# katehai/m-cedm

Measured on AMD Instinct MI355X. Metric: denoised_states_per_sec_18step_edm_heun, higher is better.
Workload: dtype f32; 1 GPU; SWE-periodic 128x128, EDM U-Net ch=128 ch_mult=[1,1,1,1] attn@16^2 (BASELINE config 3); states_per_gpu=32, global_batch=32, H=128, W=128, sampler=EDM Heun, 18 steps, 35 NFE/state, S_churn=0, w=0, fp64 state / fp32 net, parallelism=batch-sharded x1, no data-path collective, launch=one HIP graph per sampler call

## Files before the change

### include/mcedm_hip.h

```cpp
#ifndef MCEDM_HIP_H_
#define MCEDM_HIP_H_

#include <stddef.h>
#include <stdint.h>

#ifdef __cplusplus
extern "C" {
#endif

#define MCEDM_ABI_VERSION 4
#define MCEDM_REDUCE_SCRATCH_BYTES (4096 * 8 + 64)
#define MCEDM_MAX_LEVELS 8

typedef enum {
  MCEDM_OK = 0,
  MCEDM_ERR_INVALID = -1,
  MCEDM_ERR_UNSUPPORTED = -2,
  MCEDM_ERR_WORKSPACE = -3,
  MCEDM_ERR_HIP = -4
} mcedm_status;

#define MCEDM_DX_NONE 0
#define MCEDM_DX_CAT 1
#define MCEDM_DX_ENC 2
typedef struct {
  int32_t in_channels;
  int32_t cond_channels;
  int32_t out_channels;
  int32_t ch;
  int32_t n_levels;
  int32_t ch_mult[MCEDM_MAX_LEVELS];
  int32_t num_res_blocks;
  int32_t resolution;
  int32_t n_attn_resolutions;
  int32_t attn_resolutions[MCEDM_MAX_LEVELS];
  int32_t channels_per_head;
  float eps;
  int32_t dx_channels;
  int32_t dx_mode;
} mcedm_unet_desc;

typedef struct {
  int32_t timesteps;
  double sigma_min, sigma_max, rho;
  double S_churn, S_min, S_max, S_noise;
  double w;
  double sigma_data;
  double net_sigma_min, net_sigma_max;
} mcedm_sampler_desc;

typedef struct mcedm_plan mcedm_plan;

int mcedm_version(void);
const char* mcedm_last_error(void);

int mcedm_unet_plan_create(const mcedm_unet_desc* desc, mcedm_plan** out);
void mcedm_unet_plan_destroy(mcedm_plan* plan);

#define MCEDM_VARIANT_CONV_WINO 0
#define MCEDM_VARIANT_CONV_WINO1 1
#define MCEDM_VARIANT_CONV_RESIDENT 2
#define MCEDM_VARIANT_CONV8 3
#define MCEDM_VARIANT_ATTN_FUSED 4
#define MCEDM_VARIANT_WGRAD_WINO 5
#define MCEDM_VARIANT_CONV1X1_REG 6
#define MCEDM_VARIANT_CONV_WINO_FOLD 7
#define MCEDM_VARIANT_CONV_WINO_UPZ 8
int mcedm_unet_plan_set_variant(mcedm_plan* plan, int which, int value);

int mcedm_unet_param_count(const mcedm_plan* plan);
int mcedm_unet_param_info(const mcedm_plan* plan, int index, const char** name, int64_t* numel,
                          int32_t* ndim, int64_t shape[4]);

int mcedm_unet_packed_bytes(const mcedm_plan* plan, size_t* bytes);
int mcedm_unet_pack_weights(const mcedm_plan* plan, const float* const* params, void* packed, void* stream);

int mcedm_unet_workspace_bytes(const mcedm_plan* plan, int B, int H, int W, int training, size_t* bytes);

int mcedm_unet_forward(const mcedm_plan* plan, const void* packed, const float* x, const float* cond,
                       const float* x_scale, const float* noise_labels, int n_noise, float* out,
                       void* workspace, size_t workspace_bytes, int B, int H, int W, int training,
                       void* stream);

int mcedm_edm_denoise(const mcedm_plan* plan, const void* packed, const float* x, const float* sigma,
                      int n_sigma, const float* cond, float* D_out, float* F_out, void* workspace,
                      size_t workspace_bytes, int B, int H, int W, int training, double sigma_data,
                      void* stream);

int mcedm_sampler_workspace_bytes(const mcedm_plan* plan, int B, int H, int W, size_t* bytes);
int mcedm_heun_sample(const mcedm_plan* plan, const void* packed, const mcedm_sampler_desc* sp,
                      const float* cond, const float* mask, const float* init_noise,
                      const double* step_noise, double* out, int return_last, void* workspace,
                      size_t workspace_bytes, int B, int H, int W, void* stream);

int mcedm_heun_sample_rng(const mcedm_plan* plan, const void* packed, const mcedm_sampler_desc* sp, const float* cond,
                          const float* mask, const float* init_noise, const uint64_t* rng_seed, double* out, int return_last,
                          void* workspace, size_t workspace_bytes, int B, int H, int W, void* stream);
typedef struct {
  int32_t system;
  float half_dt, dx;
  float two_dx;
  float sub_h, div_h, sub_u, div_u;
  double weight;
} mcedm_guidance_desc;
int mcedm_heun_sample_guided(const mcedm_plan* plan, const void* packed, const mcedm_sampler_desc* sp,
                             const mcedm_guidance_desc* gd, const float* cond, const float* mask,
                             const float* init_noise, const double* step_noise, double* out, int return_last,
                             void* workspace, size_t workspace_bytes, int B, int H, int W, void* stream);
int mcedm_heun_sample_guided_rng(const mcedm_plan* plan, const void* packed, const mcedm_sampler_desc* sp,
                                 const mcedm_guidance_desc* gd, const float* cond, const float* mask, const float* init_noise,
                                 const uint64_t* rng_seed, double* out, int return_last, void* workspace, size_t workspace_bytes,
                                 int B, int H, int W, void* stream);
int mcedm_unet_forward_dx(const mcedm_plan* plan, const void* packed, const float* x, const float* dx, const float* cond,
                          const float* x_scale, const float* noise_labels, int n_noise, float* out, void* workspace,
                          size_t workspace_bytes, int B, int H, int W, int training, void* stream);
int mcedm_edm_denoise_dx(const mcedm_plan* plan, const void* packed, const float* x, const float* dx, const float* sigma,
                         int n_sigma, const float* cond, float* D_out, float* F_out, void* workspace,
                         size_t workspace_bytes, int B, int H, int W, int training, double sigma_data, void* stream);
int mcedm_edm_denoise_backward_dx(const mcedm_plan* plan, const void* packed, const float* const* params, const float* x,
                                  const float* dx, const float* sigma, int n_sigma, const float* cond, const float* dD,
                                  float* const* grads, void* workspace, size_t workspace_bytes, int B, int H, int W,
                                  double sigma_data, int n_buckets, const int32_t* bucket_first_param,
                                  void* const* bucket_events, void* stream);
int mcedm_heun_sample_dxcond(const mcedm_plan* plan, const void* packed, const mcedm_sampler_desc* sp,
                             const mcedm_guidance_desc* dxc, const mcedm_guidance_desc* gd, const float* cond,
                             const float* init_noise, const double* step_noise, double* out, int return_last,
                             void* workspace, size_t workspace_bytes, int B, int H, int W, void* stream);
int mcedm_heun_sample_dxcond_rng(const mcedm_plan* plan, const void* packed, const mcedm_sampler_desc* sp,
                                 const mcedm_guidance_desc* dxc, const mcedm_guidance_desc* gd, const float* cond,
                                 const float* init_noise, const uint64_t* rng_seed, double* out, int return_last, void* workspace,
                                 size_t workspace_bytes, int B, int H, int W, void* stream);
int mcedm_edm_t_steps(const mcedm_sampler_desc* sp, double* t_steps);

int mcedm_edm_loss(const float* D, const float* x, const float* mask, const float* sigma, int B, int C,
                   int H, int W, double sigma_data, float* loss_out, float* dD_out, void* scratch, size_t scratch_bytes,
                   void* stream);

int mcedm_edm_noise_inputs(const float* x, const float* mask, const float* noise, const float* rnd_normal,
                           int B, int C, int H, int W, double P_mean, double P_std, float* x_noise,
                           float* sigma_out, void* stream);

int mcedm_edm_denoise_backward(const mcedm_plan* plan, const void* packed, const float* const* params,
                               const float* x, const float* sigma, int n_sigma, const float* cond,
                               const float* dD, float* const* grads, void* workspace,
                               size_t workspace_bytes, int B, int H, int W, double sigma_data, void* stream);

int mcedm_unet_grad_buckets(const mcedm_plan* plan, int max_buckets, int32_t* first_param, int* n_buckets);
int mcedm_edm_denoise_backward_bucketed(const mcedm_plan* plan, const void* packed, const float* const* params,
                                        const float* x, const float* sigma, int n_sigma, const float* cond,
                                        const float* dD, float* const* grads, void* workspace,
                                        size_t workspace_bytes, int B, int H, int W, double sigma_data,
                                        int n_buckets, const int32_t* bucket_first_param,
                                        void* const* bucket_events, void* stream);

int mcedm_sqnorm(const float* g, size_t n, double* sqnorm_out, void* scratch, size_t scratch_bytes, void* stream);

int mcedm_adam_ema_step(float* param, const float* grad, float* exp_avg, float* exp_avg_sq, float* ema,
                        size_t n, double lr, double beta1, double beta2, double eps, double weight_decay,
                        const double* sqnorm, double max_norm, double grad_scale, double ema_beta,
                        int64_t step, void* stream);


int mcedm_eps_noise_inputs(const float* x, const float* noise, const int64_t* t, const float* sqrt_ab, const float* sqrt_1mab,
                           int n_table, int B, int C, int H, int W, float* x_noise, float* labels, void* stream);
int mcedm_eps_self_cond(const float* x_noise, const float* F0, const int64_t* t, const float* sqrt_ab, const float* sqrt_1mab,
                        int n_table, const float* cond, int cond_channels, int in_channels, int B, int H, int W,
                        float* cond_out, void* stream);
int mcedm_eps_loss(const float* F, const float* eps, int B, int C, int H, int W, float* loss_out, float* dF_out, void* scratch,
                   size_t scratch_bytes, void* stream);
int mcedm_unet_backward(const mcedm_plan* plan, const void* packed, const float* const* params, const float* x,
                        const float* cond, const float* x_scale, const float* noise_labels, int n_noise, const float* dF,
                        float* const* grads, void* workspace, size_t workspace_bytes, int B, int H, int W, void* stream);
int mcedm_unet_backward_bucketed(const mcedm_plan* plan, const void* packed, const float* const* params, const float* x,
                                 const float* cond, const float* x_scale, const float* noise_labels, int n_noise,
                                 const float* dF, float* const* grads, void* workspace, size_t workspace_bytes, int B, int H,
                                 int W, int n_buckets, const int32_t* bucket_first_param, void* const* bucket_events,
                                 void* stream);

typedef struct {
  int32_t timesteps;
  int32_t cond_channels;
  const double* t_steps;
  const double* t_hat;
  const float* c_noise;
  double S_noise;
// ... 32 lines not shown
                     mcedm_coef* coef_out, float* stats_out, void* stream);
int mcedm_op_conv(const float* xa, const float* xb, int Ca, int Cb, const mcedm_coef* coef, int coef_batch, int act,
                  int resample, int Hs, int Ws, int H, int W, const float* wpk, const float* bias_pk,
                  const float* res, int res_mode, float* out, int Cout, int B, int k, void* stream);
size_t mcedm_op_conv_wino_packed_floats(int Cout, int Cin);
int mcedm_op_pack_conv_wino(const float* w, int Cout, int Cin, float* wino, void* stream);
int mcedm_op_conv_wino(const float* xa, const float* xb, int Ca, int Cb, const mcedm_coef* coef, int coef_batch, int act,
                       int resample, int H, int W, const float* wino, const float* bias, const float* res, int res_mode,
                       float* out, int Cout, int B, void* stream);
int mcedm_op_conv_wino_sums(const float* xa, const float* xb, int Ca, int Cb, const mcedm_coef* coef, int coef_batch, int act,
                            int resample, int H, int W, const float* wino, const float* bias, const float* res, int res_mode,
                            float* out, float* gsum, int Cout, int B, void* stream);
int mcedm_op_pack_conv_wino_dgrad(const float* w, int Cout, int Cin, float* wino, void* stream);
int mcedm_op_embedding(const float* labels, int n, int ch, const float* w0, const float* b0, const float* w1,
                       const float* b1, const float* waff, const float* baff, int rows, float* freqs_scratch,
                       float* emb_out, float* film_out, void* stream);
int mcedm_op_attention(const float* qkv, float* out, int B, int heads, int T, void* stream);
int mcedm_op_attn_block64(const float* y, const float* gamma, const float* beta, float eps, const float* wq_pk,
                          const float* bq_pk, const float* wp_pk, const float* bp_pk, float* z, float* gsum, int B, void* stream);
size_t mcedm_op_wgrad_scratch_floats(int Cout, int Cin, int k, int B, int H, int W);
int mcedm_op_conv_wgrad(const float* dy, const float* xa, const float* xb, int Ca, int Cb, const mcedm_coef* coef,
                        int coef_batch, int act, int resample, int Hs, int Ws, int H, int W, int Cout, int B, int k,
                        int qkv_heads, float* scratch, float* dw, float* db, void* stream);
int mcedm_op_gn_bwd(const float* dact, int resample, const float* xa, const float* xb, int Ca, int Cb, int Hs, int Ws,
                    int B, const mcedm_coef* coef, const float* stats, const float* gamma, const float* beta,
                    const float* film, int film_batch, int film_stride, int act, float* dxa, float* dxb, int accumulate,
                    const float* add, int add_mode, float* ab, float* dgamma, float* dbeta, float* dfilm,
                    int dfilm_stride, void* stream);
#define MCEDM_GN_SYNC_WORDS 130
int mcedm_op_gn_bwd_sync(const float* dact, int resample, const float* xa, const float* xb, int Ca, int Cb, int Hs, int Ws,
                         int B, const mcedm_coef* coef, const float* stats, const float* gamma, const float* beta,
                         const float* film, int film_batch, int film_stride, int act, float* dxa, float* dxb, int accumulate,
                         const float* add, int add_mode, float* ab, float* dgamma, float* dbeta, float* dfilm,
                         int dfilm_stride, unsigned int* sync, void* stream);
int mcedm_op_attention_bwd(const float* qkv, const float* a, const float* da, float* dqkv, float* lse_scratch, int B,
                           int heads, int T, void* stream);
int mcedm_op_ddim_cond_step(const float* xt, const float* F, const float* Fu, const float* noise, double w, float s0, float s1,
                            float sa_next, float c1, float c2, float* xt_next, float* condp, float* condp_u, int cond_channels,
                            int plan_cond_channels, int B, int C, int H, int W, float* xs, int T_xs, int t_xs, float* x0s,
                            int T_x0, int t_x0, void* stream);
int mcedm_op_ddim_cond_step_rng(const float* xt, const float* F, const float* Fu, const uint64_t* rng_seed, uint64_t draw, double w,
                                float s0, float s1, float sa_next, float c1, float c2, float* xt_next, float* condp, float* condp_u,
                                int cond_channels, int plan_cond_channels, int B, int C, int H, int W, float* xs, int T_xs,
                                int t_xs, float* x0s, int T_x0, int t_x0, void* stream);
int mcedm_op_set_conv_tile(int mt, int ph, int pw);
int mcedm_op_set_conv8(int enable);
int mcedm_op_set_conv_resident(int enable);
int mcedm_op_set_conv_wino(int enable);
int mcedm_op_set_conv_wino1(int enable);
int mcedm_op_set_wgrad_wino(int enable);
int mcedm_op_set_conv1x1_reg(int enable);
int mcedm_op_set_conv_wino_fold(int enable);
int mcedm_op_set_conv_wino_upz(int enable);
int mcedm_op_pack_conv_frag(const float* w, int Cout, int Cin, float* wfrag, void* stream);
int mcedm_op_conv_skip(const float* x, int Cin, const mcedm_coef* coef, int act, int H, int W, const float* wpk, const float* wino,
                       const float* bias, const float* res, const float* sk_xa, const float* sk_xb, int sk_Ca, int sk_Cb,
                       const float* sk_wpk, const float* sk_wfrag, const float* sk_bias, float* out, float* gsum, int Cout, int B,
                       void* stream);
int mcedm_op_set_attn_fused(int enable);
int mcedm_op_set_conv_debug(unsigned long long* buf);

typedef struct {
  int32_t in_channels;
  int32_t out_channels;
  int32_t ch;
  int32_t n_levels;
  int32_t ch_mult[MCEDM_MAX_LEVELS];
  int32_t num_res_blocks;
  int32_t resolution;
  int32_t n_attn_resolutions;
  int32_t attn_resolutions[MCEDM_MAX_LEVELS];
  int32_t self_cond;
  float eps;
} mcedm_ddpm_desc;

typedef struct {
  int32_t timesteps;
  double sigma_min, sigma_max, rho;
  double S_churn, S_min, S_max, S_noise;
  double w;
  int32_t n_repeat;
  int32_t n_time_h, n_time_u;
  int32_t h_ch, u_ch;
  int32_t num_diffusion_timesteps;
  const float* edm_steps;
  const float* alphas_cumprod_ext;
} mcedm_repaint_desc;

typedef struct mcedm_ddpm_plan mcedm_ddpm_plan;
int mcedm_ddpm_plan_create(const mcedm_ddpm_desc* desc, mcedm_ddpm_plan** out);
void mcedm_ddpm_plan_destroy(mcedm_ddpm_plan* plan);
int mcedm_ddpm_plan_set_variant(mcedm_ddpm_plan* plan, int which, int value);
int mcedm_ddpm_param_count(const mcedm_ddpm_plan* plan);
int mcedm_ddpm_param_info(const mcedm_ddpm_plan* plan, int index, const char** name, int64_t* numel, int32_t* ndim,
                          int64_t shape[4]);
int mcedm_ddpm_packed_bytes(const mcedm_ddpm_plan* plan, size_t* bytes);
int mcedm_ddpm_pack_weights(const mcedm_ddpm_plan* plan, const float* const* params, const float* temb_freqs, void* packed,
                            void* stream);
int mcedm_ddpm_workspace_bytes(const mcedm_ddpm_plan* plan, int B, size_t* bytes);
int mcedm_ddpm_forward(const mcedm_ddpm_plan* plan, const void* packed, const float* x, float t, float* out, void* workspace,
                       size_t workspace_bytes, int B, void* stream);
int mcedm_ddpm_denoise(const mcedm_ddpm_plan* plan, const void* packed, const float* x, float sigma, float c_noise,
                       float* D_out, float* F_out, void* workspace, size_t workspace_bytes, int B, void* stream);
int mcedm_repaint_schedule(const mcedm_repaint_desc* sp, double* t_steps);
int mcedm_repaint_workspace_bytes(const mcedm_ddpm_plan* plan, int B, size_t* bytes);
int mcedm_repaint_sample(const mcedm_ddpm_plan* plan, const void* packed, const mcedm_repaint_desc* sp, const float* hu,
// ... 76 lines not shown
```

### m-cedm_amd/csrc/common.hpp

```cpp
#pragma once
#include <hip/hip_runtime.h>
#include <cstdarg>
#include <cstdint>
#include <cstdio>

#include "mcedm_hip.h"

namespace mcedm {

void set_error(const char* fmt, ...);

#define MCEDM_HIP_TRY(expr)                                                                   \
  do {                                                                                        \
    hipError_t e__ = (expr);                                                                  \
    if (e__ != hipSuccess) {                                                                  \
      ::mcedm::set_error("%s failed: %s (%s:%d)", #expr, hipGetErrorString(e__), __FILE__, __LINE__); \
      return MCEDM_ERR_HIP;                                                                   \
    }                                                                                         \
  } while (0)

#define MCEDM_LAUNCH_CHECK(what)                                                               \
  do {                                                                                        \
    hipError_t e__ = hipGetLastError();                                                       \
    if (e__ != hipSuccess) {                                                                  \
      ::mcedm::set_error("launch of %s failed: %s", what, hipGetErrorString(e__));            \
      return MCEDM_ERR_HIP;                                                                   \
    }                                                                                         \
  } while (0)

#define MCEDM_REQUIRE(cond, ...)                                                              \
  do {                                                                                        \
    if (!(cond)) {                                                                            \
      ::mcedm::set_error(__VA_ARGS__);                                                        \
      return MCEDM_ERR_INVALID;                                                               \
    }                                                                                         \
  } while (0)

enum KernelVariant { KV_CONV_WINO = 0, KV_CONV_WINO1 = 1, KV_CONV_RESIDENT = 2, KV_CONV8 = 3, KV_ATTN_FUSED = 4, KV_WGRAD_WINO = 5,
                     KV_CONV1X1_REG = 6, KV_CONV_WINO_FOLD = 7, KV_CONV_WINO_UPZ = 8, KV_COUNT = 9 };
struct KernelVariants { int v[KV_COUNT] = {-1, -1, -1, -1, -1, -1, -1, -1, -1}; };
const KernelVariants* current_variants();
struct VariantScope {
  const KernelVariants* prev;
  explicit VariantScope(const KernelVariants* kv);
  ~VariantScope();
};
static inline int variant_choice(int which, int global, int env_default) {
  const KernelVariants* kv = current_variants();
  if (kv && kv->v[which] >= 0) return kv->v[which];
  return global >= 0 ? global : env_default;
}

typedef float f32x16 __attribute__((ext_vector_type(16)));
typedef float f32x4 __attribute__((ext_vector_type(4)));
typedef float f32x2 __attribute__((ext_vector_type(2)));

static inline int ceil_div(int a, int b) { return (a + b - 1) / b; }
#ifdef __HIPCC__
__device__ __forceinline__ void xcd_group_map(int map, int& bx, int& by) {
  const int nx = gridDim.x, ny = gridDim.y;
  bx = blockIdx.x; by = blockIdx.y;
  if (!map || (ny & 7) != 0) return;
  const int lin = bx + by * nx;
  const int c = lin & 7, i = lin >> 3;
  by = (i / nx) * 8 + c;
  bx = i - (i / nx) * nx;
}
#endif

static inline size_t align_up(size_t v, size_t a) { return (v + a - 1) / a * a; }

struct __attribute__((aligned(16))) Coef {
  float mean, scale, offset, pad;
};

enum Resample { RS_NONE = 0, RS_UP = 1, RS_DOWN = 2, RS_S2 = 3 };

struct SumTiles {
  int tiles = 0;
  int tiles_x = 0;
  int ph = 0, pw = 0;
  int rc = 4;
};
__host__ __device__ static inline int sum_tile_count(const SumTiles& g, int t, int H, int W) {
  const int ty = t / g.tiles_x, tx = t - ty * g.tiles_x;
  const int h = H - ty * g.ph < g.ph ? H - ty * g.ph : g.ph;
  const int w = W - tx * g.pw < g.pw ? W - tx * g.pw : g.pw;
  return g.rc * h * w;
}

struct GnArgs {
  const float* xa; const float* xb; int Ca, Cb;
  int HW, B, groups;
// ... 10 lines not shown
};
int launch_gn_coef_from_sums(const GnArgs& a, hipStream_t stream);
int launch_gn_coef(const GnArgs& a, hipStream_t stream);
bool gn_sums_usable(const GnArgs& a);

struct ConvArgs {
  const float* xa;
  const float* xb;
  int Ca, Cb;
  const Coef* coef;
  int coef_batch;
  int act;
  int resample;
  int Hs, Ws;
  int H, W;
  const float* wpk;
  const float* wino;
  const float* bias;
  const float* res;
  int res_mode;
  float* out;
  int Cout;
  int B;
  float* gsum;
  int gsum_rc;
  SumTiles* gsum_tiles;
  const float* sk_xa; const float* sk_xb; int sk_Ca, sk_Cb;
  const float* sk_wpk; const float* sk_bias;
  GnArgs gn; int gn_on;
  int coef_rows;
  unsigned long long* dbg;
  const float* sk_wfrag;
};

int launch_conv(const ConvArgs& a, int taps, hipStream_t stream);
size_t conv_wino_packed_floats(int Cout, int Cin);
int launch_pack_conv_wino(const float* w, float* dst, int Cout, int Cin, int transpose_flip, hipStream_t stream);
bool conv_wino_applicable(const ConvArgs& a, int taps);
bool conv_wino_shape_ok(int Cout, int Cin, int H, int W);
bool conv_wino_fold_shape_ok(int Cout, int sk_Ca, int sk_Cb, int H, int W);
void set_conv_wino_fold(int enable);
void set_conv_wino_upz(int enable);
size_t conv_frag_packed_floats(int Cout, int Cin);
int launch_pack_conv_frag(const float* w, float* dst, int Cout, int Cin, hipStream_t stream);
void set_conv_wino(int enable);
bool conv_wino_preferred(const ConvArgs& a);
int launch_conv_wino(const ConvArgs& a, hipStream_t stream);
static inline int cout_padded(int Cout) { return (Cout + 31) / 32 * 32; }
int conv_resolve_identity(ConvArgs& a);
unsigned long long* conv_debug_buffer();
int try_launch_conv_resident(const ConvArgs& a, int taps, hipStream_t stream);
int try_launch_conv1x1_reg(const ConvArgs& a, int taps, hipStream_t stream);
void set_conv1x1_reg(int enable);
void set_conv_resident(int enable);
static inline int conv_max_tiles(int H, int W) { return ((H + 3) / 4) * ((W + 7) / 8); }
void set_conv_tile_override(int mt, int ph, int pw);
void set_conv8(int enable);
void set_conv_debug(unsigned long long* buf);
int conv_mt_for(int Cout);
int conv_kc_for(int taps);
size_t conv_packed_floats(int Cout, int Cin, int taps);
int launch_pack_conv(const float* w, float* dst, int Cout, int Cin, int taps, int qkv_heads, int transpose_flip,
                     hipStream_t stream);
int launch_pack_bias(const float* b, float* dst, int Cout, int qkv_heads, hipStream_t stream);



struct EmbArgs {
  const float* labels; int n;
  int ch;
  const float* freqs;
  const float* w0; const float* b0; const float* w1; const float* b1;
  const float* waff; const float* baff; int rows;
  float* emb;
  float* film;
};
int launch_embedding(const EmbArgs& a, hipStream_t stream);

int launch_attention(const float* qkv, float* out, int B, int heads, int T, hipStream_t stream);
bool attn_block_fused_applicable(int C, int heads, int H, int W, int groups);
int launch_attn_block64(const float* y, float* z, const float* gamma, const float* beta, float eps, int groups, const float* wq,
                        const float* bq, const float* wp, const float* bp, float* gsum, SumTiles* gsum_tiles, int B,
                        hipStream_t stream);
void set_attn_fused(int enable);

}
```

### m-cedm_amd/csrc/conv_mfma.hip

```cpp
#include <atomic>
#include <cstdlib>

#include "common.hpp"
#include "conv_tile.hpp"
#include "pack.hpp"
#include "prof.hpp"

namespace mcedm {

__device__ Coef k_identity_coef = {0.f, 1.f, 0.f, 0.f};


template <class C>
__device__ __forceinline__ void conv_skip_phase(const ConvArgs& p, const TileGeom<C, RS_NONE>& G, float* xl, float* wl,
                                                f32x16 (&acc)[C::TM][C::TN], int n, int m0, int coutp, int aoff,
                                                const int (&boff)[C::TN], int tid, int wave) {
  static_assert(C::TAPS == 9, "the folded projection rides on a 3x3 conv");
  constexpr int SUB = TileGeom<C, RS_NONE>::SUB;
  constexpr int KS = 8;
  constexpr int V4 = C::MT / 4;
  constexpr int NV4 = KS * V4;
  static_assert(NV4 <= C::NT && C::KC == KS, "one float4 of the skip slab per thread");
  const int Cin = p.sk_Ca + p.sk_Cb;
  const int iters = (Cin + KS - 1) / KS;
// ... 738 lines not shown
  if (TAPS == 9 && a.W >= 24 && (long long)a.H * a.W <= 1024) {
    if (coutp % 128 == 0 && blocks_for(128, 8, 16) >= want) return launch_cfg<ConvCfg<128, 8, 16, 1, 4, TAPS, KC>>(a, stream);
    if (coutp % 64 == 0) return launch_cfg<ConvCfg<64, 8, 16, 1, 4, TAPS, KC, 256, MID_CPI>>(a, stream);
    return launch_cfg<ConvCfg<32, 8, 32, 1, 4, TAPS, KC>>(a, stream);
  }
  if (a.W >= 24) {
    static int conv8_env = -1;
    if (conv8_env < 0) { const char* e = getenv("MCEDM_CONV8"); conv8_env = e ? atoi(e) : 0; }
    if (variant_choice(KV_CONV8, g_conv8, conv8_env) && !a.sk_wpk && a.gsum_rc != 2 && TAPS == 9 && a.resample == RS_NONE && coutp % 128 == 0 && a.Ca + a.Cb <= 2048 &&
        blocks_for(128, 16, 32) >= 224)
      return launch_conv8(a, stream);
    if (coutp % 128 == 0 && blocks_for(128, 8, 32) >= want) return launch_cfg<ConvCfg<128, 8, 32, 1, 4, TAPS, KC>>(a, stream);
    if (coutp % 64 == 0 && blocks_for(64, 8, 32) >= want) return launch_cfg<ConvCfg<64, 8, 32, 1, 4, TAPS, KC>>(a, stream);
    return launch_cfg<ConvCfg<32, 8, 32, 1, 4, TAPS, KC>>(a, stream);
  }
  if (coutp % 128 == 0 && blocks_for(128, 16, 16) >= want) return launch_cfg<ConvCfg<128, 16, 16, 1, 4, TAPS, KC>>(a, stream);
  if (coutp % 64 == 0 && blocks_for(64, 16, 16) >= want) return launch_cfg<ConvCfg<64, 16, 16, 1, 4, TAPS, KC>>(a, stream);
  return launch_cfg<ConvCfg<32, 16, 16, 1, 4, TAPS, KC>>(a, stream);
#endif
}

int launch_conv(const ConvArgs& a, int taps, hipStream_t stream) {
  MCEDM_REQUIRE(taps == 9 || taps == 1, "conv: taps must be 9 or 1 (got %d)", taps);
  MCEDM_REQUIRE(a.B > 0 && a.H > 0 && a.W > 0 && a.Cout > 0 && a.Ca + a.Cb > 0, "conv: empty shape");
  MCEDM_REQUIRE(a.out && a.wpk, "conv: null output / weights");
  if (a.resample == RS_UP) MCEDM_REQUIRE(a.Hs * 2 == a.H && a.Ws * 2 == a.W, "conv: up-resample needs H = 2*Hs");
  else if (a.resample == RS_DOWN) MCEDM_REQUIRE(a.Hs == a.H * 2 && a.Ws == a.W * 2, "conv: down-resample needs Hs = 2*H");
  else if (a.resample == RS_S2) MCEDM_REQUIRE(taps == 9 && a.Hs == a.H * 2 && a.Ws == a.W * 2 && !a.res,
                                              "conv: the stride-2 conv is 3x3 on an even-sized source, without residual");
  else MCEDM_REQUIRE(a.Hs == a.H && a.Ws == a.W, "conv: source size mismatch");
  if (a.res && a.res_mode == RS_UP) MCEDM_REQUIRE(a.H % 2 == 0 && a.W % 2 == 0, "conv: up residual needs even size");
  if (a.sk_wpk) MCEDM_REQUIRE(taps == 9 && a.resample == RS_NONE && a.sk_Ca + a.sk_Cb > 0 && (a.sk_xa || a.sk_xb) && a.Cout > 4,
                              "conv: a folded 1x1 projection rides on an un-resampled 3x3 conv with more than 4 output channels");
  MCEDM_REQUIRE((unsigned long long)a.Hs * a.Ws * 4ull < (1ull << 32) &&
                (unsigned long long)cout_padded(a.Cout) * (a.Ca + a.Cb + 16) * taps * 4ull < (1ull << 32),
                "conv: plane or weight table exceeds the 4 GiB buffer range");
  if (a.res) {
    const unsigned long long rpix = a.res_mode == RS_DOWN ? 4ull * a.H * a.W : a.res_mode == RS_UP ? (a.H / 2ull) * (a.W / 2ull)
                                                                                                    : 1ull * a.H * a.W;
    MCEDM_REQUIRE(rpix * a.Cout * 4ull < (1ull << 32), "conv: one sample of the residual exceeds the 4 GiB buffer range");
  }
  if (taps == 9 && a.Cout <= 4 && a.resample == RS_NONE && !a.res && !a.gsum && !g_force_mt && (long long)a.H * a.W >= 4096)
    return launch_small_cout(a, stream);
  if (a.resample == RS_S2) return dispatch_s2(a, stream);
  if (!g_force_mt && taps == 9 && a.wino && conv_wino_preferred(a) && conv_wino_applicable(a, taps)) return launch_conv_wino(a, stream);
  if (!g_force_mt && taps == 1) {
    const int rc = try_launch_conv1x1_reg(a, taps, stream);
    if (rc != -1) return rc;
  }
  if (!g_force_mt) {
    const int rc = try_launch_conv_resident(a, taps, stream);
    if (rc != -1) return rc;
  }
  return taps == 9 ? dispatch<9, 8>(a, stream) : dispatch<1, 16>(a, stream);
}

}
```

### m-cedm_amd/csrc/edm.hip

```cpp
#include "common.hpp"
#include "edm.hpp"

namespace mcedm {

static inline int grid_for(size_t n) {
  size_t b = (n + 255) / 256;
  return (int)(b < 2048 ? (b ? b : 1) : 2048);
}

__global__ void precond_prepare_kernel(const float* __restrict__ sigma_dev, float sigma_host, int use_host, int n,
                                       float sigma_data, int cond_ch, int in_ch, int dx_ch, float* __restrict__ coefs4,
                                       float* __restrict__ c_noise, Coef* __restrict__ conv_in_coef) {
  const int i = blockIdx.x * blockDim.x + threadIdx.x;
  if (i >= n) return;
  const float s = use_host ? sigma_host : sigma_dev[i];
  const float sd2 = sigma_data * sigma_data;
  const float s2 = s * s;
  const float c_skip = sd2 / (s2 + sd2);
  const float c_out = s * sigma_data / sqrtf(s2 + sd2);
  const float c_in = 1.0f / sqrtf(sd2 + s2);
  const float cn = logf(s) / 4.0f;
  coefs4[4 * i + 0] = c_skip;
  coefs4[4 * i + 1] = c_out;
  coefs4[4 * i + 2] = c_in;
  coefs4[4 * i + 3] = cn;
  c_noise[i] = cn;
  const int Ct = cond_ch + in_ch + dx_ch;
  for (int c = 0; c < Ct; ++c)
    conv_in_coef[(size_t)i * Ct + c] = Coef{0.f, (c < cond_ch || c >= cond_ch + in_ch) ? 1.0f : c_in, 0.f, 0.f};
}

int launch_precond_prepare(const float* sigma_dev, float sigma_host, int use_host, int n, float sigma_data,
                           int cond_ch, int in_ch, int dx_ch, float* coefs4, float* c_noise, Coef* conv_in_coef,
                           hipStream_t stream) {
  hipLaunchKernelGGL(precond_prepare_kernel, dim3(ceil_div(n, 64)), dim3(64), 0, stream, sigma_dev, sigma_host,
                     use_host, n, sigma_data, cond_ch, in_ch, dx_ch, coefs4, c_noise, conv_in_coef);
  MCEDM_LAUNCH_CHECK("precond_prepare_kernel");
  return MCEDM_OK;
}

__global__ void precond_finish_kernel(const float* __restrict__ x, const float* __restrict__ F,
                                      const float* __restrict__ Fu, float w, const float* __restrict__ coefs4,
                                      int n_sigma, size_t per_sample, size_t total, float* __restrict__ D,
                                      float* __restrict__ F_out) {
  for (size_t i = blockIdx.x * (size_t)blockDim.x + threadIdx.x; i < total; i += (size_t)gridDim.x * blockDim.x) {
    const size_t b = n_sigma == 1 ? 0 : i / per_sample;
    float f = F[i];
    if (Fu) f = (w + 1.0f) * f - w * Fu[i];
    if (F_out) F_out[i] = f;
    D[i] = coefs4[4 * b] * x[i] + coefs4[4 * b + 1] * f;
  }
}

int launch_precond_finish(const float* x, const float* F, const float* Fu, float w, const float* coefs4, int n_sigma,
                          size_t per_sample, size_t total, float* D, float* F_out, hipStream_t stream) {
  hipLaunchKernelGGL(precond_finish_kernel, dim3(grid_for(total)), dim3(256), 0, stream, x, F, Fu, w, coefs4, n_sigma,
                     per_sample, total, D, F_out);
  MCEDM_LAUNCH_CHECK("precond_finish_kernel");
  return MCEDM_OK;
}

__global__ void heun_init_kernel(const float* __restrict__ cond, int cond_ch, int in_ch, size_t hw,
                                 const float* __restrict__ mask, const float* __restrict__ noise, double t0,
                                 size_t total, double* __restrict__ x, float* __restrict__ x32) {
  for (size_t i = blockIdx.x * (size_t)blockDim.x + threadIdx.x; i < total; i += (size_t)gridDim.x * blockDim.x) {
    const size_t b = i / (in_ch * hw), r = i % (in_ch * hw);
    const float m = mask ? mask[i] : 1.0f;
    const float known = mask ? cond[b * cond_ch * hw + r] : 0.0f;
    const float keep = known * (1.0f - m);
    const double v = (double)keep + ((double)noise[i] * t0) * (double)m;
    x[i] = v;
    x32[i] = (float)v;
  }
}

__global__ void heun_churn_kernel(double* __restrict__ x, const double* __restrict__ eps, const float* __restrict__ mask,
                                  double c, size_t total, float* __restrict__ x32) {
  for (size_t i = blockIdx.x * (size_t)blockDim.x + threadIdx.x; i < total; i += (size_t)gridDim.x * blockDim.x) {
    const double v = x[i] + (c * eps[i]) * (mask ? (double)mask[i] : 1.0);
    x[i] = v;
    x32[i] = (float)v;
  }
}

__global__ void heun_euler_kernel(const double* __restrict__ x_hat, const float* __restrict__ D,
                                  const float* __restrict__ mask, double t_hat, double dt, size_t total,
                                  double* __restrict__ d_cur, double* __restrict__ x_next, float* __restrict__ x32,
                                  const float* __restrict__ dxg, float wgt, float gdiv) {
  for (size_t i = blockIdx.x * (size_t)blockDim.x + threadIdx.x; i < total; i += (size_t)gridDim.x * blockDim.x) {
    const double xh = x_hat[i];
    double d = (xh - (double)D[i]) / t_hat;
    if (dxg) d = d - (double)((wgt * dxg[i]) / gdiv);
    const double v = xh + (dt * d) * (mask ? (double)mask[i] : 1.0);
    d_cur[i] = d;
    x_next[i] = v;
    x32[i] = (float)v;
  }
}

__global__ void heun_correct_kernel(const double* __restrict__ x_hat, const double* __restrict__ d_cur,
                                    const float* __restrict__ D, const float* __restrict__ mask, double t_next, double dt,
                                    size_t total, double* __restrict__ x_next, float* __restrict__ x32,
                                    const float* __restrict__ dxg, float wgt, float gdiv) {
  for (size_t i = blockIdx.x * (size_t)blockDim.x + threadIdx.x; i < total; i += (size_t)gridDim.x * blockDim.x) {
    double dp = (x_next[i] - (double)D[i]) / t_next;
    if (dxg) dp = dp - (double)((wgt * dxg[i]) / gdiv);
    const double v = x_hat[i] + (dt * (0.5 * d_cur[i] + 0.5 * dp)) * (mask ? (double)mask[i] : 1.0);
    x_next[i] = v;
    x32[i] = (float)v;
  }
}

__global__ void heun_store_kernel(const double* __restrict__ x, int C, size_t hw, int t, int T, size_t total,
                                  double* __restrict__ out) {
  for (size_t i = blockIdx.x * (size_t)blockDim.x + threadIdx.x; i < total; i += (size_t)gridDim.x * blockDim.x) {
    const size_t c = i % C;
    const size_t p = (i / C) % hw;
    const size_t b = i / (C * hw);
    out[((b * T + t) * hw + p) * C + c] = x[(b * C + c) * hw + p];
  }
}

int launch_heun_init(const float* cond, int cond_ch, int in_ch, size_t hw, const float* mask, const float* noise,
                     double t0, size_t total, double* x, float* x32, hipStream_t s) {
  hipLaunchKernelGGL(heun_init_kernel, dim3(grid_for(total)), dim3(256), 0, s, cond, cond_ch, in_ch, hw, mask, noise, t0,
                     total, x, x32);
  MCEDM_LAUNCH_CHECK("heun_init_kernel");
  return MCEDM_OK;
}
int launch_heun_churn(double* x, const double* eps, const float* mask, double c, size_t total, float* x32, hipStream_t s) {
  hipLaunchKernelGGL(heun_churn_kernel, dim3(grid_for(total)), dim3(256), 0, s, x, eps, mask, c, total, x32);
  MCEDM_LAUNCH_CHECK("heun_churn_kernel");
  return MCEDM_OK;
}
int launch_heun_euler(const double* x_hat, const float* D, const float* mask, double t_hat, double dt, size_t total,
                      double* d_cur, double* x_next, float* x32, hipStream_t s, const float* dxg, float wgt, float gdiv) {
  hipLaunchKernelGGL(heun_euler_kernel, dim3(grid_for(total)), dim3(256), 0, s, x_hat, D, mask, t_hat, dt, total, d_cur,
                     x_next, x32, dxg, wgt, gdiv);
  MCEDM_LAUNCH_CHECK("heun_euler_kernel");
  return MCEDM_OK;
}
int launch_heun_correct(const double* x_hat, const double* d_cur, const float* D, const float* mask, double t_next,
                        double dt, size_t total, double* x_next, float* x32, hipStream_t s, const float* dxg, float wgt,
                        float gdiv) {
  hipLaunchKernelGGL(heun_correct_kernel, dim3(grid_for(total)), dim3(256), 0, s, x_hat, d_cur, D, mask, t_next, dt,
                     total, x_next, x32, dxg, wgt, gdiv);
  MCEDM_LAUNCH_CHECK("heun_correct_kernel");
  return MCEDM_OK;
}
int launch_heun_store(const double* x, int C, size_t hw, int t, int T, size_t total, double* out, hipStream_t s) {
  hipLaunchKernelGGL(heun_store_kernel, dim3(grid_for(total)), dim3(256), 0, s, x, C, hw, t, T, total, out);
  MCEDM_LAUNCH_CHECK("heun_store_kernel");
  return MCEDM_OK;
}

__device__ __forceinline__ void philox4x32_10(unsigned (&c)[4], unsigned k0, unsigned k1) {
#pragma unroll
  for (int r = 0; r < 10; ++r) {
    const unsigned long long p0 = 0xD2511F53ull * c[0], p1 = 0xCD9E8D57ull * c[2];
    const unsigned n0 = (unsigned)(p1 >> 32) ^ c[1] ^ k0, n1 = (unsigned)p1;
    const unsigned n2 = (unsigned)(p0 >> 32) ^ c[3] ^ k1, n3 = (unsigned)p0;
    c[0] = n0; c[1] = n1; c[2] = n2; c[3] = n3;
    k0 += 0x9E3779B9u; k1 += 0xBB67AE85u;
  }
}
__device__ __forceinline__ void normal_pair(const unsigned (&c)[4], double& z0, double& z1) {
  const double u1 = ((double)((((unsigned long long)c[0] << 32) | c[1]) >> 11) + 1.0) * (1.0 / 9007199254740992.0);
  const double u2 = (double)((((unsigned long long)c[2] << 32) | c[3]) >> 11) * (1.0 / 9007199254740992.0);
  const double r = sqrt(-2.0 * log(u1));
  double sn, cs;
  sincos(6.283185307179586476925 * u2, &sn, &cs);
  z0 = r * cs; z1 = r * sn;
}
__global__ void heun_churn_rng_kernel(double* __restrict__ x, const unsigned long long* __restrict__ seed_dev,
                                      unsigned long long draw, double c, size_t total, float* __restrict__ x32,
                                      const float* __restrict__ mask) {
  const unsigned long long seed = *seed_dev;
  const size_t pairs = (total + 1) / 2;
  for (size_t i = blockIdx.x * (size_t)blockDim.x + threadIdx.x; i < pairs; i += (size_t)gridDim.x * blockDim.x) {
    unsigned ctr[4] = {(unsigned)i, (unsigned)((unsigned long long)i >> 32), (unsigned)draw, (unsigned)(draw >> 32)};
    philox4x32_10(ctr, (unsigned)seed, (unsigned)(seed >> 32));
    double z0, z1;
    normal_pair(ctr, z0, z1);
    const double m0 = mask ? (double)mask[2 * i] : 1.0;
    const double v0 = x[2 * i] + (c * z0) * m0;
    x[2 * i] = v0; x32[2 * i] = (float)v0;
    if (2 * i + 1 < total) {
      const double m1 = mask ? (double)mask[2 * i + 1] : 1.0;
      const double v1 = x[2 * i + 1] + (c * z1) * m1;
      x[2 * i + 1] = v1; x32[2 * i + 1] = (float)v1;
    }
  }
}
int launch_heun_churn_rng(double* x, const unsigned long long* seed_dev, unsigned long long draw, double c, size_t total, float* x32,
                          hipStream_t s, const float* mask) {
  hipLaunchKernelGGL(heun_churn_rng_kernel, dim3(grid_for((total + 1) / 2)), dim3(256), 0, s, x, seed_dev, draw, c, total, x32, mask);
  MCEDM_LAUNCH_CHECK("heun_churn_rng_kernel");
// ... 599 lines not shown
```

### m-cedm_amd/csrc/edm.hpp

```cpp
#pragma once
#include <cmath>
#include <vector>

#include "common.hpp"

namespace mcedm {

int launch_precond_prepare(const float* sigma_dev, float sigma_host, int use_host, int n, float sigma_data,
                           int cond_ch, int in_ch, int dx_ch, float* coefs4, float* c_noise, Coef* conv_in_coef,
                           hipStream_t stream);
int launch_precond_finish(const float* x, const float* F, const float* Fu, float w, const float* coefs4, int n_sigma,
                          size_t per_sample, size_t total, float* D, float* F_out, hipStream_t stream);
int launch_heun_init(const float* cond, int cond_ch, int in_ch, size_t hw, const float* mask, const float* noise,
                     double t0, size_t total, double* x, float* x32, hipStream_t s);
int launch_heun_churn(double* x, const double* eps, const float* mask, double c, size_t total, float* x32,
                      hipStream_t s);
int launch_heun_churn_rng(double* x, const unsigned long long* seed_dev, unsigned long long draw, double c, size_t total, float* x32,
                          hipStream_t s, const float* mask = nullptr);
int launch_normal_fill(double* out, const unsigned long long* seed_dev, unsigned long long draw, size_t total, hipStream_t s);
int launch_uniform_fill(float* out, const unsigned long long* seed_dev, unsigned long long draw, size_t total, hipStream_t s);
int launch_heun_euler(const double* x_hat, const float* D, const float* mask, double t_hat, double dt, size_t total,
                      double* d_cur, double* x_next, float* x32, hipStream_t s, const float* dxg = nullptr, float wgt = 0.f,
                      float gdiv = 1.f);
int launch_heun_correct(const double* x_hat, const double* d_cur, const float* D, const float* mask, double t_next,
                        double dt, size_t total, double* x_next, float* x32, hipStream_t s, const float* dxg = nullptr,
                        float wgt = 0.f, float gdiv = 1.f);
int launch_heun_store(const double* x, int C, size_t hw, int t, int T, size_t total, double* out, hipStream_t s);

struct GuideIO {
  const float* in[2]; const float* gt[2];
  long in_sb[2], st, sx;
  float* out[2]; long out_sb[2], out_st, out_sx;
  float sub[2], div[2];
  int mean;
};
int launch_swe_guidance(const GuideIO& io, int B, int T, int X, float half_dt, float dx, float scale2_h, float scale2_u,
                        hipStream_t s);
int launch_darcy_guidance(const GuideIO& io, float* scratch, int B, int S, float two_dx, int calc_prob, hipStream_t s);

int launch_vp_finish(const float* x, const float* F, float sigma, size_t total, float* D, hipStream_t s);
int launch_vp_coef(float c_in, int n_self, int n_in, Coef* out, hipStream_t s);
int launch_vp_prepare(float c_in, int n_rows, float c_noise, Coef* coef, float* label, hipStream_t s);
int launch_vp_cfg_finish(const float* x, const float* F, const float* Fu, double w, float sigma, size_t total, float* D,
                         hipStream_t s);
int launch_edm_cfg_finish(const float* x, const float* F, const float* Fu, double w, float c_skip, float c_out, size_t total,
                          float* D, float* F_out, hipStream_t s);
int launch_repaint_init(const float* hu, const float* noise, const float* mask, float sa, float sb, double t0, size_t total,
                        double* x, float* x32, hipStream_t s);
int launch_repaint_known(double* x, const float* hu, const float* noise, const float* mask, float sa, float sb, int final_clean,
                         size_t total, float* x32, hipStream_t s);

int launch_ddim_x0(float* xt, const float* et, const float* hu, const float* mask, float s0, float s1, int renoise, size_t total,
                   float* x0, hipStream_t s);
int launch_ddim_next(const float* x0, const float* et, const float* hu, const float* hn, const float* mask, const float* noise,
                     float sa, float c1, float c2, size_t total, float* xt, hipStream_t s);
int launch_ddim_next_rng(const float* x0, const float* et, const float* hu, const float* hn, const float* mask,
                         const unsigned long long* seed_dev, unsigned long long draw, float sa, float c1, float c2, size_t total,
                         float* xt, hipStream_t s);
int launch_ddim_init(const float* hu, const float* hn, const float* mask, float sa, float sb, size_t total, float* xt, hipStream_t s);
int launch_store_f32(const float* x, int C, size_t hw, int t, int T, size_t total, float* out, hipStream_t s);

static inline std::vector<int> ddim_timestep_seq(int n, int N, int skip_type) {
  std::vector<int> seq;
  if (skip_type == 0) {
    const int skip = n / N;
    for (int v = 0; v < n; v += skip) seq.push_back(v);
  } else {
    const double hi = std::sqrt(n * 0.8);
    const double step = N > 1 ? hi / (double)(N - 1) : 0.0;
    for (int i = 0; i < N; ++i) {
      const double v = (N > 1 && i == N - 1) ? hi : (double)i * step;
      seq.push_back((int)(v * v));
    }
  }
  return seq;
}

struct DdimCondStep {
  const float *xt, *F, *Fu, *noise;
// ... 14 lines not shown
```

### m-cedm_amd/csrc/heun.hpp

```cpp
#pragma once
#include <cmath>
#include <utility>
#include <vector>

#include "edm.hpp"
#include "plan.hpp"

namespace mcedm {

struct HeunBufs { size_t x, xn, d, x32, D, total; };
template <class Bufs>
static inline size_t heun_take(Bufs& b, size_t bytes) { size_t o = b.total; b.total += align_up(bytes, 256); return o; }
static inline HeunBufs heun_bufs(size_t n) {
  HeunBufs b{};
  b.x = heun_take(b, n * 8); b.xn = heun_take(b, n * 8); b.d = heun_take(b, n * 8);
  b.x32 = heun_take(b, n * 4); b.D = heun_take(b, n * 4);
  return b;
}

struct HeunState {
  double *x, *xn, *d;
  float *x32, *D;
  int C;
  size_t hw, total;
  int N, Tout, return_last;
  hipStream_t s;
  double* out;
};
static inline HeunState heun_state(void* ws, const HeunBufs& b, int B, int C, size_t hw, int N, int return_last, double* out,
                                   hipStream_t s) {
  return HeunState{at<double>(ws, b.x), at<double>(ws, b.xn), at<double>(ws, b.d), at<float>(ws, b.x32), at<float>(ws, b.D),
                   C, hw, (size_t)B * C * hw, N, return_last ? 1 : N + 1, return_last, s, out};
}

static inline int heun_check_workspace(const char* who, size_t have, size_t need) {
  if (need > have) {
    set_error("%s: workspace too small (%zu < %zu bytes)", who, have, need);
    return MCEDM_ERR_WORKSPACE;
  }
  return MCEDM_OK;
}

static inline int heun_store_step(const HeunState& h, int slot) {
  return h.return_last ? MCEDM_OK : launch_heun_store(h.x, h.C, h.hw, slot, h.Tout, h.total, h.out, h.s);
}
static inline int heun_store_last(const HeunState& h) {
  return h.return_last ? launch_heun_store(h.x, h.C, h.hw, 0, 1, h.total, h.out, h.s) : MCEDM_OK;
}

static inline int heun_churn(const HeunState& h, double c, const double* eps, const unsigned long long* seed,
                             unsigned long long draw, const float* mask) {
  if (eps) return launch_heun_churn(h.x, eps, mask, c, h.total, h.x32, h.s);
  return launch_heun_churn_rng(h.x, seed, draw, c, h.total, h.x32, h.s, mask);
}

template <class Denoise>
static inline int heun_update(HeunState& h, int i, double t_hat, double t_next, const float* mask, Denoise&& denoise,
                              const float* dxg = nullptr, float wgt = 0.f, float gdiv = 1.f) {
  int rc;
  if ((rc = denoise(t_hat, false))) return rc;
  if ((rc = launch_heun_euler(h.x, h.D, mask, t_hat, t_next - t_hat, h.total, h.d, h.xn, h.x32, h.s, dxg, wgt, gdiv)))
    return rc;
  if (i < h.N - 1) {
    if ((rc = denoise(t_next, true))) return rc;
    if ((rc = launch_heun_correct(h.x, h.d, h.D, mask, t_next, t_next - t_hat, h.total, h.xn, h.x32, h.s, dxg, wgt, gdiv)))
      return rc;
  }
  std::swap(h.x, h.xn);
  return MCEDM_OK;
}

static inline int guidance_dx(int cond_channels, const mcedm_guidance_desc& g, const float* cond, const float* D, float* dx,
                              float* scratch, int B, int H, int W, hipStream_t s) {
  GuideIO io{};
  const long hw = (long)H * W;
  io.in[0] = cond; io.in[1] = D; io.gt[0] = cond; io.gt[1] = D;
  io.in_sb[0] = (long)cond_channels * hw; io.in_sb[1] = hw; io.st = W; io.sx = 1;
  io.out[0] = dx; io.out[1] = nullptr; io.out_sb[0] = hw; io.out_sb[1] = 0; io.out_st = W; io.out_sx = 1;
  io.sub[0] = g.sub_h; io.sub[1] = g.sub_u; io.div[0] = g.div_h; io.div[1] = g.div_u;
  io.mean = 1;
  if (g.system == 1)
    return launch_swe_guidance(io, B, H, W, g.half_dt, g.dx, g.div_h * g.div_h, g.div_u * g.div_u, s);
  MCEDM_REQUIRE(H == W && H > 4, "guidance: the Darcy residual needs a square grid larger than 4 x 4 (got %d x %d)", H, W);
  return launch_darcy_guidance(io, scratch, B, H, g.two_dx, 1, s);
}

static inline int vp_check_schedule(const mcedm_vp_sampler_desc* sp, const double* step_noise, const uint64_t* rng_seed) {
  MCEDM_REQUIRE(sp->timesteps >= 1 && sp->timesteps <= 4096, "vp_heun_sample: timesteps=%d out of range", sp->timesteps);
  for (int i = 0; i < sp->timesteps; ++i) {
    MCEDM_REQUIRE(sp->t_hat[i] >= sp->t_steps[i] && sp->t_steps[i] > 0.0, "vp_heun_sample: step %d: t_hat %g < t_cur %g or t_cur <= 0", i,
                  sp->t_hat[i], sp->t_steps[i]);
    MCEDM_REQUIRE(sp->t_hat[i] == sp->t_steps[i] || step_noise != nullptr || rng_seed != nullptr,
                  "vp_heun_sample: step %d churns (t_hat > t_cur) and needs step_noise (or mcedm_vp_heun_sample_rng)", i);
  }
  return MCEDM_OK;
}

template <class Denoise>
static inline int vp_heun_loop(HeunState& h, const mcedm_vp_sampler_desc* sp, const float* init_noise, const double* step_noise,
                               const uint64_t* rng_seed, Denoise&& denoise, const float* dxg = nullptr, float wgt = 0.f) {
  int rc;
  const int N = sp->timesteps;
  const double* t = sp->t_steps;
  if ((rc = launch_heun_init(nullptr, 0, h.C, h.hw, nullptr, init_noise, t[0], h.total, h.x, h.x32, h.s))) return rc;
  if ((rc = heun_store_step(h, 0))) return rc;
  for (int i = 0; i < N; ++i) {
    const double t_cur = t[i], t_next = t[i + 1], t_hat = sp->t_hat[i];
    if (t_hat != t_cur) {
      const double c = std::sqrt(t_hat * t_hat - t_cur * t_cur) * sp->S_noise;
      if ((rc = heun_churn(h, c, step_noise ? step_noise + (size_t)i * h.total : nullptr,
                           reinterpret_cast<const unsigned long long*>(rng_seed), (unsigned long long)i, nullptr))) return rc;
    }
    auto at_level = [&](double sigma, bool second) { return denoise(sigma, sp->c_noise[2 * i + (second ? 1 : 0)]); };
    if ((rc = heun_update(h, i, t_hat, t_next, nullptr, at_level, dxg, wgt, dxg ? (float)t_hat : 1.f))) return rc;
    if ((rc = heun_store_step(h, i + 1))) return rc;
  }
  return heun_store_last(h);
}
// ... 71 lines not shown
```

### m-cedm_amd/csrc/norm_emb_attn.hip

```cpp
#include <cstdlib>
#include <atomic>
#include "common.hpp"
#include "prof.hpp"

namespace mcedm {

__global__ __launch_bounds__(256) void gn_coef_kernel(GnArgs a) {
  const int C = a.Ca + a.Cb;
  const int cpg = C / a.groups;
  const int n = blockIdx.x / a.groups;
  const int g = blockIdx.x % a.groups;
  const int c0 = g * cpg;
  auto plane = [&](int c) {
    return (c < a.Ca) ? a.xa + ((size_t)n * a.Ca + c) * a.HW : a.xb + ((size_t)n * a.Cb + (c - a.Ca)) * a.HW;
  };
  const int N = cpg * a.HW;
  const float shift = plane(c0)[0];
  float s1[4] = {0.f, 0.f, 0.f, 0.f}, s2[4] = {0.f, 0.f, 0.f, 0.f};
  const int tid = threadIdx.x;
  for (int cl = 0; cl < cpg; ++cl) {
    const float* src = plane(c0 + cl);
    if ((a.HW & 3) == 0) {
      const float4* s4 = reinterpret_cast<const float4*>(src);
      const int N4 = a.HW >> 2;
// ... 158 lines not shown
#pragma unroll
  for (int off = 32; off > 0; off >>= 1)
#pragma unroll
    for (int r = 0; r < R; ++r) s[r] += __shfl_xor(s[r], off);
#pragma unroll
  for (int r = 0; r < R; ++r) out[r] = s[r];
}

constexpr int EMB_NT = 1024, EMB_R = 4;
__global__ __launch_bounds__(EMB_NT) void embedding_kernel(EmbArgs a) {
  extern __shared__ float sm[];
  float* e0 = sm;
  float* e1 = sm + a.ch;
  constexpr int NW = EMB_NT / 64;
  const int n = blockIdx.x, split = blockIdx.y, nsplit = gridDim.y;
  const int tid = threadIdx.x, lane = tid & 63, wave = tid >> 6, ch = a.ch, half = a.ch / 2;
  const float x = a.labels[n];
  for (int k = tid; k < ch; k += EMB_NT) {
    const float arg = x * a.freqs[k < half ? k : k - half];
    e0[k] = (k < half) ? cosf(arg) : sinf(arg);
  }
  __syncthreads();
  float s[EMB_R];
  for (int j = wave * EMB_R; j < ch; j += NW * EMB_R) {
    wave_dot_rows<EMB_R>(e0, a.w0 + (size_t)j * ch, ch, ch - j, ch, lane, s);
    if (lane == 0)
      for (int r = 0; r < EMB_R && j + r < ch; ++r) e1[j + r] = silu_e(s[r] + a.b0[j + r]);
  }
  __syncthreads();
  for (int j = wave * EMB_R; j < ch; j += NW * EMB_R) {
    wave_dot_rows<EMB_R>(e1, a.w1 + (size_t)j * ch, ch, ch - j, ch, lane, s);
    if (lane == 0)
      for (int r = 0; r < EMB_R && j + r < ch; ++r) {
        const float v = silu_e(s[r] + a.b1[j + r]);
        e0[j + r] = v;
        if (a.emb && split == 0) a.emb[(size_t)n * ch + j + r] = v;
      }
  }
  __syncthreads();
  const int per = (a.rows + nsplit - 1) / nsplit;
  const int r1 = min(a.rows, (split + 1) * per);
  for (int r0 = split * per + wave * EMB_R; r0 < r1; r0 += NW * EMB_R) {
    wave_dot_rows<EMB_R>(e0, a.waff + (size_t)r0 * ch, ch, r1 - r0, ch, lane, s);
    if (lane == 0)
      for (int r = 0; r < EMB_R && r0 + r < r1; ++r) a.film[(size_t)n * a.rows + r0 + r] = s[r] + a.baff[r0 + r];
  }
}

int launch_embedding(const EmbArgs& a, hipStream_t stream) {
  MCEDM_REQUIRE(a.n > 0 && a.ch > 0 && a.ch % 2 == 0, "embedding: bad shape n=%d ch=%d", a.n, a.ch);
  int nsplit = a.rows / 64;
  if (nsplit > 512 / a.n) nsplit = 512 / a.n;
  if (nsplit < 1) nsplit = 1;
  hipLaunchKernelGGL(embedding_kernel, dim3(a.n, nsplit), dim3(EMB_NT), 2 * a.ch * sizeof(float), stream, a);
  MCEDM_LAUNCH_CHECK("embedding_kernel");
  return MCEDM_OK;
}

__global__ __launch_bounds__(64) void attention_kernel(const float* __restrict__ qkv, float* __restrict__ out,
                                                       int T) {
  const int lane = threadIdx.x;
  const int l31 = lane & 31, h = lane >> 5;
  const int q0 = blockIdx.x * 32;
  const size_t bh = blockIdx.y;
  const float* Q = qkv + (bh * 3 + 0) * 64 * (size_t)T;
  const float* K = qkv + (bh * 3 + 1) * 64 * (size_t)T;
  const float* V = qkv + (bh * 3 + 2) * 64 * (size_t)T;
  const int q = q0 + l31;
  const int qc = q < T ? q : T - 1;

  float qreg[32];
#pragma unroll
  for (int s = 0; s < 32; ++s) qreg[s] = Q[(size_t)(2 * s + h) * T + qc] * 0.125f;

  float m = -INFINITY, l = 0.f;
  f32x16 o[2];
#pragma unroll
  for (int i = 0; i < 2; ++i)
#pragma unroll
    for (int r = 0; r < 16; ++r) o[i][r] = 0.f;

  for (int k0 = 0; k0 < T; k0 += 32) {
    const bool full = (k0 + 32 <= T);
    const int kk = k0 + l31;
    const int kc = kk < T ? kk : T - 1;
    f32x16 s;
#pragma unroll
    for (int r = 0; r < 16; ++r) s[r] = 0.f;
#pragma unroll
    for (int st = 0; st < 32; ++st) {
      const float a = K[(size_t)(2 * st + h) * T + kc];
      s = __builtin_amdgcn_mfma_f32_32x32x2f32(a, qreg[st], s, 0, 0, 0);
    }
    float mx = -INFINITY;
#pragma unroll
    for (int r = 0; r < 16; ++r) {
      const int key = k0 + (r & 3) + 8 * (r >> 2) + 4 * h;
      if (!full && key >= T) s[r] = -INFINITY;
      mx = fmaxf(mx, s[r]);
    }
    mx = fmaxf(mx, __shfl_xor(mx, 32));
    const float m_new = fmaxf(m, mx);
    const float alpha = expf(m - m_new);
    float p[16];
    float rs = 0.f;
#pragma unroll
// ... 343 lines not shown
```

### m-cedm_amd/csrc/ops_api.hip

```cpp
#include "common.hpp"
#include "conv_wino.hpp"
#include "bwd.hpp"
#include "edm.hpp"

using namespace mcedm;

static_assert(sizeof(mcedm_coef) == sizeof(Coef), "mcedm_coef must mirror Coef");

extern "C" size_t mcedm_op_conv_packed_floats(int Cout, int Cin, int k) {
  if (Cout <= 0 || Cin <= 0 || (k != 1 && k != 3)) return 0;
  return conv_packed_floats(Cout, Cin, k * k);
}

extern "C" int mcedm_op_pack_conv(const float* w, const float* b, int Cout, int Cin, int k, int qkv_heads, int dgrad,
                                  float* wpk, float* bias_pk, void* stream) {
  MCEDM_REQUIRE(w && wpk, "op_pack_conv: null pointer");
  MCEDM_REQUIRE(Cout > 0 && Cin > 0 && (k == 1 || k == 3), "op_pack_conv: bad shape");
  MCEDM_REQUIRE(qkv_heads == 0 || (Cout % (3 * qkv_heads) == 0 && !dgrad), "op_pack_conv: bad qkv_heads");
  int rc = dgrad ? launch_pack_conv(w, wpk, Cin, Cout, k * k, 0, 1, (hipStream_t)stream)
                 : launch_pack_conv(w, wpk, Cout, Cin, k * k, qkv_heads, 0, (hipStream_t)stream);
  if (rc) return rc;
  if (b && bias_pk) rc = launch_pack_bias(b, bias_pk, Cout, qkv_heads, (hipStream_t)stream);
  return rc;
}
// ... 153 lines not shown
              stats, gamma, film, film_batch, film_stride, act, dxa, dxb, accumulate, add, add_mode, C, ab};
  a.sync = sync;
  int rc = launch_gn_bwd(a, (hipStream_t)stream);
  if (rc) return rc;
  return launch_gn_param_grads(ab, gamma, beta, film, film_batch, film_stride, B, C, dgamma, dbeta, dfilm, dfilm_stride,
                               (hipStream_t)stream);
}

extern "C" int mcedm_op_gn_bwd(const float* dact, int resample, const float* xa, const float* xb, int Ca, int Cb, int Hs,
                               int Ws, int B, const mcedm_coef* coef, const float* stats, const float* gamma,
                               const float* beta, const float* film, int film_batch, int film_stride, int act,
                               float* dxa, float* dxb, int accumulate, const float* add, int add_mode, float* ab,
                               float* dgamma, float* dbeta, float* dfilm, int dfilm_stride, void* stream) {
  return op_gn_bwd_impl(dact, resample, xa, xb, Ca, Cb, Hs, Ws, B, coef, stats, gamma, beta, film, film_batch, film_stride, act, dxa, dxb,
                        accumulate, add, add_mode, ab, dgamma, dbeta, dfilm, dfilm_stride, nullptr, stream);
}

extern "C" int mcedm_op_gn_bwd_sync(const float* dact, int resample, const float* xa, const float* xb, int Ca, int Cb, int Hs,
                                    int Ws, int B, const mcedm_coef* coef, const float* stats, const float* gamma,
                                    const float* beta, const float* film, int film_batch, int film_stride, int act,
                                    float* dxa, float* dxb, int accumulate, const float* add, int add_mode, float* ab,
                                    float* dgamma, float* dbeta, float* dfilm, int dfilm_stride, unsigned int* sync, void* stream) {
  return op_gn_bwd_impl(dact, resample, xa, xb, Ca, Cb, Hs, Ws, B, coef, stats, gamma, beta, film, film_batch, film_stride, act, dxa, dxb,
                        accumulate, add, add_mode, ab, dgamma, dbeta, dfilm, dfilm_stride, sync, stream);
}

extern "C" int mcedm_op_attention_bwd(const float* qkv, const float* a, const float* da, float* dqkv, float* lse_scratch,
                                      int B, int heads, int T, void* stream) {
  return launch_attention_bwd(qkv, a, da, dqkv, lse_scratch, B, heads, T, (hipStream_t)stream);
}

extern "C" int mcedm_op_set_conv8(int enable) {
  set_conv8(enable);
  return MCEDM_OK;
}

extern "C" int mcedm_op_set_conv_wino(int enable) {
  set_conv_wino(enable);
  return MCEDM_OK;
}

extern "C" int mcedm_op_set_conv_wino1(int enable) {
  set_conv_wino1(enable);
  return MCEDM_OK;
}

extern "C" int mcedm_op_set_conv_wino_fold(int enable) {
  set_conv_wino_fold(enable);
  return MCEDM_OK;
}

extern "C" int mcedm_op_set_conv_wino_upz(int enable) {
  set_conv_wino_upz(enable);
  return MCEDM_OK;
}

extern "C" int mcedm_op_set_conv1x1_reg(int enable) {
  set_conv1x1_reg(enable);
  return MCEDM_OK;
}

extern "C" int mcedm_op_set_wgrad_wino(int enable) {
  set_wgrad_wino(enable);
  return MCEDM_OK;
}

extern "C" int mcedm_op_set_conv_resident(int enable) {
  set_conv_resident(enable);
  return MCEDM_OK;
}

extern "C" int mcedm_op_set_attn_fused(int enable) {
  set_attn_fused(enable);
  return MCEDM_OK;
}

extern "C" int mcedm_op_set_conv_debug(unsigned long long* buf) {
  set_conv_debug(buf);
  return MCEDM_OK;
}

static int op_ddim_cond_step(const float* xt, const float* F, const float* Fu, const float* noise, const uint64_t* rng_seed,
                             uint64_t draw, double w, float s0, float s1, float sa_next, float c1, float c2, float* xt_next,
                             float* condp, float* condp_u, int cond_channels, int plan_cond_channels, int B, int C, int H, int W,
                             float* xs, int T_xs, int t_xs, float* x0s, int T_x0, int t_x0, void* stream) {
  MCEDM_REQUIRE(xt && F && xt_next, "op_ddim_cond_step: null pointer");
  MCEDM_REQUIRE(B > 0 && C > 0 && H > 0 && W > 0, "op_ddim_cond_step: empty shape");
  MCEDM_REQUIRE(!condp_u || condp, "op_ddim_cond_step: the twin goes with cond'");
  MCEDM_REQUIRE(!condp || (cond_channels >= 0 && cond_channels + C <= plan_cond_channels),
                "op_ddim_cond_step: channels [%d, %d) outside cond' (%d channels)", cond_channels, cond_channels + C, plan_cond_channels);
  MCEDM_REQUIRE((!xs || (t_xs >= 0 && t_xs < T_xs)) && (!x0s || (t_x0 >= 0 && t_x0 < T_x0)), "op_ddim_cond_step: slot outside the trajectory");
  DdimCondStep k{};
  k.xt = xt; k.F = F; k.Fu = Fu; k.noise = noise;
  k.seed = reinterpret_cast<const unsigned long long*>(rng_seed); k.draw = draw;
  k.w1 = (float)(w + 1.0); k.w = (float)w; k.s0 = s0; k.s1 = s1; k.sa = sa_next; k.c1 = c1; k.c2 = c2;
  k.xt_next = xt_next; k.sc = condp; k.sc_u = condp_u;
  k.C = C; k.Cp = plan_cond_channels; k.sc_off = cond_channels; k.hw = (size_t)H * W; k.n = (size_t)B * C * k.hw;
  k.xs = xs; k.x0s = x0s; k.T_xs = T_xs; k.t_xs = t_xs; k.T_x0 = T_x0; k.t_x0 = t_x0;
  return launch_ddim_cond_step(k, (hipStream_t)stream);
}
extern "C" int mcedm_op_ddim_cond_step(const float* xt, const float* F, const float* Fu, const float* noise, double w, float s0,
                                       float s1, float sa_next, float c1, float c2, float* xt_next, float* condp, float* condp_u,
                                       int cond_channels, int plan_cond_channels, int B, int C, int H, int W, float* xs,
                                       int T_xs, int t_xs, float* x0s, int T_x0, int t_x0, void* stream) {
  return op_ddim_cond_step(xt, F, Fu, noise, nullptr, 0, w, s0, s1, sa_next, c1, c2, xt_next, condp, condp_u, cond_channels,
                           plan_cond_channels, B, C, H, W, xs, T_xs, t_xs, x0s, T_x0, t_x0, stream);
// ... 11 lines not shown
```

### m-cedm_amd/csrc/plan.hip

```cpp
#include <algorithm>
#include <cmath>
#include <cstring>

#include "edm.hpp"
#include "pack.hpp"
#include "plan.hpp"
#include "prof.hpp"
#include "bwd.hpp"

namespace mcedm {

static thread_local char g_err[1024] = "";

void set_error(const char* fmt, ...) {
  va_list ap;
  va_start(ap, fmt);
  vsnprintf(g_err, sizeof(g_err), fmt, ap);
  va_end(ap);
}

static NormP make_norm(mcedm_plan& P, const std::string& key, int C) {
  NormP n;
  n.C = C;
  n.groups = std::min(32, C / 4);
// ... 448 lines not shown

  for (const BlockP& b : P.enc) {
    const int o = do_block(b, cur, -1);
    lb.retain(o);
    lb.retain(o); skips.push_back(o);
    lb.release(cur);
    cur = o;
  }
  for (const BlockP& b : P.dec) {
    int xb = -1;
    if (L.t[cur].C != b.cin) {
      MCEDM_REQUIRE(!skips.empty(), "layout: skip stack underflow at %s", b.key.c_str());
      xb = skips.back(); skips.pop_back();
      MCEDM_REQUIRE(L.t[cur].C + L.t[xb].C == b.cin && L.t[cur].H == L.t[xb].H && L.t[cur].W == L.t[xb].W,
                    "layout: concat mismatch at %s", b.key.c_str());
    }
    const int o = do_block(b, cur, xb);
    lb.retain(o);
    lb.release(cur);
    lb.release(xb);
    cur = o;
  }
  L.last = cur;
  L.coef_out = lb.coef(P.out_norm.C);
  if (training) L.stats_out = lb.stats(P.out_norm.groups);
  L.total_bytes = lb.pool.peak;
  return MCEDM_OK;
}

Header header_for(const mcedm_plan& P, int B, int H, int W) {
  Header h;
  size_t cur = 0;
  auto take = [&](size_t bytes) { size_t o = cur; cur += align_up(bytes, 256); return o; };
  const int Ct = P.desc.in_channels + P.desc.cond_channels + P.desc.dx_channels;
  h.coefs4 = take((size_t)B * 4 * sizeof(float));
  h.c_noise = take((size_t)B * sizeof(float));
  h.coef_in = take((size_t)B * Ct * sizeof(Coef));
  h.F = take((size_t)B * P.desc.out_channels * H * W * sizeof(float));
  h.Fu = take((size_t)B * P.desc.out_channels * H * W * sizeof(float));
  h.total = cur;
  return h;
}


static int gn_for_conv(const GnArgs& g, ConvArgs& c, bool need_table, hipStream_t s) {
  if (!need_table && g.stats == nullptr && gn_sums_usable(g)) {
    c.gn = g; c.gn_on = 1; c.coef = nullptr;
    return MCEDM_OK;
  }
  return launch_gn_coef_from_sums(g, s);
}

static int run_block(const mcedm_plan& P, const BlockP& b, const BlockLayout& bl, const Layout& L, void* act,
                     const float* pk, int B, int n_noise, hipStream_t s, std::vector<SumTiles>& st) {
  auto T = [&](int id) -> float* { return id < 0 ? nullptr : at<float>(act, L.t[id].off); };
  auto CF = [&](int id) -> Coef* { return id < 0 ? nullptr : at<Coef>(act, L.t[id].off); };
  auto SUMS = [&](int id) -> float* { return (id < 0 || L.t[id].sums == NONE) ? nullptr : at<float>(act, L.t[id].sums); };
  auto TL = [&](int id) -> SumTiles { return id < 0 ? SumTiles{} : st[id]; };
  const float* xa = T(bl.xa);
  const float* xb = T(bl.xb);
  const int Ca = L.t[bl.xa].C, Cb = bl.xb >= 0 ? L.t[bl.xb].C : 0;
  const float eps = P.desc.eps;
  int rc;
  GnArgs g0{xa, xb, Ca, Cb, bl.Hin * bl.Win, B, b.norm0.groups, pk + b.norm0.gamma, pk + b.norm0.beta,
            nullptr, 0, 0, eps, CF(bl.coef0), T(bl.stats0), SUMS(bl.xa), SUMS(bl.xb), TL(bl.xa), TL(bl.xb), bl.Win};
  ConvArgs c0{};
  c0.xa = xa; c0.xb = xb; c0.Ca = Ca; c0.Cb = Cb;
  c0.coef = CF(bl.coef0); c0.coef_batch = 1; c0.act = 1;
  const int rs = b.up ? RS_UP : (b.down ? RS_DOWN : RS_NONE);
  c0.resample = rs;
  c0.Hs = bl.Hin; c0.Ws = bl.Win; c0.H = bl.H; c0.W = bl.W;
  c0.wpk = pk + b.conv0.wpk; c0.bias = pk + b.conv0.bias;
  c0.wino = b.conv0.wino != NONE ? pk + b.conv0.wino : nullptr;
  c0.out = T(bl.h); c0.Cout = b.cout; c0.B = B; c0.gsum = SUMS(bl.h); c0.gsum_tiles = &st[bl.h];
  if ((rc = gn_for_conv(g0, c0, bl.xd >= 0, s))) return rc;
  if (bl.xd >= 0) {
    WgradArgs m{};
    m.xa = xa; m.xb = xb; m.Ca = Ca; m.Cb = Cb; m.coef = c0.coef; m.coef_batch = 1; m.act = 1; m.resample = RS_DOWN;
    m.Hs = bl.Hin; m.Ws = bl.Win; m.H = bl.H; m.W = bl.W; m.B = B;
    if ((rc = launch_act_materialize(m, T(bl.xd), s))) return rc;
    c0.xa = T(bl.xd); c0.xb = nullptr; c0.Ca = Ca + Cb; c0.Cb = 0;
    c0.coef = nullptr; c0.act = 0; c0.resample = RS_NONE; c0.Hs = bl.H; c0.Ws = bl.W;
  }
  if ((rc = launch_conv(c0, 9, s))) return rc;
  const float* film = at<float>(act, L.t[L.film].off) + b.film_row0;
  GnArgs g1{T(bl.h), nullptr, b.cout, 0, bl.H * bl.W, B, b.norm1.groups, pk + b.norm1.gamma, pk + b.norm1.beta,
            film, n_noise > 1 ? 1 : 0, P.film_rows, eps, CF(bl.coef1), T(bl.stats1), SUMS(bl.h), nullptr, TL(bl.h), SumTiles{}, bl.W};
  const float* res = xa;
  int res_mode = RS_NONE;
  const bool fold_skip = b.skip_kernel == 1 && (bl.sk < 0 || bl.wfold);
  if (b.skip_kernel == 1 && !fold_skip) {
    ConvArgs cs{};
    cs.xa = xa; cs.xb = xb; cs.Ca = Ca; cs.Cb = Cb;
    cs.resample = rs; cs.Hs = bl.Hin; cs.Ws = bl.Win; cs.H = bl.H; cs.W = bl.W;
    cs.wpk = pk + b.skip.wpk; cs.bias = pk + b.skip.bias;
    cs.out = T(bl.sk); cs.Cout = b.cout; cs.B = B;
    if ((rc = launch_conv(cs, 1, s))) return rc;
    res = T(bl.sk);
  } else if (b.skip_kernel == 0) {
    res_mode = rs;
  }
  ConvArgs c1{};
  c1.xa = T(bl.h); c1.Ca = b.cout;
  c1.coef = CF(bl.coef1); c1.coef_batch = 1; c1.act = 1;
  c1.Hs = bl.H; c1.Ws = bl.W; c1.H = bl.H; c1.W = bl.W;
  c1.wpk = pk + b.conv1.wpk; c1.bias = pk + b.conv1.bias;
  c1.wino = b.conv1.wino != NONE ? pk + b.conv1.wino : nullptr;
  c1.res = res; c1.res_mode = res_mode;
  if (fold_skip) {
    c1.res = nullptr; c1.res_mode = RS_NONE;
    c1.sk_xa = xa; c1.sk_xb = xb; c1.sk_Ca = Ca; c1.sk_Cb = Cb;
    c1.sk_wpk = pk + b.skip.wpk; c1.sk_bias = pk + b.skip.bias;
    c1.sk_wfrag = b.skip.wfrag != NONE ? pk + b.skip.wfrag : nullptr;
  }
  c1.out = T(bl.y); c1.Cout = b.cout; c1.B = B; c1.gsum = SUMS(bl.y); c1.gsum_tiles = &st[bl.y];
  if ((rc = gn_for_conv(g1, c1, false, s))) return rc;
  if ((rc = launch_conv(c1, 9, s))) return rc;
  if (!b.attn) return MCEDM_OK;
  if (bl.stats2 < 0 && attn_block_fused_applicable(b.cout, b.heads, bl.H, bl.W, b.norm2.groups))
    return launch_attn_block64(T(bl.y), T(bl.z), pk + b.norm2.gamma, pk + b.norm2.beta, eps, b.norm2.groups, pk + b.qkv.wpk,
                               pk + b.qkv.bias, pk + b.proj.wpk, pk + b.proj.bias, SUMS(bl.z), &st[bl.z], B, s);
  GnArgs g2{T(bl.y), nullptr, b.cout, 0, bl.H * bl.W, B, b.norm2.groups, pk + b.norm2.gamma, pk + b.norm2.beta,
            nullptr, 0, 0, eps, CF(bl.coef2), T(bl.stats2), SUMS(bl.y), nullptr, TL(bl.y), SumTiles{}, bl.W};
  ConvArgs cq{};
  cq.xa = T(bl.y); cq.Ca = b.cout;
  cq.coef = CF(bl.coef2); cq.coef_batch = 1; cq.act = 0;
  cq.Hs = bl.H; cq.Ws = bl.W; cq.H = bl.H; cq.W = bl.W;
  cq.wpk = pk + b.qkv.wpk; cq.bias = pk + b.qkv.bias;
  cq.out = T(bl.qkv); cq.Cout = 3 * b.cout; cq.B = B;
  if ((rc = gn_for_conv(g2, cq, false, s))) return rc;
  if ((rc = launch_conv(cq, 1, s))) return rc;
  if ((rc = launch_attention(T(bl.qkv), T(bl.a), B, b.heads, bl.H * bl.W, s))) return rc;
  ConvArgs cp{};
  cp.xa = T(bl.a); cp.Ca = b.cout;
  cp.Hs = bl.H; cp.Ws = bl.W; cp.H = bl.H; cp.W = bl.W;
  cp.wpk = pk + b.proj.wpk; cp.bias = pk + b.proj.bias;
  cp.res = T(bl.y); cp.res_mode = RS_NONE;
  cp.out = T(bl.z); cp.Cout = b.cout; cp.B = B; cp.gsum = SUMS(bl.z); cp.gsum_tiles = &st[bl.z];
  return launch_conv(cp, 1, s);
}

__global__ void concat_x_dx_kernel(const float* __restrict__ x, const float* __restrict__ dx, int cx, int cd, size_t hw,
                                   size_t total, float* __restrict__ out) {
  for (size_t i = blockIdx.x * (size_t)blockDim.x + threadIdx.x; i < total; i += (size_t)gridDim.x * blockDim.x) {
    const size_t per = (size_t)(cx + cd) * hw;
    const size_t n = i / per, r = i - n * per;
    out[i] = r < (size_t)cx * hw ? x[n * cx * hw + r] : (dx ? dx[n * cd * hw + (r - (size_t)cx * hw)] : 0.f);
  }
}
__global__ void gelu_kernel(const float* __restrict__ v, const float* g, float* out, size_t n, int mode) {
  for (size_t i = blockIdx.x * (size_t)blockDim.x + threadIdx.x; i < n; i += (size_t)gridDim.x * blockDim.x) {
    const float a = v[i];
    const float cdf = 0.5f * (1.0f + erff(a * 0.70710678118654752440f));
    out[i] = mode ? g[i] * (cdf + a * 0.39894228040143267794f * expf(-0.5f * a * a)) : a * cdf;
  }
}
int launch_gelu(const float* v, const float* g, float* out, size_t n, int mode, hipStream_t s) {
  const size_t b = (n + 255) / 256;
  hipLaunchKernelGGL(gelu_kernel, dim3((unsigned)(b < 4096 ? (b ? b : 1) : 4096)), dim3(256), 0, s, v, g, out, n, mode);
  MCEDM_LAUNCH_CHECK("gelu_kernel");
  return MCEDM_OK;
}

int forward_impl(const mcedm_plan& P, const Layout& L, const float* pk, const float* x, const float* dx, const float* cond,
                 const Coef* coef_in, int coef_batch, const float* noise_labels, int n_noise, float* out,
                 void* act, int B, int H, int W, hipStream_t s) {
  const int ch = P.desc.ch;
  const int dxm = P.desc.dx_mode;
  int rc;
  EmbArgs e{noise_labels, n_noise, ch, pk + P.freqs, pk + P.w0, pk + P.b0, pk + P.w1, pk + P.b1,
            pk + P.waff, pk + P.baff, P.film_rows, nullptr, at<float>(act, L.t[L.film].off)};
  if ((rc = launch_embedding(e, s))) return rc;
  std::vector<SumTiles> st(L.t.size());
  ConvArgs ci{};
  ci.xa = cond; ci.Ca = P.desc.cond_channels;
  ci.xb = x; ci.Cb = P.desc.in_channels;
  if (dxm == MCEDM_DX_CAT) {
    float* xdx = at<float>(act, L.t[L.xdx].off);
    const size_t hw = (size_t)H * W, total = (size_t)B * (P.desc.in_channels + P.desc.dx_channels) * hw;
    const size_t nb = (total + 255) / 256;
    hipLaunchKernelGGL(concat_x_dx_kernel, dim3((unsigned)(nb < 4096 ? nb : 4096)), dim3(256), 0, s, x, dx, P.desc.in_channels,
                       P.desc.dx_channels, hw, total, xdx);
    MCEDM_LAUNCH_CHECK("concat_x_dx_kernel");
    ci.xb = xdx; ci.Cb = P.desc.in_channels + P.desc.dx_channels;
  }
  ci.coef = coef_in; ci.coef_batch = coef_batch; ci.act = 0;
  ci.Hs = H; ci.Ws = W; ci.H = H; ci.W = W;
  ci.wpk = pk + P.conv_in.wpk; ci.bias = pk + P.conv_in.bias;
  ci.out = at<float>(act, L.t[L.t0].off); ci.Cout = P.conv_in.cout; ci.B = B;
  ci.gsum = at<float>(act, L.t[L.t0].sums); ci.gsum_tiles = &st[L.t0];
  if (dxm == MCEDM_DX_ENC) { ci.out = at<float>(act, L.t[L.xf].off); ci.gsum = nullptr; ci.gsum_tiles = nullptr; }
  if ((rc = launch_conv(ci, 9, s))) return rc;
  if (dxm == MCEDM_DX_ENC) {
    const int c0 = P.conv_in.cout;
    float* d2 = at<float>(act, L.t[L.d2].off);
    auto plain = [&](const ConvP& cv, const float* xa, int Ca, const float* xb, int Cb, float* o) {
      ConvArgs c{};
      c.xa = xa; c.Ca = Ca; c.xb = xb; c.Cb = Cb;
      c.Hs = H; c.Ws = W; c.H = H; c.W = W;
      c.wpk = pk + cv.wpk; c.bias = pk + cv.bias;
      c.wino = cv.wino != NONE ? pk + cv.wino : nullptr;
      c.out = o; c.Cout = cv.cout; c.B = B;
      return c;
    };
    if (dx) {
      float* d1 = at<float>(act, L.t[L.d1].off);
      float* g1 = at<float>(act, L.t[L.g1].off);
      ConvArgs ca = plain(P.dx_enc0, dx, P.desc.dx_channels, nullptr, 0, d1);
      if ((rc = launch_conv(ca, 9, s))) return rc;
      if ((rc = launch_gelu(d1, nullptr, g1, (size_t)B * c0 * H * W, 0, s))) return rc;
      ConvArgs cb = plain(P.dx_enc2, g1, c0, nullptr, 0, d2);
      if ((rc = launch_conv(cb, 9, s))) return rc;
    } else {
      MCEDM_HIP_TRY(hipMemsetAsync(d2, 0, L.t[L.d2].bytes, s));
    }
    ConvArgs cc = plain(P.combine, at<float>(act, L.t[L.xf].off), c0, d2, c0, at<float>(act, L.t[L.t0].off));
    cc.gsum = at<float>(act, L.t[L.t0].sums); cc.gsum_tiles = &st[L.t0];
    if ((rc = launch_conv(cc, 9, s))) return rc;
  }
  size_t bi = 0;
  for (const BlockP& b : P.enc) if ((rc = run_block(P, b, L.blocks[bi++], L, act, pk, B, n_noise, s, st))) return rc;
  for (const BlockP& b : P.dec) if ((rc = run_block(P, b, L.blocks[bi++], L, act, pk, B, n_noise, s, st))) return rc;
  const TRef& last = L.t[L.last];
  GnArgs go{at<float>(act, last.off), nullptr, last.C, 0, H * W, B, P.out_norm.groups, pk + P.out_norm.gamma,
            pk + P.out_norm.beta, nullptr, 0, 0, 1e-5f, at<Coef>(act, L.t[L.coef_out].off),
            L.stats_out >= 0 ? at<float>(act, L.t[L.stats_out].off) : nullptr,
            last.sums != NONE ? at<float>(act, last.sums) : nullptr, nullptr, st[L.last], SumTiles{}, W};
  ConvArgs co{};
  co.xa = at<float>(act, last.off); co.Ca = last.C;
  co.coef = at<Coef>(act, L.t[L.coef_out].off); co.coef_batch = 1; co.act = 1;
  co.Hs = H; co.Ws = W; co.H = H; co.W = W;
  co.wpk = pk + P.conv_out.wpk; co.bias = pk + P.conv_out.bias;
  co.out = out; co.Cout = P.desc.out_channels; co.B = B;
  if ((rc = gn_for_conv(go, co, false, s))) return rc;
  return launch_conv(co, 9, s);
}

__global__ void scale_to_coef_kernel(const float* __restrict__ x_scale, int n, int cond_ch, int in_ch, int dx_ch, Coef* out) {
  const int i = blockIdx.x * blockDim.x + threadIdx.x;
  if (i >= n) return;
  const int Ct = cond_ch + in_ch + dx_ch;
  for (int c = 0; c < Ct; ++c) out[(size_t)i * Ct + c] = Coef{0.f, (c < cond_ch || c >= cond_ch + in_ch) ? 1.0f : x_scale[i], 0.f, 0.f};
}

int denoise_impl(const mcedm_plan& P, const Layout& L, const Header& hd, const float* pk, const float* x, const float* dx,
                 const float* sigma_dev, float sigma_host, int use_host, int n_sigma, const float* cond,
                 float w, float* D_out, float* F_out, void* ws, int B, int H, int W, float sigma_data,
                 hipStream_t s) {
  int rc;
  float* coefs4 = at<float>(ws, hd.coefs4);
  float* c_noise = at<float>(ws, hd.c_noise);
  Coef* coef_in = at<Coef>(ws, hd.coef_in);
  float* Fbuf = at<float>(ws, hd.F);
  void* act = at<char>(ws, hd.total);
  if ((rc = launch_precond_prepare(sigma_dev, sigma_host, use_host, n_sigma, sigma_data, P.desc.cond_channels,
                                   P.desc.in_channels, P.desc.dx_mode == MCEDM_DX_CAT ? P.desc.dx_channels : 0, coefs4, c_noise,
                                   coef_in, s))) return rc;
  if ((rc = forward_impl(P, L, pk, x, dx, cond, coef_in, n_sigma > 1 ? 1 : 0, c_noise, n_sigma, Fbuf, act, B, H, W, s))) return rc;
  const float* Fu = nullptr;
  if (fabsf(w) >= 0.001f && (cond != nullptr || dx != nullptr)) {
    float* Fubuf = at<float>(ws, hd.Fu);
    if ((rc = forward_impl(P, L, pk, x, nullptr, nullptr, coef_in, n_sigma > 1 ? 1 : 0, c_noise, n_sigma, Fubuf, act, B, H, W, s))) return rc;
    Fu = Fubuf;
  }
  const size_t per = (size_t)P.desc.out_channels * H * W;
  return launch_precond_finish(x, Fbuf, Fu, w, coefs4, n_sigma, per, per * B, D_out, F_out, s);
}

}

extern "C" int mcedm_unet_workspace_bytes(const mcedm_plan* plan, int B, int H, int W, int training, size_t* bytes) {
  VariantScope variant_scope__(plan ? &plan->variants : nullptr);
  MCEDM_REQUIRE(plan && bytes, "workspace_bytes: null argument");
  Layout L;
  int rc = build_layout(*plan, B, H, W, training, B, &L);
  if (rc) return rc;
  *bytes = header_for(*plan, B, H, W).total + L.total_bytes + (training ? backward_scratch_bytes(*plan, L, B, H, W) : 0);
  return MCEDM_OK;
}

extern "C" int mcedm_unet_forward_dx(const mcedm_plan* plan, const void* packed, const float* x, const float* dx, const float* cond,
                                     const float* x_scale, const float* noise_labels, int n_noise, float* out,
                                     void* workspace, size_t workspace_bytes, int B, int H, int W, int training,
                                     void* stream) {
  VariantScope variant_scope__(plan ? &plan->variants : nullptr);
  MCEDM_REQUIRE(plan && packed && x && noise_labels && out && workspace, "unet_forward: null argument");
  MCEDM_REQUIRE(dx == nullptr || plan->desc.dx_mode != MCEDM_DX_NONE, "unet_forward: dx given to a plan without dx_cond");
  Layout L;
  int rc = build_layout(*plan, B, H, W, training, n_noise, &L);
  if (rc) return rc;
  const Header hd = header_for(*plan, B, H, W);
  if (hd.total + L.total_bytes > workspace_bytes) {
    set_error("unet_forward: workspace too small (%zu < %zu bytes)", workspace_bytes, hd.total + L.total_bytes);
    return MCEDM_ERR_WORKSPACE;
  }
  hipStream_t s = (hipStream_t)stream;
  const Coef* coef_in = nullptr;
  if (x_scale) {
    Coef* c = at<Coef>(workspace, hd.coef_in);
    hipLaunchKernelGGL(scale_to_coef_kernel, dim3(ceil_div(n_noise, 64)), dim3(64), 0, s, x_scale, n_noise,
                       plan->desc.cond_channels, plan->desc.in_channels,
                       plan->desc.dx_mode == MCEDM_DX_CAT ? plan->desc.dx_channels : 0, c);
    MCEDM_LAUNCH_CHECK("scale_to_coef_kernel");
    coef_in = c;
  }
  return forward_impl(*plan, L, (const float*)packed, x, dx, cond, coef_in, n_noise > 1 ? 1 : 0, noise_labels, n_noise, out,
                      at<char>(workspace, hd.total), B, H, W, s);
}

extern "C" int mcedm_unet_forward(const mcedm_plan* plan, const void* packed, const float* x, const float* cond,
                                  const float* x_scale, const float* noise_labels, int n_noise, float* out,
                                  void* workspace, size_t workspace_bytes, int B, int H, int W, int training,
                                  void* stream) {
  VariantScope variant_scope__(plan ? &plan->variants : nullptr);
  return mcedm_unet_forward_dx(plan, packed, x, nullptr, cond, x_scale, noise_labels, n_noise, out, workspace, workspace_bytes, B, H,
                               W, training, stream);
}
// ... 29 lines not shown
```

### m-cedm_amd/csrc/plan.hpp

```cpp
#pragma once
#include <algorithm>
#include <initializer_list>
#include <string>
#include <utility>
#include <vector>

#include "common.hpp"

namespace mcedm {

constexpr size_t NONE = (size_t)-1;

struct Pool {
  std::vector<std::pair<size_t, size_t>> free_;
  size_t top = 0, peak = 0;
  bool keep_all = false;
  size_t alloc(size_t bytes) {
    bytes = align_up(bytes ? bytes : 1, 256);
    for (size_t i = 0; i < free_.size(); ++i)
      if (free_[i].second >= bytes) {
        const size_t off = free_[i].first;
        if (free_[i].second == bytes) free_.erase(free_.begin() + i);
        else { free_[i].first += bytes; free_[i].second -= bytes; }
        return off;
// ... 111 lines not shown
  int ref = 0;
};

struct BlockLayout {
  int xa = -1, xb = -1;
  int coef0 = -1, h = -1, coef1 = -1, sk = -1, y = -1, coef2 = -1, qkv = -1, a = -1, z = -1;
  int stats0 = -1, stats1 = -1, stats2 = -1;
  int xd = -1;
  int out = -1;
  int wfold = 0;
  int Hin = 0, Win = 0, H = 0, W = 0;
};

struct Layout {
  std::vector<TRef> t;
  std::vector<BlockLayout> blocks;
  int film = -1, t0 = -1, coef_out = -1, stats_out = -1, last = -1;
  int xdx = -1, xf = -1, d1 = -1, g1 = -1, d2 = -1;
  size_t sums_base = 0, sums_bytes = 0;
  size_t total_bytes = 0;
};

}

struct mcedm_plan {
  mcedm_unet_desc desc;
  std::vector<mcedm::ParamInfo> params;
  mcedm::ConvP conv_in, conv_out;
  mcedm::ConvP dx_enc0, dx_enc2, combine;
  mcedm::NormP out_norm;
  std::vector<mcedm::BlockP> enc, dec;
  int map0_w = -1, map0_b = -1, map1_w = -1, map1_b = -1;
  size_t freqs = mcedm::NONE, w0 = mcedm::NONE, b0 = mcedm::NONE, w1 = mcedm::NONE, b1 = mcedm::NONE;
  size_t waff = mcedm::NONE, baff = mcedm::NONE;
  int film_rows = 0;
  size_t packed_floats = 0;
  int levels_div = 1;
  mcedm::KernelVariants variants;
};

namespace mcedm {
int build_layout(const mcedm_plan& P, int B, int H, int W, int training, int n_noise, Layout* out);

struct Header {
  size_t coefs4, c_noise, coef_in, F, Fu, total;
};
Header header_for(const mcedm_plan& P, int B, int H, int W);

template <class T>
static inline T* at(void* ws, size_t off) { return reinterpret_cast<T*>(reinterpret_cast<char*>(ws) + off); }

int forward_impl(const mcedm_plan& P, const Layout& L, const float* pk, const float* x, const float* dx, const float* cond,
                 const Coef* coef_in, int coef_batch, const float* noise_labels, int n_noise, float* out,
                 void* act, int B, int H, int W, hipStream_t s);
int denoise_impl(const mcedm_plan& P, const Layout& L, const Header& hd, const float* pk, const float* x, const float* dx,
                 const float* sigma_dev, float sigma_host, int use_host, int n_sigma, const float* cond,
                 float w, float* D_out, float* F_out, void* ws, int B, int H, int W, float sigma_data,
                 hipStream_t s);

size_t backward_scratch_bytes(const mcedm_plan& P, const Layout& L, int B, int H, int W);
}
```

### m-cedm_amd/csrc/sampler.hip

```cpp
#include <algorithm>
#include <cmath>
#include <vector>

#include "heun.hpp"

using namespace mcedm;

extern "C" int mcedm_edm_t_steps(const mcedm_sampler_desc* sp, double* t) {
  MCEDM_REQUIRE(sp && t, "t_steps: null argument");
  MCEDM_REQUIRE(sp->timesteps >= 2, "t_steps: timesteps=%d (the reference divides by timesteps-1)", sp->timesteps);
  const double smin = std::max(sp->sigma_min, sp->net_sigma_min);
  const double smax = std::min(sp->sigma_max, sp->net_sigma_max);
  const int N = sp->timesteps;
  const double a = std::pow(smax, 1.0 / sp->rho), b = std::pow(smin, 1.0 / sp->rho) - std::pow(smax, 1.0 / sp->rho);
  for (int i = 0; i < N; ++i) t[i] = std::pow(a + (double)i / (double)(N - 1) * b, sp->rho);
  t[N] = 0.0;
  return MCEDM_OK;
}

namespace mcedm {
struct SamplerBufs : HeunBufs { size_t dx, g, dxin; };
static SamplerBufs sampler_bufs(const mcedm_plan& P, int B, int H, int W) {
  const size_t n = (size_t)B * P.desc.in_channels * H * W;
  SamplerBufs s{heun_bufs(n), 0, 0, 0};
  s.dx = heun_take(s, n * 4); s.g = heun_take(s, n * 4);
  s.dxin = heun_take(s, n * 4);
  return s;
}
}

extern "C" int mcedm_sampler_workspace_bytes(const mcedm_plan* plan, int B, int H, int W, size_t* bytes) {
  VariantScope variant_scope__(plan ? &plan->variants : nullptr);
  MCEDM_REQUIRE(plan && bytes, "sampler_workspace_bytes: null argument");
  const int rc = mcedm_unet_workspace_bytes(plan, B, H, W, 0, bytes);
  if (rc == MCEDM_OK) *bytes += sampler_bufs(*plan, B, H, W).total;
  return rc;
}

static int heun_sample_impl(const mcedm_plan* plan, const void* packed, const mcedm_sampler_desc* sp,
                            const float* cond, const float* mask, const float* init_noise,
                            const double* step_noise, double* out, int return_last, void* workspace,
                            size_t workspace_bytes, int B, int H, int W, const mcedm_guidance_desc* gd, void* stream,
                            const mcedm_guidance_desc* dxc, const uint64_t* rng_seed) {
  MCEDM_REQUIRE(plan && packed && sp && init_noise && out && workspace, "heun_sample: null argument");
  const mcedm_plan& P = *plan;
  int rc;
  MCEDM_REQUIRE(P.desc.in_channels == P.desc.out_channels, "heun_sample: in_channels != out_channels");
  MCEDM_REQUIRE(mask == nullptr || (cond != nullptr && P.desc.cond_channels >= P.desc.in_channels),
                "heun_sample: with a mask, cond must carry hu_known in its first %d channels", P.desc.in_channels);
  MCEDM_REQUIRE(sp->timesteps >= 2 && sp->timesteps <= 4096, "heun_sample: timesteps=%d out of range", sp->timesteps);
  const int N = sp->timesteps;
  std::vector<double> t(N + 1);
  if ((rc = mcedm_edm_t_steps(sp, t.data()))) return rc;
  std::vector<double> gammas(N);
  for (int i = 0; i < N; ++i) {
    const bool in_range = sp->S_min <= t[i] && t[i] <= sp->S_max;
    gammas[i] = in_range ? std::min(sp->S_churn / N, std::sqrt(2.0) - 1.0) : 0.0;
    MCEDM_REQUIRE(gammas[i] == 0.0 || step_noise != nullptr || rng_seed != nullptr, "heun_sample: S_churn > 0 needs step_noise (or mcedm_heun_sample_rng)");
  }
  Layout L;
  if ((rc = build_layout(P, B, H, W, 0, 1, &L))) return rc;
  const Header hd = header_for(P, B, H, W);
  const SamplerBufs sb = sampler_bufs(P, B, H, W);
  if ((rc = heun_check_workspace("heun_sample", workspace_bytes, sb.total + hd.total + L.total_bytes))) return rc;
  hipStream_t s = (hipStream_t)stream;
  const float* pk = (const float*)packed;
  HeunState h = heun_state(workspace, sb, B, P.desc.in_channels, (size_t)H * W, N, return_last, out, s);
  void* uws = at<char>(workspace, sb.total);
  const float w = (float)sp->w;
  const float sd = (float)sp->sigma_data;
  float* gscratch = at<float>(workspace, sb.g);
  float* dxin = dxc ? at<float>(workspace, sb.dxin) : nullptr;
  float* dxg = gd ? at<float>(workspace, sb.dx) : nullptr;
  const float wgt = gd ? (float)gd->weight : 0.f;
  auto denoise = [&](double sigma, bool) -> int {
    int e = dxc ? guidance_dx(P.desc.cond_channels, *dxc, cond, h.x32, dxin, gscratch, B, H, W, s) : MCEDM_OK;
    if (e) return e;
    e = denoise_impl(P, L, hd, pk, h.x32, dxin, nullptr, (float)sigma, 1, 1, cond, w, h.D, nullptr, uws, B, H, W, sd, s);
    if (e) return e;
    return gd ? guidance_dx(P.desc.cond_channels, *gd, cond, h.D, dxg, gscratch, B, H, W, s) : MCEDM_OK;
  };

  if ((rc = launch_heun_init(cond, P.desc.cond_channels, h.C, h.hw, mask, init_noise, t[0], h.total, h.x, h.x32, s))) return rc;
  if ((rc = heun_store_step(h, 0))) return rc;
  for (int i = 0; i < N; ++i) {
    const double t_cur = t[i], t_next = t[i + 1];
    const double t_hat = t_cur + gammas[i] * t_cur;
    if (gammas[i] != 0.0) {
      const double c = std::sqrt(t_hat * t_hat - t_cur * t_cur) * sp->S_noise;
      if ((rc = heun_churn(h, c, step_noise ? step_noise + (size_t)i * h.total : nullptr,
                           reinterpret_cast<const unsigned long long*>(rng_seed), (unsigned long long)i, mask))) return rc;
    }
    if ((rc = heun_update(h, i, t_hat, t_next, mask, denoise, dxg, wgt, (float)t_hat))) return rc;
    if ((rc = heun_store_step(h, i + 1))) return rc;
  }
  return heun_store_last(h);
}

extern "C" int mcedm_heun_sample(const mcedm_plan* plan, const void* packed, const mcedm_sampler_desc* sp,
                                 const float* cond, const float* mask, const float* init_noise,
                                 const double* step_noise, double* out, int return_last, void* workspace,
                                 size_t workspace_bytes, int B, int H, int W, void* stream) {
  VariantScope variant_scope__(plan ? &plan->variants : nullptr);
  return heun_sample_impl(plan, packed, sp, cond, mask, init_noise, step_noise, out, return_last, workspace, workspace_bytes,
                          B, H, W, nullptr, stream, nullptr, nullptr);
}

extern "C" int mcedm_heun_sample_rng(const mcedm_plan* plan, const void* packed, const mcedm_sampler_desc* sp,
                                     const float* cond, const float* mask, const float* init_noise, const uint64_t* rng_seed,
                                     double* out, int return_last, void* workspace, size_t workspace_bytes, int B, int H, int W,
                                     void* stream) {
  VariantScope variant_scope__(plan ? &plan->variants : nullptr);
  MCEDM_REQUIRE(rng_seed != nullptr, "heun_sample_rng: rng_seed (a 64-bit seed in device memory) is null");
  return heun_sample_impl(plan, packed, sp, cond, mask, init_noise, nullptr, out, return_last, workspace, workspace_bytes,
                          B, H, W, nullptr, stream, nullptr, rng_seed);
}

static int heun_guided(const mcedm_plan* plan, const void* packed, const mcedm_sampler_desc* sp, const mcedm_guidance_desc* gd,
                       const float* cond, const float* mask, const float* init_noise, const double* step_noise,
                       const uint64_t* rng_seed, double* out, int return_last, void* workspace, size_t workspace_bytes, int B, int H,
                       int W, void* stream) {
  MCEDM_REQUIRE(gd != nullptr && (gd->system == 1 || gd->system == 2), "heun_sample_guided: guidance system must be 1 (SWE) or 2 (Darcy)");
  MCEDM_REQUIRE(plan && plan->desc.in_channels == 1 && plan->desc.cond_channels >= 1 && cond != nullptr && mask == nullptr,
                "heun_sample_guided: PDE guidance is defined for the single-task sampler (state u, conditioning h in cond[:, 0]; "
                "mask NULL), models/ddim.py:1532-1601; the joint model's hook fails in the reference (models/mcedm.py:500-518)");
  return heun_sample_impl(plan, packed, sp, cond, mask, init_noise, step_noise, out, return_last, workspace, workspace_bytes,
                          B, H, W, gd, stream, nullptr, rng_seed);
}

extern "C" int mcedm_heun_sample_guided(const mcedm_plan* plan, const void* packed, const mcedm_sampler_desc* sp,
                                        const mcedm_guidance_desc* gd, const float* cond, const float* mask,
                                        const float* init_noise, const double* step_noise, double* out, int return_last,
// ... 223 lines not shown
```

### m-cedm_amd/lib.py

```python
from __future__ import annotations

import ctypes as C
import os
from typing import Dict, List, Optional, Sequence

import torch

_HERE = os.path.dirname(os.path.abspath(__file__))
LIB_PATH = os.environ.get("MCEDM_LIB") or os.path.join(_HERE, "libmcedm_hip.so")
MAX_LEVELS = 8

EXPORTS = [
    "mcedm_version", "mcedm_last_error", "mcedm_unet_plan_create", "mcedm_unet_plan_destroy",
    "mcedm_unet_param_count", "mcedm_unet_param_info", "mcedm_unet_packed_bytes", "mcedm_unet_pack_weights",
    "mcedm_unet_workspace_bytes", "mcedm_unet_forward", "mcedm_edm_denoise", "mcedm_sampler_workspace_bytes",
    "mcedm_heun_sample", "mcedm_edm_t_steps", "mcedm_edm_loss", "mcedm_edm_noise_inputs",
    "mcedm_edm_denoise_backward", "mcedm_edm_denoise_backward_bucketed", "mcedm_unet_grad_buckets", "mcedm_sqnorm",
    "mcedm_adam_ema_step",
    "mcedm_swe_fv_step", "mcedm_swe_fv_residual", "mcedm_darcy_residual", "mcedm_swe_fv_guidance", "mcedm_darcy_guidance",
    "mcedm_heun_sample_guided",
    "mcedm_ddpm_plan_create", "mcedm_ddpm_plan_destroy", "mcedm_ddpm_param_count", "mcedm_ddpm_param_info",
    "mcedm_ddpm_packed_bytes", "mcedm_ddpm_pack_weights", "mcedm_ddpm_workspace_bytes", "mcedm_ddpm_forward",
    "mcedm_ddpm_denoise", "mcedm_repaint_schedule", "mcedm_repaint_workspace_bytes", "mcedm_repaint_sample",
    "mcedm_repaint_sample_rng", "mcedm_normal_fill", "mcedm_ddpm_forward_sc", "mcedm_ddim_workspace_bytes",
    "mcedm_ddim_repaint_sample", "mcedm_ddim_timesteps",
    "mcedm_unet_forward_dx", "mcedm_edm_denoise_dx", "mcedm_edm_denoise_backward_dx", "mcedm_heun_sample_dxcond",
    "mcedm_unet_plan_set_variant", "mcedm_ddpm_plan_set_variant", "mcedm_heun_sample_rng",
    "mcedm_eps_noise_inputs", "mcedm_eps_self_cond", "mcedm_eps_loss", "mcedm_unet_backward", "mcedm_unet_backward_bucketed",
    "mcedm_vp_sampler_workspace_bytes", "mcedm_vp_heun_sample", "mcedm_vp_heun_sample_rng",
    "mcedm_cond_ddim_workspace_bytes", "mcedm_cond_ddim_sample",
    "mcedm_uniform_fill", "mcedm_cond_ddim_sample_rng", "mcedm_ddim_repaint_sample_rng", "mcedm_heun_sample_guided_rng",
    "mcedm_heun_sample_dxcond_rng",
    "mcedm_ddpm_plan_create_cond", "mcedm_ddpm_cond_map", "mcedm_ddpm_forward_cond", "mcedm_ddpm_vp_sampler_workspace_bytes",
    "mcedm_ddpm_vp_heun_sample", "mcedm_ddpm_vp_heun_sample_rng", "mcedm_ddpm_cond_ddim_workspace_bytes",
    "mcedm_ddpm_cond_ddim_sample", "mcedm_ddpm_cond_ddim_sample_rng",
    "mcedm_ddpm_forward_cat", "mcedm_ddpm_edm_denoise", "mcedm_ddpm_edm_sampler_workspace_bytes", "mcedm_ddpm_edm_heun_sample",
    "mcedm_ddpm_edm_heun_sample_rng",
]
SAMPLER_STEMS = {
    "mcedm_heun_sample": 1, "mcedm_heun_sample_guided": 1, "mcedm_heun_sample_dxcond": 1,
    "mcedm_vp_heun_sample": 1, "mcedm_ddpm_vp_heun_sample": 1, "mcedm_cond_ddim_sample": 1, "mcedm_ddpm_cond_ddim_sample": 1,
    "mcedm_ddim_repaint_sample": 1, "mcedm_repaint_sample": 2, "mcedm_ddpm_edm_heun_sample": 1,
}
GN_SYNC_WORDS = 130
VARIANTS = {"conv_wino": 0, "conv_wino1": 1, "conv_resident": 2, "conv8": 3, "attn_fused": 4, "wgrad_wino": 5, "conv1x1_reg": 6,
            "conv_wino_fold": 7, "conv_wino_upz": 8}


class UNetDesc(C.Structure):
    _fields_ = [("in_channels", C.c_int32), ("cond_channels", C.c_int32), ("out_channels", C.c_int32),
                ("ch", C.c_int32), ("n_levels", C.c_int32), ("ch_mult", C.c_int32 * MAX_LEVELS),
                ("num_res_blocks", C.c_int32), ("resolution", C.c_int32), ("n_attn_resolutions", C.c_int32),
                ("attn_resolutions", C.c_int32 * MAX_LEVELS), ("channels_per_head", C.c_int32), ("eps", C.c_float),
                ("dx_channels", C.c_int32), ("dx_mode", C.c_int32)]


DX_NONE, DX_CAT, DX_ENC = 0, 1, 2
ABI_VERSION = 4
REDUCE_SCRATCH_BYTES = 4096 * 8 + 64


class SamplerDesc(C.Structure):
    _fields_ = [("timesteps", C.c_int32), ("sigma_min", C.c_double), ("sigma_max", C.c_double), ("rho", C.c_double),
                ("S_churn", C.c_double), ("S_min", C.c_double), ("S_max", C.c_double), ("S_noise", C.c_double),
                ("w", C.c_double), ("sigma_data", C.c_double), ("net_sigma_min", C.c_double),
                ("net_sigma_max", C.c_double)]


class GuidanceDesc(C.Structure):
    _fields_ = [("system", C.c_int32), ("half_dt", C.c_float), ("dx", C.c_float), ("two_dx", C.c_float), ("sub_h", C.c_float),
                ("div_h", C.c_float), ("sub_u", C.c_float), ("div_u", C.c_float), ("weight", C.c_double)]


class DdpmDesc(C.Structure):
    _fields_ = [("in_channels", C.c_int32), ("out_channels", C.c_int32), ("ch", C.c_int32), ("n_levels", C.c_int32),
                ("ch_mult", C.c_int32 * MAX_LEVELS), ("num_res_blocks", C.c_int32), ("resolution", C.c_int32),
                ("n_attn_resolutions", C.c_int32), ("attn_resolutions", C.c_int32 * MAX_LEVELS), ("self_cond", C.c_int32),
                ("eps", C.c_float)]


class DdpmCondDesc(C.Structure):
    _fields_ = [("cond_channels", C.c_int32), ("cat_cond", C.c_int32)]


class RepaintDesc(C.Structure):
    _fields_ = [("timesteps", C.c_int32), ("sigma_min", C.c_double), ("sigma_max", C.c_double), ("rho", C.c_double),
                ("S_churn", C.c_double), ("S_min", C.c_double), ("S_max", C.c_double), ("S_noise", C.c_double),
                ("w", C.c_double), ("n_repeat", C.c_int32), ("n_time_h", C.c_int32), ("n_time_u", C.c_int32),
                ("h_ch", C.c_int32), ("u_ch", C.c_int32), ("num_diffusion_timesteps", C.c_int32),
                ("edm_steps", C.POINTER(C.c_float)), ("alphas_cumprod_ext", C.POINTER(C.c_float))]


class DdimDesc(C.Structure):
    _fields_ = [("timesteps", C.c_int32), ("skip_type", C.c_int32), ("eta", C.c_double), ("n_repeat", C.c_int32),
                ("n_time_h", C.c_int32), ("n_time_u", C.c_int32), ("h_ch", C.c_int32), ("u_ch", C.c_int32),
                ("num_diffusion_timesteps", C.c_int32), ("self_cond", C.c_int32), ("alphas_cumprod_ext", C.POINTER(C.c_float))]


class VpSamplerDesc(C.Structure):
    _fields_ = [("timesteps", C.c_int32), ("cond_channels", C.c_int32), ("t_steps", C.POINTER(C.c_double)),
                ("t_hat", C.POINTER(C.c_double)), ("c_noise", C.POINTER(C.c_float)), ("S_noise", C.c_double), ("w", C.c_double)]


class CondDdimDesc(C.Structure):
    _fields_ = [("timesteps", C.c_int32), ("skip_type", C.c_int32), ("eta", C.c_double), ("w", C.c_double),
                ("cond_channels", C.c_int32), ("self_cond", C.c_int32), ("num_diffusion_timesteps", C.c_int32),
                ("alphas_cumprod_ext", C.POINTER(C.c_float))]


_lib = None


def load() -> C.CDLL:
    global _lib
    if _lib is not None:
        return _lib
    if not os.path.exists(LIB_PATH):
        raise RuntimeError(f"{LIB_PATH} not found: build it with `python m-cedm_amd/build.py` "
                           "(hipcc --offload-arch=gfx950); there is no CPU/PyTorch fallback")
    lib = C.CDLL(LIB_PATH)
    vp, i32, f32p, f64p, sz = C.c_void_p, C.c_int, C.c_void_p, C.c_void_p, C.c_size_t
    lib.mcedm_version.restype = C.c_int
    if lib.mcedm_version() != ABI_VERSION:
        raise RuntimeError(f"{LIB_PATH} implements ABI {lib.mcedm_version()}, this binding ABI {ABI_VERSION}: rebuild it with "
                           "`python m-cedm_amd/build.py`")
    lib.mcedm_last_error.restype = C.c_char_p
    lib.mcedm_unet_plan_create.argtypes = [C.POINTER(UNetDesc), C.POINTER(vp)]
    lib.mcedm_unet_plan_destroy.argtypes = [vp]
    lib.mcedm_unet_plan_destroy.restype = None
    lib.mcedm_unet_param_count.argtypes = [vp]
    lib.mcedm_unet_param_info.argtypes = [vp, i32, C.POINTER(C.c_char_p), C.POINTER(C.c_int64), C.POINTER(C.c_int32),
                                          C.POINTER(C.c_int64 * 4)]
    lib.mcedm_unet_packed_bytes.argtypes = [vp, C.POINTER(sz)]
    lib.mcedm_unet_pack_weights.argtypes = [vp, C.POINTER(vp), vp, vp]
    lib.mcedm_unet_workspace_bytes.argtypes = [vp, i32, i32, i32, i32, C.POINTER(sz)]
    lib.mcedm_unet_forward.argtypes = [vp, vp, f32p, f32p, f32p, f32p, i32, f32p, vp, sz, i32, i32, i32, i32, vp]
    lib.mcedm_edm_denoise.argtypes = [vp, vp, f32p, f32p, i32, f32p, f32p, f32p, vp, sz, i32, i32, i32, i32,
                                      C.c_double, vp]
    lib.mcedm_sampler_workspace_bytes.argtypes = [vp, i32, i32, i32, C.POINTER(sz)]
    lib.mcedm_heun_sample.argtypes = [vp, vp, C.POINTER(SamplerDesc), f32p, f32p, f32p, f64p, f64p, i32, vp, sz,
                                      i32, i32, i32, vp]
    lib.mcedm_heun_sample_rng.argtypes = [vp, vp, C.POINTER(SamplerDesc), f32p, f32p, f32p, vp, f64p, i32, vp, sz,
                                          i32, i32, i32, vp]
    lib.mcedm_unet_plan_set_variant.argtypes = [vp, i32, i32]
    lib.mcedm_ddpm_plan_set_variant.argtypes = [vp, i32, i32]
    lib.mcedm_edm_t_steps.argtypes = [C.POINTER(SamplerDesc), C.POINTER(C.c_double)]
    lib.mcedm_edm_loss.argtypes = [f32p, f32p, f32p, f32p, i32, i32, i32, i32, C.c_double, f32p, f32p, vp, sz, vp]
    lib.mcedm_edm_noise_inputs.argtypes = [f32p, f32p, f32p, f32p, i32, i32, i32, i32, C.c_double, C.c_double, f32p,
                                           f32p, vp]
    lib.mcedm_edm_denoise_backward.argtypes = [vp, vp, C.POINTER(vp), f32p, f32p, i32, f32p, f32p, C.POINTER(vp), vp,
                                               sz, i32, i32, i32, C.c_double, vp]
    lib.mcedm_edm_denoise_backward_bucketed.argtypes = [vp, vp, C.POINTER(vp), f32p, f32p, i32, f32p, f32p, C.POINTER(vp),
                                                        vp, sz, i32, i32, i32, C.c_double, i32, C.POINTER(C.c_int32),
                                                        C.POINTER(vp), vp]
    lib.mcedm_unet_grad_buckets.argtypes = [vp, i32, C.POINTER(C.c_int32), C.POINTER(C.c_int)]
    lib.mcedm_unet_forward_dx.argtypes = [vp, vp, f32p, f32p, f32p, f32p, f32p, i32, f32p, vp, sz, i32, i32, i32, i32, vp]
    lib.mcedm_edm_denoise_dx.argtypes = [vp, vp, f32p, f32p, f32p, i32, f32p, f32p, f32p, vp, sz, i32, i32, i32, i32,
                                         C.c_double, vp]
    lib.mcedm_edm_denoise_backward_dx.argtypes = [vp, vp, C.POINTER(vp), f32p, f32p, f32p, i32, f32p, f32p, C.POINTER(vp),
                                                  vp, sz, i32, i32, i32, C.c_double, i32, C.POINTER(C.c_int32),
                                                  C.POINTER(vp), vp]
    lib.mcedm_heun_sample_dxcond.argtypes = [vp, vp, C.POINTER(SamplerDesc), C.POINTER(GuidanceDesc), C.POINTER(GuidanceDesc),
                                             f32p, f32p, f64p, f64p, i32, vp, sz, i32, i32, i32, vp]
    lib.mcedm_sqnorm.argtypes = [f32p, sz, f64p, vp, sz, vp]
    lib.mcedm_adam_ema_step.argtypes = [f32p, f32p, f32p, f32p, f32p, sz, C.c_double, C.c_double, C.c_double,
                                        C.c_double, C.c_double, f64p, C.c_double, C.c_double, C.c_double, C.c_int64, vp]
    lib.mcedm_swe_fv_step.argtypes = [f32p, f32p, i32, i32, i32, C.c_float, C.c_float, vp]
    lib.mcedm_swe_fv_residual.argtypes = [f32p, f32p, f32p, i32, i32, i32, C.c_float, C.c_float, C.c_float, C.c_float,
                                          i32, vp]
    lib.mcedm_darcy_residual.argtypes = [f32p, f32p, i32, i32, C.c_float, C.c_float, i32, vp]
    lib.mcedm_swe_fv_guidance.argtypes = [f32p, f32p, f32p, i32, i32, i32, C.c_float, C.c_float, C.c_float, C.c_float, vp]
    lib.mcedm_darcy_guidance.argtypes = [f32p, f32p, f32p, i32, i32, C.c_float, i32, vp]
    lib.mcedm_heun_sample_guided.argtypes = [vp, vp, C.POINTER(SamplerDesc), C.POINTER(GuidanceDesc), f32p, f32p, f32p, f64p,
                                             f64p, i32, vp, sz, i32, i32, i32, vp]
    lib.mcedm_heun_sample_guided_rng.argtypes = [vp, vp, C.POINTER(SamplerDesc), C.POINTER(GuidanceDesc), f32p, f32p, f32p, vp,
                                                 f64p, i32, vp, sz, i32, i32, i32, vp]
    lib.mcedm_heun_sample_dxcond_rng.argtypes = [vp, vp, C.POINTER(SamplerDesc), C.POINTER(GuidanceDesc), C.POINTER(GuidanceDesc),
                                                 f32p, f32p, vp, f64p, i32, vp, sz, i32, i32, i32, vp]
    lib.mcedm_ddpm_plan_create.argtypes = [C.POINTER(DdpmDesc), C.POINTER(vp)]
    lib.mcedm_ddpm_plan_destroy.argtypes = [vp]
    lib.mcedm_ddpm_plan_destroy.restype = None
    lib.mcedm_ddpm_param_count.argtypes = [vp]
    lib.mcedm_ddpm_param_info.argtypes = [vp, i32, C.POINTER(C.c_char_p), C.POINTER(C.c_int64), C.POINTER(C.c_int32),
                                          C.POINTER(C.c_int64 * 4)]
    lib.mcedm_ddpm_packed_bytes.argtypes = [vp, C.POINTER(sz)]
    lib.mcedm_ddpm_pack_weights.argtypes = [vp, C.POINTER(vp), f32p, vp, vp]
    lib.mcedm_ddpm_workspace_bytes.argtypes = [vp, i32, C.POINTER(sz)]
    lib.mcedm_ddpm_forward.argtypes = [vp, vp, f32p, C.c_float, f32p, vp, sz, i32, vp]
    lib.mcedm_ddpm_denoise.argtypes = [vp, vp, f32p, C.c_float, C.c_float, f32p, f32p, vp, sz, i32, vp]
    lib.mcedm_repaint_schedule.argtypes = [C.POINTER(RepaintDesc), C.POINTER(C.c_double)]
    lib.mcedm_repaint_workspace_bytes.argtypes = [vp, i32, C.POINTER(sz)]
    lib.mcedm_repaint_sample.argtypes = [vp, vp, C.POINTER(RepaintDesc), f32p, f32p, f64p, f64p, f64p, i32, vp, sz, i32, vp]
    lib.mcedm_repaint_sample_rng.argtypes = [vp, vp, C.POINTER(RepaintDesc), f32p, f32p, vp, f64p, i32, vp, sz, i32, vp]
    lib.mcedm_normal_fill.argtypes = [f64p, sz, vp, C.c_uint64, vp]
    lib.mcedm_uniform_fill.argtypes = [f32p, sz, vp, C.c_uint64, vp]
    lib.mcedm_ddpm_forward_sc.argtypes = [vp, vp, f32p, f32p, C.c_float, f32p, vp, sz, i32, vp]
    lib.mcedm_ddim_workspace_bytes.argtypes = [vp, i32, C.POINTER(sz)]
    lib.mcedm_ddim_repaint_sample.argtypes = [vp, vp, C.POINTER(DdimDesc), f32p, f32p, f32p, f32p, f32p, i32, vp, sz, i32, vp]
    lib.mcedm_ddim_repaint_sample_rng.argtypes = [vp, vp, C.POINTER(DdimDesc), f32p, f32p, vp, f32p, f32p, i32, vp, sz, i32, vp]
# ... 27 lines not shown
    lib.mcedm_ddpm_forward_cat.argtypes = [vp, vp, f32p, f32p, C.c_float, f32p, vp, sz, i32, vp]
    lib.mcedm_ddpm_edm_denoise.argtypes = [vp, vp, f32p, f32p, C.c_float, C.c_float, C.c_double, C.c_double, f32p, f32p, vp, sz, i32, vp]
    lib.mcedm_ddpm_edm_sampler_workspace_bytes.argtypes = [vp, i32, C.POINTER(sz)]
    lib.mcedm_ddpm_edm_heun_sample.argtypes = [vp, vp, C.POINTER(VpSamplerDesc), C.c_double, C.POINTER(GuidanceDesc), f32p, f32p, f64p,
                                               f64p, i32, vp, sz, i32, vp]
    lib.mcedm_ddpm_edm_heun_sample_rng.argtypes = [vp, vp, C.POINTER(VpSamplerDesc), C.c_double, C.POINTER(GuidanceDesc), f32p, f32p, vp,
                                                   f64p, i32, vp, sz, i32, vp]
    for name in EXPORTS:
        fn = getattr(lib, name)
        if name not in ("mcedm_last_error", "mcedm_unet_plan_destroy", "mcedm_ddpm_plan_destroy"):
            fn.restype = C.c_int
    _lib = lib
    return lib


def check(rc: int, what: str = "") -> None:
    if rc != 0:
        msg = load().mcedm_last_error().decode(errors="replace")
        raise RuntimeError(f"libmcedm_hip {what} failed ({rc}): {msg}")


def _ptr(t: Optional[torch.Tensor], dtype=torch.float32) -> Optional[int]:
    if t is None:
        return None
    if not t.is_cuda:
        raise RuntimeError("libmcedm_hip needs device tensors (got a CPU tensor); there is no CPU fallback")
    if t.dtype != dtype:
        raise RuntimeError(f"expected dtype {dtype}, got {t.dtype}")
    if not t.is_contiguous():
        raise RuntimeError("expected a contiguous tensor")
    return t.data_ptr()


def _stream() -> int:
    return torch.cuda.current_stream().cuda_stream


def sampler_desc(sp, sigma_data=1.0, net_sigma_min=0.002, net_sigma_max=80.0) -> SamplerDesc:
    return SamplerDesc(int(sp.timesteps), float(sp.sigma_min), float(sp.sigma_max), float(sp.rho), float(sp.S_churn),
                       float(sp.S_min), float(sp.S_max), float(sp.S_noise), float(sp.w), float(sigma_data),
                       float(net_sigma_min), float(net_sigma_max))


def desc_key(desc: C.Structure, skip: Sequence[str] = ()) -> tuple:
    return tuple(getattr(desc, f) for f, _ in desc._fields_ if f not in skip)


def edm_t_steps(sd: SamplerDesc) -> List[float]:
    arr = (C.c_double * (sd.timesteps + 1))()
    check(load().mcedm_edm_t_steps(C.byref(sd), arr), "edm_t_steps")
    return list(arr)


class Workspace:

    def __init__(self):
        self.buf: Optional[torch.Tensor] = None

    def get(self, nbytes: int, device) -> torch.Tensor:
        if self.buf is None or self.buf.numel() < nbytes or self.buf.device != torch.device(device):
            self.buf = None
            self.buf = torch.empty(int(nbytes), dtype=torch.uint8, device=device)
        return self.buf


def _bucket_args(bucket_first, bucket_events, who: str):
    if bucket_first is None:
        return 0, None, None
    nb = len(bucket_first)
    firsts = (C.c_int32 * nb)(*[int(f) for f in bucket_first])
    handles = [int(e.cuda_event) for e in bucket_events]
    if len(handles) != nb or not all(handles):
        raise RuntimeError(f"{who}: one created (recorded at least once) torch.cuda.Event per bucket is needed")
    return nb, firsts, (C.c_void_p * nb)(*handles)


def _seed_ptr(rng_seed: torch.Tensor, device, who: str) -> int:
    if rng_seed.dtype != torch.int64 or rng_seed.numel() != 1 or rng_seed.device != device:
        raise RuntimeError(f"{who}: rng_seed must be a one-element int64 tensor on the sampler's device")
    return rng_seed.data_ptr()


class _PlanBase:
    _SYM = _WHAT = ""

    def _adopt(self, lib, h) -> None:
        self._h, self._lib = h, lib
        self.param_names: List[str] = []
        self.param_shapes: List[tuple] = []
        for i in range(getattr(lib, self._SYM + "_param_count")(h)):
            name, numel, ndim, shape = C.c_char_p(), C.c_int64(), C.c_int32(), (C.c_int64 * 4)()
            check(getattr(lib, self._SYM + "_param_info")(h, i, C.byref(name), C.byref(numel), C.byref(ndim), C.byref(shape)))
            self.param_names.append(name.value.decode())
            self.param_shapes.append(tuple(shape[j] for j in range(ndim.value)))
        self.packed_bytes = self._bytes(self._SYM + "_packed_bytes", "")

    def __del__(self):
        h, self._h = getattr(self, "_h", None), None
        if h:
            getattr(self._lib, self._SYM + "_plan_destroy")(h)

    def set_variant(self, which: str, value: int = -1) -> None:
        fn = getattr(self._lib, self._SYM + "_plan_set_variant")
        check(fn(self._h, VARIANTS[which], int(value)), self._WHAT + "plan_set_variant")

    def _collect(self, params: Dict[str, torch.Tensor]) -> List[torch.Tensor]:
# ... 52 lines not shown
                         ws: Optional["Workspace"] = None, out=None, rng_seed: Optional[torch.Tensor] = None):
        H, W = self._state_hw(init_noise, cond, "cond_ddim_sample")
        B, Cc = init_noise.shape[0], self.in_channels
        S = len(ddim_timesteps(dd.num_diffusion_timesteps, dd.timesteps, dd.skip_type))
        return self._sample_call("cond_ddim_sample", f"mcedm_{self._WHAT}cond_ddim_sample", packed,
                                 (C.byref(dd), _ptr(cond), _ptr(init_noise)),
                                 [("eta_noise", eta_noise, torch.float32, (S,) + tuple(init_noise.shape))], rng_seed, out,
                                 [(B, 1 if return_last else S + 1, H, W, Cc), (B, 1 if return_last else S, H, W, Cc)],
                                 torch.float32, return_last, ws, self.cond_ddim_workspace_bytes(B, H, W), self._dims(B, H, W),
                                 init_noise.device)


class Plan(_PlanBase):
    _SYM, _WHAT = "mcedm_unet", ""

    def __init__(self, in_channels: int, cond_channels: int, out_channels: int, ch: int, ch_mult: Sequence[int],
                 num_res_blocks: int, attn_resolutions: Sequence[int], resolution: int, channels_per_head: int = 64,
                 eps: float = 1e-5, dx_channels: int = 0, dx_mode: int = DX_NONE):
        lib = load()
        if len(ch_mult) > MAX_LEVELS or len(attn_resolutions) > MAX_LEVELS:
            raise RuntimeError("too many levels / attention resolutions")
        d = UNetDesc()
        d.in_channels, d.cond_channels, d.out_channels, d.ch = in_channels, cond_channels, out_channels, ch
        d.n_levels = len(ch_mult)
        for i, m in enumerate(ch_mult):
            d.ch_mult[i] = int(m)
        d.num_res_blocks, d.resolution = num_res_blocks, resolution
        d.n_attn_resolutions = len(attn_resolutions)
        for i, r in enumerate(attn_resolutions):
            d.attn_resolutions[i] = int(r)
        d.channels_per_head, d.eps = channels_per_head, eps
        d.dx_channels, d.dx_mode = int(dx_channels), int(dx_mode)
        self.dx_channels, self.dx_mode = int(dx_channels), int(dx_mode)
        self.desc = d
        h = C.c_void_p()
        check(lib.mcedm_unet_plan_create(C.byref(d), C.byref(h)), "plan_create")
        self._adopt(lib, h)
        self.in_channels, self.cond_channels, self.out_channels = in_channels, cond_channels, out_channels

    def pack(self, params: Dict[str, torch.Tensor], packed: Optional[torch.Tensor] = None) -> torch.Tensor:
        tens = self._collect(params)
        dev = tens[0].device
        if packed is None:
            packed = torch.empty(self.packed_bytes, dtype=torch.uint8, device=dev)
        arr = (C.c_void_p * len(tens))(*[_ptr(t) for t in tens])
        check(self._lib.mcedm_unet_pack_weights(self._h, arr, packed.data_ptr(), _stream()), "pack_weights")
        return packed

    def workspace_bytes(self, B: int, H: int, W: int, training: bool = False) -> int:
        return self._bytes("mcedm_unet_workspace_bytes", "workspace_bytes", B, H, W, int(training))

    def sampler_workspace_bytes(self, B: int, H: int, W: int) -> int:
        return self._bytes("mcedm_sampler_workspace_bytes", "sampler_workspace_bytes", B, H, W)

    def _check_dx(self, x, dx):
        if dx is None:
            return
        if self.dx_mode == DX_NONE:
            raise RuntimeError("dx given to a plan without dx_cond")
        if tuple(dx.shape) != (x.shape[0], self.dx_channels, x.shape[2], x.shape[3]) or dx.dtype != torch.float32:
            raise RuntimeError(f"dx must be fp32 [B, {self.dx_channels}, H, W], got {tuple(dx.shape)} {dx.dtype}")

    def forward(self, packed, x, noise_labels, cond=None, x_scale=None, ws: Optional[Workspace] = None,
                training: bool = False, dx=None) -> torch.Tensor:
        self._check_dx(x, dx)
        B, _, H, W = x.shape
        n_noise = noise_labels.numel()
        ws = ws or Workspace()
        need = self.workspace_bytes(B, H, W, training)
        buf = ws.get(need, x.device)
        out = torch.empty((B, self.out_channels, H, W), dtype=torch.float32, device=x.device)
        check(self._lib.mcedm_unet_forward_dx(self._h, packed.data_ptr(), _ptr(x), _ptr(dx), _ptr(cond), _ptr(x_scale),
                                              _ptr(noise_labels), n_noise, _ptr(out), buf.data_ptr(), buf.numel(), B, H, W,
                                              int(training), _stream()), "unet_forward")
        return out

    def denoise(self, packed, x, sigma, cond=None, ws: Optional[Workspace] = None, training: bool = False,
                sigma_data: float = 1.0, want_F: bool = False, dx=None):
        self._check_dx(x, dx)
        B, _, H, W = x.shape
        n_sigma = sigma.numel()
        ws = ws or Workspace()
        buf = ws.get(self.workspace_bytes(B, H, W, training), x.device)
        D = torch.empty((B, self.out_channels, H, W), dtype=torch.float32, device=x.device)
        F = torch.empty_like(D) if want_F else None
        check(self._lib.mcedm_edm_denoise_dx(self._h, packed.data_ptr(), _ptr(x), _ptr(dx), _ptr(sigma), n_sigma, _ptr(cond),
                                             _ptr(D), _ptr(F), buf.data_ptr(), buf.numel(), B, H, W, int(training),
                                             float(sigma_data), _stream()), "edm_denoise")
        return (D, F) if want_F else D

    def grad_buckets(self, max_buckets: int) -> List[int]:
        arr = (C.c_int32 * max(1, max_buckets))()
        n = C.c_int()
        check(self._lib.mcedm_unet_grad_buckets(self._h, int(max_buckets), arr, C.byref(n)), "grad_buckets")
        return [arr[i] for i in range(n.value)]

    def denoise_backward(self, packed, params: Dict[str, torch.Tensor], x, sigma, cond, dD, grads: Sequence[torch.Tensor],
                         ws: Workspace, sigma_data: float = 1.0, bucket_first: Optional[Sequence[int]] = None,
                         bucket_events: Optional[Sequence[torch.cuda.Event]] = None, dx=None) -> None:
        self._check_dx(x, dx)
        B, _, H, W = x.shape
        buf = ws.get(self.workspace_bytes(B, H, W, True), x.device)
        parr = (C.c_void_p * len(self.param_names))(*[_ptr(params[n].detach()) for n in self.param_names])
        garr = (C.c_void_p * len(self.param_names))(*[_ptr(g) for g in grads])
        if dx is None and bucket_first is None:
            check(self._lib.mcedm_edm_denoise_backward(self._h, packed.data_ptr(), parr, _ptr(x), _ptr(sigma), sigma.numel(),
# ... 650 lines not shown
def _bind_ops():
    global _OPS_BOUND
    lib = load()
    if _OPS_BOUND:
        return lib
    vp, i32, sz = C.c_void_p, C.c_int, C.c_size_t
    lib.mcedm_op_conv_packed_floats.argtypes = [i32, i32, i32]
    lib.mcedm_op_conv_packed_floats.restype = sz
    lib.mcedm_op_pack_conv.argtypes = [vp, vp, i32, i32, i32, i32, i32, vp, vp, vp]
    lib.mcedm_op_gn_coef.argtypes = [vp, vp, i32, i32, i32, i32, vp, vp, vp, i32, i32, C.c_float, vp, vp, vp]
    lib.mcedm_op_conv.argtypes = [vp, vp, i32, i32, vp, i32, i32, i32, i32, i32, i32, i32, vp, vp, vp, i32, vp, i32,
                                  i32, i32, vp]
    lib.mcedm_op_attention.argtypes = [vp, vp, i32, i32, i32, vp]
    lib.mcedm_op_attn_block64.argtypes = [vp, vp, vp, C.c_float, vp, vp, vp, vp, vp, vp, i32, vp]
    lib.mcedm_op_embedding.argtypes = [vp, i32, i32, vp, vp, vp, vp, vp, vp, i32, vp, vp, vp, vp]
    lib.mcedm_op_wgrad_scratch_floats.argtypes = [i32, i32, i32, i32, i32, i32]
    lib.mcedm_op_wgrad_scratch_floats.restype = sz
    lib.mcedm_op_conv_wgrad.argtypes = [vp, vp, vp, i32, i32, vp, i32, i32, i32, i32, i32, i32, i32, i32, i32, i32, i32,
                                        vp, vp, vp, vp]
    lib.mcedm_op_gn_bwd.argtypes = [vp, i32, vp, vp, i32, i32, i32, i32, i32, vp, vp, vp, vp, vp, i32, i32, i32, vp, vp,
                                    i32, vp, i32, vp, vp, vp, vp, i32, vp]
    lib.mcedm_op_gn_bwd_sync.argtypes = [vp, i32, vp, vp, i32, i32, i32, i32, i32, vp, vp, vp, vp, vp, i32, i32, i32, vp, vp,
                                         i32, vp, i32, vp, vp, vp, vp, i32, vp, vp]
    lib.mcedm_op_attention_bwd.argtypes = [vp, vp, vp, vp, vp, i32, i32, i32, vp]
    lib.mcedm_op_conv_wino_packed_floats.argtypes = [i32, i32]
    lib.mcedm_op_conv_wino_packed_floats.restype = sz
    lib.mcedm_op_pack_conv_wino.argtypes = [vp, i32, i32, vp, vp]
    lib.mcedm_op_pack_conv_wino_dgrad.argtypes = [vp, i32, i32, vp, vp]
    lib.mcedm_op_conv_wino.argtypes = [vp, vp, i32, i32, vp, i32, i32, i32, i32, i32, vp, vp, vp, i32, vp, i32, i32, vp]
    lib.mcedm_op_conv_wino_sums.argtypes = [vp, vp, i32, i32, vp, i32, i32, i32, i32, i32, vp, vp, vp, i32, vp, vp, i32, i32, vp]
    lib.mcedm_op_pack_conv_frag.argtypes = [vp, i32, i32, vp, vp]
    lib.mcedm_op_conv_skip.argtypes = [vp, i32, vp, i32, i32, i32, vp, vp, vp, vp, vp, vp, i32, i32, vp, vp, vp, vp, vp, i32, i32, vp]
    f32 = C.c_float
    lib.mcedm_op_ddim_cond_step.argtypes = [vp, vp, vp, vp, C.c_double, f32, f32, f32, f32, f32, vp, vp, vp, i32, i32, i32, i32, i32,
                                            i32, vp, i32, i32, vp, i32, i32, vp]
    lib.mcedm_op_ddim_cond_step_rng.argtypes = [vp, vp, vp, vp, C.c_uint64, C.c_double, f32, f32, f32, f32, f32, vp, vp, vp, i32, i32,
                                                i32, i32, i32, i32, vp, i32, i32, vp, i32, i32, vp]
    for n in ("mcedm_op_pack_conv", "mcedm_op_gn_coef", "mcedm_op_conv", "mcedm_op_attention", "mcedm_op_embedding", "mcedm_op_conv_wgrad",
              "mcedm_op_gn_bwd", "mcedm_op_gn_bwd_sync", "mcedm_op_attention_bwd", "mcedm_op_pack_conv_wino", "mcedm_op_conv_wino",
              "mcedm_op_conv_wino_sums", "mcedm_op_pack_conv_wino_dgrad", "mcedm_op_ddim_cond_step", "mcedm_op_ddim_cond_step_rng", "mcedm_op_pack_conv_frag", "mcedm_op_conv_skip",
              "mcedm_op_attn_block64"):
        getattr(lib, n).restype = C.c_int
    _OPS_BOUND = True
    return lib


OP_EXPORTS = ["mcedm_op_conv_packed_floats", "mcedm_op_pack_conv", "mcedm_op_gn_coef", "mcedm_op_conv",
              "mcedm_op_attention", "mcedm_op_set_conv_tile", "mcedm_prof_enable", "mcedm_prof_report",
              "mcedm_op_wgrad_scratch_floats", "mcedm_op_conv_wgrad", "mcedm_op_gn_bwd", "mcedm_op_attention_bwd",
              "mcedm_op_set_conv_debug", "mcedm_op_set_conv8", "mcedm_op_set_conv_resident", "mcedm_op_set_attn_fused", "mcedm_op_embedding",
              "mcedm_op_conv_wino_packed_floats", "mcedm_op_pack_conv_wino", "mcedm_op_conv_wino", "mcedm_op_set_conv_wino", "mcedm_op_set_conv_wino1",
              "mcedm_op_set_wgrad_wino", "mcedm_op_set_conv1x1_reg", "mcedm_op_gn_bwd_sync", "mcedm_op_pack_conv_wino_dgrad",
              "mcedm_op_ddim_cond_step", "mcedm_op_ddim_cond_step_rng", "mcedm_op_set_conv_wino_fold", "mcedm_op_set_conv_wino_upz", "mcedm_op_conv_wino_sums", "mcedm_op_pack_conv_frag", "mcedm_op_conv_skip",
              "mcedm_op_attn_block64"]


def prof_enable(on: bool) -> None:
    lib = load()
    lib.mcedm_prof_enable.argtypes = [C.c_int]
    check(lib.mcedm_prof_enable(int(on)), "prof_enable")


def prof_report() -> list:
    import json
    lib = load()
    lib.mcedm_prof_report.argtypes = [C.c_char_p, C.c_size_t]
    buf = C.create_string_buffer(1 << 16)
    check(lib.mcedm_prof_report(buf, len(buf)), "prof_report")
    return json.loads(buf.value.decode())


def set_conv_tile(mt: int = 0, ph: int = 0, pw: int = 0) -> None:
    lib = _bind_ops()
    lib.mcedm_op_set_conv_tile.argtypes = [C.c_int, C.c_int, C.c_int]
    check(lib.mcedm_op_set_conv_tile(mt, ph, pw), "set_conv_tile")
def set_conv8(enable: int = -1) -> None:
    lib = _bind_ops()
    lib.mcedm_op_set_conv8.argtypes = [C.c_int]
    check(lib.mcedm_op_set_conv8(int(enable)), "set_conv8")


def set_conv_wino(enable: int = -1) -> None:
    lib = _bind_ops()
    lib.mcedm_op_set_conv_wino.argtypes = [C.c_int]
    check(lib.mcedm_op_set_conv_wino(int(enable)), "set_conv_wino")


def set_conv_wino1(enable: int = -1) -> None:
    lib = _bind_ops()
    lib.mcedm_op_set_conv_wino1.argtypes = [C.c_int]
    check(lib.mcedm_op_set_conv_wino1(int(enable)), "set_conv_wino1")


def set_conv1x1_reg(enable: int = -1) -> None:
    lib = _bind_ops()
    lib.mcedm_op_set_conv1x1_reg.argtypes = [C.c_int]
    check(lib.mcedm_op_set_conv1x1_reg(int(enable)), "set_conv1x1_reg")


def set_conv_wino_fold(enable: int = -1) -> None:
    lib = _bind_ops()
    lib.mcedm_op_set_conv_wino_fold.argtypes = [C.c_int]
    check(lib.mcedm_op_set_conv_wino_fold(int(enable)), "set_conv_wino_fold")


def set_conv_wino_upz(enable: int = -1) -> None:
    lib = _bind_ops()
    lib.mcedm_op_set_conv_wino_upz.argtypes = [C.c_int]
    check(lib.mcedm_op_set_conv_wino_upz(int(enable)), "set_conv_wino_upz")


def set_wgrad_wino(enable: int = -1) -> None:
    lib = _bind_ops()
    lib.mcedm_op_set_wgrad_wino.argtypes = [C.c_int]
    check(lib.mcedm_op_set_wgrad_wino(int(enable)), "set_wgrad_wino")


def set_conv_resident(enable: int = -1) -> None:
    lib = _bind_ops()
    lib.mcedm_op_set_conv_resident.argtypes = [C.c_int]
    check(lib.mcedm_op_set_conv_resident(int(enable)), "set_conv_resident")


def set_attn_fused(enable: int = -1) -> None:
    lib = _bind_ops()
    lib.mcedm_op_set_attn_fused.argtypes = [C.c_int]
    check(lib.mcedm_op_set_attn_fused(int(enable)), "set_attn_fused")


def set_conv_debug(buf: Optional[torch.Tensor] = None) -> None:
    lib = _bind_ops()
    lib.mcedm_op_set_conv_debug.argtypes = [C.c_void_p]
    if buf is not None and (not buf.is_cuda or buf.element_size() != 8 or not buf.is_contiguous() or buf.numel() % 16):
        raise ValueError("set_conv_debug: buf must be a contiguous device tensor of 64-bit words, 16 per workgroup")
    check(lib.mcedm_op_set_conv_debug(buf.data_ptr() if buf is not None else None), "set_conv_debug")


RS_NONE, RS_UP, RS_DOWN, RS_S2 = 0, 1, 2, 3


def op_pack_conv(w: torch.Tensor, b: Optional[torch.Tensor], qkv_heads: int = 0, dgrad: bool = False):
    lib = _bind_ops()
    Cout, Cin, k, _ = w.shape
    rows, cols = (Cin, Cout) if dgrad else (Cout, Cin)
    n = lib.mcedm_op_conv_packed_floats(rows, cols, k)
    wpk = torch.empty(n, dtype=torch.float32, device=w.device)
    bpk = torch.zeros((Cout + 31) // 32 * 32, dtype=torch.float32, device=w.device) if b is not None else None
    check(lib.mcedm_op_pack_conv(_ptr(w), _ptr(b), Cout, Cin, k, qkv_heads, int(dgrad), _ptr(wpk), _ptr(bpk), _stream()),
          "op_pack_conv")
    return wpk, bpk


def op_gn_coef(xa, xb, gamma, beta, film=None, film_batch=0, film_stride=0, eps=1e-5, want_stats=False):
    lib = _bind_ops()
    B, Ca = xa.shape[:2]
    Cb = xb.shape[1] if xb is not None else 0
    HW = xa[0, 0].numel()
    Ct = Ca + Cb
    coef = torch.empty((B, Ct, 4), dtype=torch.float32, device=xa.device)
    stats = torch.empty((B, min(32, Ct // 4), 2), dtype=torch.float32, device=xa.device) if want_stats else None
    check(lib.mcedm_op_gn_coef(_ptr(xa), _ptr(xb), Ca, Cb, B, HW, _ptr(gamma), _ptr(beta), _ptr(film), film_batch,
                               film_stride, eps, _ptr(coef), _ptr(stats), _stream()), "op_gn_coef")
# ... 161 lines not shown
```

Measured before the change: 81.92 states/s.

## Add thin-input conv kernel and precomputed per-step sampler tables with fused Heun precond

Adds a specialized 3x3 conv kernel for layers with at most 4 input channels (the U-Net input conv). It stages input tiles in LDS with double buffering and uses MFMA with a small K, instead of the generic path that pads Cin to 8. The sampler now precomputes the preconditioning coefficients, noise embeddings and FiLM rows for every evaluation sigma in one upfront pass, then indexes these tables per step. It also fuses the precond finish into the Heun Euler and correct update kernels. This removes per-step small kernel launches and redundant embedding work, at the cost of extra workspace and a stricter check that each evaluation matches its table row.

```diff
diff --git a/include/mcedm_hip.h b/include/mcedm_hip.h
--- a/include/mcedm_hip.h
+++ b/include/mcedm_hip.h
@@ -66,6 +66,7 @@
 #define MCEDM_VARIANT_CONV1X1_REG 6
 #define MCEDM_VARIANT_CONV_WINO_FOLD 7
 #define MCEDM_VARIANT_CONV_WINO_UPZ 8
+#define MCEDM_VARIANT_CONV_THIN_IN 9
 int mcedm_unet_plan_set_variant(mcedm_plan* plan, int which, int value);
 
 int mcedm_unet_param_count(const mcedm_plan* plan);
@@ -131,6 +132,8 @@
                                  const float* init_noise, const uint64_t* rng_seed, double* out, int return_last, void* workspace,
                                  size_t workspace_bytes, int B, int H, int W, void* stream);
 int mcedm_edm_t_steps(const mcedm_sampler_desc* sp, double* t_steps);
+int mcedm_edm_eval_sigmas(const mcedm_sampler_desc* sp, float* sigmas);
+int mcedm_sampler_table_bytes(const mcedm_plan* plan, size_t* bytes);
 
 int mcedm_edm_loss(const float* D, const float* x, const float* mask, const float* sigma, int B, int C,
                    int H, int W, double sigma_data, float* loss_out, float* dD_out, void* scratch, size_t scratch_bytes,
@@ -269,6 +272,8 @@
 int mcedm_op_set_conv1x1_reg(int enable);
 int mcedm_op_set_conv_wino_fold(int enable);
 int mcedm_op_set_conv_wino_upz(int enable);
+int mcedm_op_set_conv_thin_in(int enable);
+int mcedm_op_set_sampler_tables(int enable);
 int mcedm_op_pack_conv_frag(const float* w, int Cout, int Cin, float* wfrag, void* stream);
 int mcedm_op_conv_skip(const float* x, int Cin, const mcedm_coef* coef, int act, int H, int W, const float* wpk, const float* wino,
                        const float* bias, const float* res, const float* sk_xa, const float* sk_xb, int sk_Ca, int sk_Cb,
diff --git a/m-cedm_amd/csrc/common.hpp b/m-cedm_amd/csrc/common.hpp
--- a/m-cedm_amd/csrc/common.hpp
+++ b/m-cedm_amd/csrc/common.hpp
@@ -37,8 +37,8 @@
   } while (0)
 
 enum KernelVariant { KV_CONV_WINO = 0, KV_CONV_WINO1 = 1, KV_CONV_RESIDENT = 2, KV_CONV8 = 3, KV_ATTN_FUSED = 4, KV_WGRAD_WINO = 5,
-                     KV_CONV1X1_REG = 6, KV_CONV_WINO_FOLD = 7, KV_CONV_WINO_UPZ = 8, KV_COUNT = 9 };
-struct KernelVariants { int v[KV_COUNT] = {-1, -1, -1, -1, -1, -1, -1, -1, -1}; };
+                     KV_CONV1X1_REG = 6, KV_CONV_WINO_FOLD = 7, KV_CONV_WINO_UPZ = 8, KV_CONV_THIN_IN = 9, KV_COUNT = 10 };
+struct KernelVariants { int v[KV_COUNT] = {-1, -1, -1, -1, -1, -1, -1, -1, -1, -1}; };
 const KernelVariants* current_variants();
 struct VariantScope {
   const KernelVariants* prev;
@@ -155,6 +155,8 @@
 int try_launch_conv_resident(const ConvArgs& a, int taps, hipStream_t stream);
 int try_launch_conv1x1_reg(const ConvArgs& a, int taps, hipStream_t stream);
 void set_conv1x1_reg(int enable);
+int try_launch_conv_thin_in(const ConvArgs& a, int taps, hipStream_t stream);
+void set_conv_thin_in(int enable);
 void set_conv_resident(int enable);
 static inline int conv_max_tiles(int H, int W) { return ((H + 3) / 4) * ((W + 7) / 8); }
 void set_conv_tile_override(int mt, int ph, int pw);
diff --git a/m-cedm_amd/csrc/conv_mfma.hip b/m-cedm_amd/csrc/conv_mfma.hip
--- a/m-cedm_amd/csrc/conv_mfma.hip
+++ b/m-cedm_amd/csrc/conv_mfma.hip
@@ -814,6 +814,10 @@
     const int rc = try_launch_conv_resident(a, taps, stream);
     if (rc != -1) return rc;
   }
+  if (!g_force_mt) {
+    const int rc = try_launch_conv_thin_in(a, taps, stream);
+    if (rc != -1) return rc;
+  }
   return taps == 9 ? dispatch<9, 8>(a, stream) : dispatch<1, 16>(a, stream);
 }
 
diff --git a/m-cedm_amd/csrc/conv_thin_in.hip b/m-cedm_amd/csrc/conv_thin_in.hip
--- /dev/null
+++ b/m-cedm_amd/csrc/conv_thin_in.hip
@@ -0,0 +1,194 @@
+#include <cstdlib>
+
+#include "common.hpp"
+#include "conv_tile.hpp"
+#include "prof.hpp"
+
+namespace mcedm {
+
+template <int MT_, int NP_>
+struct ThinCfg : ConvCfg<MT_, 8, 32, 1, 4, 9, 8> {
+  static constexpr int NP = NP_, NCH = 2 * NP_;
+  static constexpr int PER = 4;
+};
+
+template <class C>
+__global__ __launch_bounds__(256, 2) void conv_thin_in_kernel(ConvArgs p, int tiles_x, int tiles, int mtiles, int groups,
+                                                              int coutp) {
+  constexpr int NCH = C::NCH, NP = C::NP, SUB = (C::PLANE + 255) / 256;
+  __shared__ __attribute__((aligned(16))) float xl[2][NCH * C::PLANE];
+  __shared__ __attribute__((aligned(16))) float wl[9 * NCH * C::MT];
+  __shared__ __attribute__((aligned(16))) float red[4 * (C::MT / 2) * 3];
+  __shared__ __attribute__((aligned(16))) float bl[C::MT];
+  extern __shared__ __attribute__((aligned(16))) float dyn_lds[];
+  Coef* cfl = reinterpret_cast<Coef*>(dyn_lds);
+  const int tid = threadIdx.x;
+  const int lane = tid & 63;
+  const int wn = tid >> 6;
+
+  int bid = blockIdx.x;
+  const int mt = bid % mtiles; bid /= mtiles;
+  const int g = bid % groups;
+  const int n = bid / groups;
+  const int m0 = mt * C::MT;
+  const int t0 = g * C::PER;
+  const int cnt = tiles - t0 < C::PER ? tiles - t0 : C::PER;
+
+  int er[SUB], ec[SUB];
+#pragma unroll
+  for (int sub = 0; sub < SUB; ++sub) {
+    const int e = tid + sub * 256;
+    er[sub] = e / C::PITCH; ec[sub] = e - er[sub] * C::PITCH;
+  }
+  const int Cin = p.Ca + p.Cb;
+  const size_t plane = (size_t)p.H * p.W;
+  const float* safe = p.xa ? p.xa : p.xb;
+  const float* pl[NCH];
+  unsigned ckeep[NCH];
+#pragma unroll
+  for (int ci = 0; ci < NCH; ++ci) {
+    const bool in_a = ci < p.Ca;
+    const float* src = in_a ? p.xa : p.xb;
+    const int cc = in_a ? ci : ci - p.Ca, CC = in_a ? p.Ca : p.Cb;
+    const bool ok = ci < Cin && src != nullptr;
+    pl[ci] = ok ? src + ((size_t)n * CC + cc) * plane : safe;
+    ckeep[ci] = ok ? 0xffffffffu : 0u;
+  }
+  float raw[NCH][SUB];
+  unsigned keep[SUB];
+  auto issue = [&](int t) {
+    const int ty = t / tiles_x, tx = t - ty * tiles_x;
+#pragma unroll
+    for (int sub = 0; sub < SUB; ++sub) {
+      const int y = ty * C::PH + er[sub] - 1, x = tx * C::PW + ec[sub] - 1;
+      const bool inb = tid + sub * 256 < C::PLANE && (unsigned)y < (unsigned)p.H && (unsigned)x < (unsigned)p.W;
+      keep[sub] = inb ? 0xffffffffu : 0u;
+      const unsigned off = inb ? (unsigned)(y * p.W + x) : 0u;
+#pragma unroll
+      for (int ci = 0; ci < NCH; ++ci) raw[ci][sub] = pl[ci][off];
+    }
+  };
+  auto commit = [&](float* dst) {
+#pragma unroll
+    for (int ci = 0; ci < NCH; ++ci) {
+      const Coef cf = cfl[ci < Cin ? ci : Cin - 1];
+#pragma unroll
+      for (int sub = 0; sub < SUB; ++sub) {
+        float v = apply_coef(raw[ci][sub], cf, p.act);
+        v = __builtin_bit_cast(float, __builtin_bit_cast(unsigned, v) & (keep[sub] & ckeep[ci]));
+        if (tid + sub * 256 < C::PLANE) dst[ci * C::PLANE + tid + sub * 256] = v;
+      }
+    }
+  };
+
+  issue(t0);
+  {
+    constexpr int V4 = C::MT / 4;
+    for (int idx = tid; idx < 9 * NCH * V4; idx += 256) {
+      const int row = idx / V4, c4 = idx - row * V4;
+      const int tap = row / NCH, cil = row - tap * NCH;
+      reinterpret_cast<f32x4*>(wl)[idx] = *reinterpret_cast<const f32x4*>(p.wpk + (size_t)(tap * 8 + cil) * coutp + m0 + c4 * 4);
+    }
+  }
+  stage_coef_rows<256>(p, n, cfl, tid);
+  if (tid < C::MT) bl[tid] = (p.bias ? p.bias[m0 + tid] : 0.f) + 0.f;
+  __syncthreads();
+  commit(xl[0]);
+
+  const int aoff = (lane >> 5) * C::MT + (lane & 31);
+  int boff[C::TN];
+#pragma unroll
+  for (int j = 0; j < C::TN; ++j) boff[j] = (lane >> 5) * C::PLANE + (wn * C::TN + j) * C::PITCH + (lane & 31);
+
+#pragma unroll 1
+  for (int k = 0; k < cnt; ++k) {
+    const int t = t0 + k;
+    issue(t0 + (k + 1 < cnt ? k + 1 : k));
+    __syncthreads();
+    const float* xc = xl[k & 1];
+    f32x16 acc[C::TM][C::TN];
+#pragma unroll
+    for (int i = 0; i < C::TM; ++i) {
+#pragma unroll
+      for (int q = 0; q < 4; ++q) {
+        const f32x4 b4 = *reinterpret_cast<const f32x4*>(bl + i * 32 + 4 * (lane >> 5) + 8 * q);
+#pragma unroll
+        for (int j = 0; j < C::TN; ++j)
+#pragma unroll
+          for (int r = 0; r < 4; ++r) acc[i][j][4 * q + r] = b4[r];
+      }
+    }
+#pragma unroll
+    for (int tap = 0; tap < 9; ++tap) {
+      const int toff = (tap / 3) * C::PITCH + tap % 3;
+#pragma unroll
+      for (int kk = 0; kk < NP; ++kk) {
+        float fa[C::TM], fb[C::TN];
+#pragma unroll
+        for (int i = 0; i < C::TM; ++i) fa[i] = wl[aoff + (tap * NCH + 2 * kk) * C::MT + i * 32];
+#pragma unroll
+        for (int j = 0; j < C::TN; ++j) fb[j] = xc[boff[j] + toff + 2 * kk * C::PLANE];
+#pragma unroll
+        for (int i = 0; i < C::TM; ++i)
+#pragma unroll
+          for (int j = 0; j < C::TN; ++j) acc[i][j] = __builtin_amdgcn_mfma_f32_32x32x2f32(fa[i], fb[j], acc[i][j], 0, 0, 0);
+      }
+    }
+#pragma unroll
+    for (int i = 0; i < C::TM; ++i)
+#pragma unroll
+      for (int j = 0; j < C::TN; ++j) acc[i][j] = __builtin_amdgcn_mfma_f32_32x32x2f32(0.f, 0.f, acc[i][j], 0, 0, 0);
+    commit(xl[(k + 1) & 1]);
+    const int ty = t / tiles_x, tx = t - ty * tiles_x;
+    int ne = n, me = m0;
+    asm volatile("" : "+s"(ne), "+s"(me));
+    if (!p.gsum) conv_epilogue<C, true, 0>(p, acc, ne, me, ty * C::PH, tx * C::PW, 0, wn, lane, red);
+    else if (p.gsum_rc == 2) conv_epilogue<C, true, 2>(p, acc, ne, me, ty * C::PH, tx * C::PW, 0, wn, lane, red);
+    else conv_epilogue<C, true, 4>(p, acc, ne, me, ty * C::PH, tx * C::PW, 0, wn, lane, red);
+    if (p.gsum) {
+      __syncthreads();
+      conv_stats_store<C, C::WN>(p, red, n, m0, t, tiles, tid);
+    }
+  }
+}
+
+static int g_thin_in = -1;
+void set_conv_thin_in(int enable) { g_thin_in = enable; }
+
+template <class C>
+static int launch_thin(const ConvArgs& a, hipStream_t stream) {
+  const int tiles_x = a.W / C::PW, tiles = tiles_x * (a.H / C::PH);
+  const int mtiles = a.Cout / C::MT;
+  const int groups = ceil_div(tiles, C::PER);
+  const long long blocks = (long long)a.B * groups * mtiles;
+  if (blocks <= 0 || blocks > 0x7fffffffLL) { set_error("conv grid out of range (%lld blocks)", blocks); return MCEDM_ERR_INVALID; }
+  char name[64] = "";
+  if (prof_enabled()) snprintf(name, sizeof(name), "conv_thin_in_kernel<ThinCfg<%d, %d> >", C::MT, C::NP);
+  const double px = (double)a.B * a.H * a.W;
+  const int Cin = a.Ca + a.Cb;
+  ProfScope ps(name, 2.0 * px * a.Cout * (double)Cin * 9, 4.0 * ((double)a.B * Cin * a.Hs * a.Ws + px * a.Cout + (double)a.Cout * Cin * 9),
+               stream);
+  hipLaunchKernelGGL((conv_thin_in_kernel<C>), dim3((unsigned)blocks), dim3(256), (unsigned)Cin * (unsigned)sizeof(Coef), stream, a,
+                     tiles_x, tiles, mtiles, groups, cout_padded(a.Cout));
+  MCEDM_LAUNCH_CHECK("conv_thin_in_kernel");
+  if (a.gsum_tiles) *a.gsum_tiles = SumTiles{tiles, tiles_x, C::PH, C::PW, a.gsum_rc == 2 ? 2 : 4};
+  return MCEDM_OK;
+}
+
+int try_launch_conv_thin_in(const ConvArgs& a_in, int taps, hipStream_t stream) {
+  static int env = -1;
+  if (env < 0) { const char* e = getenv("MCEDM_CONV_THIN_IN"); env = e ? atoi(e) : 1; }
+  const int on = variant_choice(KV_CONV_THIN_IN, g_thin_in, env);
+  const int Cin = a_in.Ca + a_in.Cb;
+  if (!on || taps != 9 || (!a_in.xa && !a_in.xb) || a_in.resample != RS_NONE || a_in.res || a_in.sk_wpk || Cin > 4 || a_in.Cout % 64 != 0 || a_in.W % 32 != 0 ||
+      a_in.H % 8 != 0 || ((long long)a_in.H * a_in.W < 4096 && on != 2))
+    return -1;
+  ConvArgs a = a_in;
+  a.dbg = nullptr;
+  const int rc = conv_resolve_identity(a);
+  if (rc) return rc;
+  if (a.Cout % 128 == 0) return Cin <= 2 ? launch_thin<ThinCfg<128, 1>>(a, stream) : launch_thin<ThinCfg<128, 2>>(a, stream);
+  return Cin <= 2 ? launch_thin<ThinCfg<64, 1>>(a, stream) : launch_thin<ThinCfg<64, 2>>(a, stream);
+}
+
+}
diff --git a/m-cedm_amd/csrc/edm.hip b/m-cedm_amd/csrc/edm.hip
--- a/m-cedm_amd/csrc/edm.hip
+++ b/m-cedm_amd/csrc/edm.hip
@@ -1,5 +1,6 @@
 #include "common.hpp"
 #include "edm.hpp"
+#include "prof.hpp"
 
 namespace mcedm {
 
@@ -8,12 +9,8 @@
   return (int)(b < 2048 ? (b ? b : 1) : 2048);
 }
 
-__global__ void precond_prepare_kernel(const float* __restrict__ sigma_dev, float sigma_host, int use_host, int n,
-                                       float sigma_data, int cond_ch, int in_ch, int dx_ch, float* __restrict__ coefs4,
-                                       float* __restrict__ c_noise, Coef* __restrict__ conv_in_coef) {
-  const int i = blockIdx.x * blockDim.x + threadIdx.x;
-  if (i >= n) return;
-  const float s = use_host ? sigma_host : sigma_dev[i];
+__device__ __forceinline__ void precond_rows(float s, int i, float sigma_data, int cond_ch, int in_ch, int dx_ch,
+                                             float* __restrict__ coefs4, float* __restrict__ c_noise, Coef* __restrict__ conv_in_coef) {
   const float sd2 = sigma_data * sigma_data;
   const float s2 = s * s;
   const float c_skip = sd2 / (s2 + sd2);
@@ -30,9 +27,40 @@
     conv_in_coef[(size_t)i * Ct + c] = Coef{0.f, (c < cond_ch || c >= cond_ch + in_ch) ? 1.0f : c_in, 0.f, 0.f};
 }
 
+__global__ void precond_prepare_kernel(const float* __restrict__ sigma_dev, float sigma_host, int use_host, int n,
+                                       float sigma_data, int cond_ch, int in_ch, int dx_ch, float* __restrict__ coefs4,
+                                       float* __restrict__ c_noise, Coef* __restrict__ conv_in_coef) {
+  const int i = blockIdx.x * blockDim.x + threadIdx.x;
+  if (i >= n) return;
+  precond_rows(use_host ? sigma_host : sigma_dev[i], i, sigma_data, cond_ch, in_ch, dx_ch, coefs4, c_noise, conv_in_coef);
+}
+
+struct SigmaRowArgs { float s[SIGMA_ROWS]; };
+__global__ void precond_prepare_rows_kernel(SigmaRowArgs sig, int n, int row0, float sigma_data, int cond_ch, int in_ch, int dx_ch,
+                                            float* __restrict__ coefs4, float* __restrict__ c_noise, Coef* __restrict__ conv_in_coef) {
+  const int i = threadIdx.x;
+  if (i >= n) return;
+  precond_rows(sig.s[i], row0 + i, sigma_data, cond_ch, in_ch, dx_ch, coefs4, c_noise, conv_in_coef);
+}
+
+int launch_precond_prepare_rows(const float* sigmas_host, int n, float sigma_data, int cond_ch, int in_ch, int dx_ch, float* coefs4,
+                                float* c_noise, Coef* conv_in_coef, hipStream_t stream) {
+  for (int row0 = 0; row0 < n; row0 += SIGMA_ROWS) {
+    SigmaRowArgs sig{};
+    const int m = n - row0 < SIGMA_ROWS ? n - row0 : SIGMA_ROWS;
+    for (int i = 0; i < m; ++i) sig.s[i] = sigmas_host[row0 + i];
+    ProfScope ps("precond_prepare_rows_kernel", 0.0, 4.0 * m * (5 + 4 * (cond_ch + in_ch + dx_ch)), stream);
+    hipLaunchKernelGGL(precond_prepare_rows_kernel, dim3(1), dim3(SIGMA_ROWS), 0, stream, sig, m, row0, sigma_data, cond_ch, in_ch,
+                       dx_ch, coefs4, c_noise, conv_in_coef);
+    MCEDM_LAUNCH_CHECK("precond_prepare_rows_kernel");
+  }
+  return MCEDM_OK;
+}
+
 int launch_precond_prepare(const float* sigma_dev, float sigma_host, int use_host, int n, float sigma_data,
                            int cond_ch, int in_ch, int dx_ch, float* coefs4, float* c_noise, Coef* conv_in_coef,
                            hipStream_t stream) {
+  ProfScope ps("precond_prepare_kernel", 0.0, 4.0 * n * (5 + 4 * (cond_ch + in_ch + dx_ch)), stream);
   hipLaunchKernelGGL(precond_prepare_kernel, dim3(ceil_div(n, 64)), dim3(64), 0, stream, sigma_dev, sigma_host,
                      use_host, n, sigma_data, cond_ch, in_ch, dx_ch, coefs4, c_noise, conv_in_coef);
   MCEDM_LAUNCH_CHECK("precond_prepare_kernel");
@@ -54,6 +82,7 @@
 
 int launch_precond_finish(const float* x, const float* F, const float* Fu, float w, const float* coefs4, int n_sigma,
                           size_t per_sample, size_t total, float* D, float* F_out, hipStream_t stream) {
+  ProfScope ps("precond_finish_kernel", 3.0 * total, 4.0 * total * (Fu ? 4 : 3), stream);
   hipLaunchKernelGGL(precond_finish_kernel, dim3(grid_for(total)), dim3(256), 0, stream, x, F, Fu, w, coefs4, n_sigma,
                      per_sample, total, D, F_out);
   MCEDM_LAUNCH_CHECK("precond_finish_kernel");
@@ -98,6 +127,21 @@
   }
 }
 
+__global__ void heun_euler_precond_kernel(const double* __restrict__ x_hat, const float* __restrict__ F, const float* __restrict__ c4,
+                                          const float* __restrict__ mask, double t_hat, double dt, size_t total,
+                                          double* __restrict__ d_cur, double* __restrict__ x_next, float* __restrict__ x32) {
+  const float c_skip = c4[0], c_out = c4[1];
+  for (size_t i = blockIdx.x * (size_t)blockDim.x + threadIdx.x; i < total; i += (size_t)gridDim.x * blockDim.x) {
+    const float D = c_skip * x32[i] + c_out * F[i];
+    const double xh = x_hat[i];
+    const double d = (xh - (double)D) / t_hat;
+    const double v = xh + (dt * d) * (mask ? (double)mask[i] : 1.0);
+    d_cur[i] = d;
+    x_next[i] = v;
+    x32[i] = (float)v;
+  }
+}
+
 __global__ void heun_correct_kernel(const double* __restrict__ x_hat, const double* __restrict__ d_cur,
                                     const float* __restrict__ D, const float* __restrict__ mask, double t_next, double dt,
                                     size_t total, double* __restrict__ x_next, float* __restrict__ x32,
@@ -111,6 +155,20 @@
   }
 }
 
+__global__ void heun_correct_precond_kernel(const double* __restrict__ x_hat, const double* __restrict__ d_cur,
+                                            const float* __restrict__ F, const float* __restrict__ c4, const float* __restrict__ mask,
+                                            double t_next, double dt, size_t total, double* __restrict__ x_next,
+                                            float* __restrict__ x32) {
+  const float c_skip = c4[0], c_out = c4[1];
+  for (size_t i = blockIdx.x * (size_t)blockDim.x + threadIdx.x; i < total; i += (size_t)gridDim.x * blockDim.x) {
+    const float D = c_skip * x32[i] + c_out * F[i];
+    const double dp = (x_next[i] - (double)D) / t_next;
+    const double v = x_hat[i] + (dt * (0.5 * d_cur[i] + 0.5 * dp)) * (mask ? (double)mask[i] : 1.0);
+    x_next[i] = v;
+    x32[i] = (float)v;
+  }
+}
+
 __global__ void heun_store_kernel(const double* __restrict__ x, int C, size_t hw, int t, int T, size_t total,
                                   double* __restrict__ out) {
   for (size_t i = blockIdx.x * (size_t)blockDim.x + threadIdx.x; i < total; i += (size_t)gridDim.x * blockDim.x) {
@@ -134,7 +192,15 @@
   return MCEDM_OK;
 }
 int launch_heun_euler(const double* x_hat, const float* D, const float* mask, double t_hat, double dt, size_t total,
-                      double* d_cur, double* x_next, float* x32, hipStream_t s, const float* dxg, float wgt, float gdiv) {
+                      double* d_cur, double* x_next, float* x32, hipStream_t s, const float* dxg, float wgt, float gdiv,
+                      const float* F, const float* c4) {
+  if (F) {
+    MCEDM_REQUIRE(c4 && !dxg, "heun_euler: the fused preconditioning needs its coefficient row and has no guidance term");
+    hipLaunchKernelGGL(heun_euler_precond_kernel, dim3(grid_for(total)), dim3(256), 0, s, x_hat, F, c4, mask, t_hat, dt, total, d_cur,
+                       x_next, x32);
+    MCEDM_LAUNCH_CHECK("heun_euler_precond_kernel");
+    return MCEDM_OK;
+  }
   hipLaunchKernelGGL(heun_euler_kernel, dim3(grid_for(total)), dim3(256), 0, s, x_hat, D, mask, t_hat, dt, total, d_cur,
                      x_next, x32, dxg, wgt, gdiv);
   MCEDM_LAUNCH_CHECK("heun_euler_kernel");
@@ -142,7 +208,14 @@
 }
 int launch_heun_correct(const double* x_hat, const double* d_cur, const float* D, const float* mask, double t_next,
                         double dt, size_t total, double* x_next, float* x32, hipStream_t s, const float* dxg, float wgt,
-                        float gdiv) {
+                        float gdiv, const float* F, const float* c4) {
+  if (F) {
+    MCEDM_REQUIRE(c4 && !dxg, "heun_correct: the fused preconditioning needs its coefficient row and has no guidance term");
+    hipLaunchKernelGGL(heun_correct_precond_kernel, dim3(grid_for(total)), dim3(256), 0, s, x_hat, d_cur, F, c4, mask, t_next, dt,
+                       total, x_next, x32);
+    MCEDM_LAUNCH_CHECK("heun_correct_precond_kernel");
+    return MCEDM_OK;
+  }
   hipLaunchKernelGGL(heun_correct_kernel, dim3(grid_for(total)), dim3(256), 0, s, x_hat, d_cur, D, mask, t_next, dt,
                      total, x_next, x32, dxg, wgt, gdiv);
   MCEDM_LAUNCH_CHECK("heun_correct_kernel");
diff --git a/m-cedm_amd/csrc/edm.hpp b/m-cedm_amd/csrc/edm.hpp
--- a/m-cedm_amd/csrc/edm.hpp
+++ b/m-cedm_amd/csrc/edm.hpp
@@ -9,6 +9,9 @@
 int launch_precond_prepare(const float* sigma_dev, float sigma_host, int use_host, int n, float sigma_data,
                            int cond_ch, int in_ch, int dx_ch, float* coefs4, float* c_noise, Coef* conv_in_coef,
                            hipStream_t stream);
+constexpr int SIGMA_ROWS = 64;
+int launch_precond_prepare_rows(const float* sigmas_host, int n, float sigma_data, int cond_ch, int in_ch, int dx_ch, float* coefs4,
+                                float* c_noise, Coef* conv_in_coef, hipStream_t stream);
 int launch_precond_finish(const float* x, const float* F, const float* Fu, float w, const float* coefs4, int n_sigma,
                           size_t per_sample, size_t total, float* D, float* F_out, hipStream_t stream);
 int launch_heun_init(const float* cond, int cond_ch, int in_ch, size_t hw, const float* mask, const float* noise,
@@ -21,10 +24,11 @@
 int launch_uniform_fill(float* out, const unsigned long long* seed_dev, unsigned long long draw, size_t total, hipStream_t s);
 int launch_heun_euler(const double* x_hat, const float* D, const float* mask, double t_hat, double dt, size_t total,
                       double* d_cur, double* x_next, float* x32, hipStream_t s, const float* dxg = nullptr, float wgt = 0.f,
-                      float gdiv = 1.f);
+                      float gdiv = 1.f, const float* F = nullptr, const float* c4 = nullptr);
 int launch_heun_correct(const double* x_hat, const double* d_cur, const float* D, const float* mask, double t_next,
                         double dt, size_t total, double* x_next, float* x32, hipStream_t s, const float* dxg = nullptr,
-                        float wgt = 0.f, float gdiv = 1.f);
+                        float wgt = 0.f, float gdiv = 1.f, const float* F = nullptr, const float* c4 = nullptr);
+void set_sampler_tables(int enable);
 int launch_heun_store(const double* x, int C, size_t hw, int t, int T, size_t total, double* out, hipStream_t s);
 
 struct GuideIO {
diff --git a/m-cedm_amd/csrc/heun.hpp b/m-cedm_amd/csrc/heun.hpp
--- a/m-cedm_amd/csrc/heun.hpp
+++ b/m-cedm_amd/csrc/heun.hpp
@@ -26,6 +26,8 @@
   int N, Tout, return_last;
   hipStream_t s;
   double* out;
+  const float* F = nullptr;
+  const float* c4 = nullptr;
 };
 static inline HeunState heun_state(void* ws, const HeunBufs& b, int B, int C, size_t hw, int N, int return_last, double* out,
                                    hipStream_t s) {
@@ -59,11 +61,11 @@
                               const float* dxg = nullptr, float wgt = 0.f, float gdiv = 1.f) {
   int rc;
   if ((rc = denoise(t_hat, false))) return rc;
-  if ((rc = launch_heun_euler(h.x, h.D, mask, t_hat, t_next - t_hat, h.total, h.d, h.xn, h.x32, h.s, dxg, wgt, gdiv)))
+  if ((rc = launch_heun_euler(h.x, h.D, mask, t_hat, t_next - t_hat, h.total, h.d, h.xn, h.x32, h.s, dxg, wgt, gdiv, h.F, h.c4)))
     return rc;
   if (i < h.N - 1) {
     if ((rc = denoise(t_next, true))) return rc;
-    if ((rc = launch_heun_correct(h.x, h.d, h.D, mask, t_next, t_next - t_hat, h.total, h.xn, h.x32, h.s, dxg, wgt, gdiv)))
+    if ((rc = launch_heun_correct(h.x, h.d, h.D, mask, t_next, t_next - t_hat, h.total, h.xn, h.x32, h.s, dxg, wgt, gdiv, h.F, h.c4)))
       return rc;
   }
   std::swap(h.x, h.xn);
diff --git a/m-cedm_amd/csrc/norm_emb_attn.hip b/m-cedm_amd/csrc/norm_emb_attn.hip
--- a/m-cedm_amd/csrc/norm_emb_attn.hip
+++ b/m-cedm_amd/csrc/norm_emb_attn.hip
@@ -234,6 +234,8 @@
   int nsplit = a.rows / 64;
   if (nsplit > 512 / a.n) nsplit = 512 / a.n;
   if (nsplit < 1) nsplit = 1;
+  ProfScope ps("embedding_kernel", 2.0 * a.n * ((double)nsplit * 2 * a.ch * a.ch + (double)a.rows * a.ch),
+               4.0 * ((double)a.rows * a.ch + 2.0 * a.ch * a.ch + (double)a.n * a.rows), stream);
   hipLaunchKernelGGL(embedding_kernel, dim3(a.n, nsplit), dim3(EMB_NT), 2 * a.ch * sizeof(float), stream, a);
   MCEDM_LAUNCH_CHECK("embedding_kernel");
   return MCEDM_OK;
diff --git a/m-cedm_amd/csrc/ops_api.hip b/m-cedm_amd/csrc/ops_api.hip
--- a/m-cedm_amd/csrc/ops_api.hip
+++ b/m-cedm_amd/csrc/ops_api.hip
@@ -229,6 +229,16 @@
 
 extern "C" int mcedm_op_set_conv_wino_upz(int enable) {
   set_conv_wino_upz(enable);
+  return MCEDM_OK;
+}
+
+extern "C" int mcedm_op_set_conv_thin_in(int enable) {
+  set_conv_thin_in(enable);
+  return MCEDM_OK;
+}
+
+extern "C" int mcedm_op_set_sampler_tables(int enable) {
+  set_sampler_tables(enable);
   return MCEDM_OK;
 }
 
diff --git a/m-cedm_amd/csrc/plan.hip b/m-cedm_amd/csrc/plan.hip
--- a/m-cedm_amd/csrc/plan.hip
+++ b/m-cedm_amd/csrc/plan.hip
@@ -524,7 +524,7 @@
 }
 
 static int run_block(const mcedm_plan& P, const BlockP& b, const BlockLayout& bl, const Layout& L, void* act,
-                     const float* pk, int B, int n_noise, hipStream_t s, std::vector<SumTiles>& st) {
+                     const float* pk, int B, int n_noise, hipStream_t s, std::vector<SumTiles>& st, const float* film_table) {
   auto T = [&](int id) -> float* { return id < 0 ? nullptr : at<float>(act, L.t[id].off); };
   auto CF = [&](int id) -> Coef* { return id < 0 ? nullptr : at<Coef>(act, L.t[id].off); };
   auto SUMS = [&](int id) -> float* { return (id < 0 || L.t[id].sums == NONE) ? nullptr : at<float>(act, L.t[id].sums); };
@@ -555,7 +555,7 @@
     c0.coef = nullptr; c0.act = 0; c0.resample = RS_NONE; c0.Hs = bl.H; c0.Ws = bl.W;
   }
   if ((rc = launch_conv(c0, 9, s))) return rc;
-  const float* film = at<float>(act, L.t[L.film].off) + b.film_row0;
+  const float* film = film_table + b.film_row0;
   GnArgs g1{T(bl.h), nullptr, b.cout, 0, bl.H * bl.W, B, b.norm1.groups, pk + b.norm1.gamma, pk + b.norm1.beta,
             film, n_noise > 1 ? 1 : 0, P.film_rows, eps, CF(bl.coef1), T(bl.stats1), SUMS(bl.h), nullptr, TL(bl.h), SumTiles{}, bl.W};
   const float* res = xa;
@@ -634,15 +634,23 @@
   return MCEDM_OK;
 }
 
+int launch_plan_embedding(const mcedm_plan& P, const float* pk, const float* labels, int n, float* film, hipStream_t s) {
+  EmbArgs e{labels, n, P.desc.ch, pk + P.freqs, pk + P.w0, pk + P.b0, pk + P.w1, pk + P.b1,
+            pk + P.waff, pk + P.baff, P.film_rows, nullptr, film};
+  return launch_embedding(e, s);
+}
+
 int forward_impl(const mcedm_plan& P, const Layout& L, const float* pk, const float* x, const float* dx, const float* cond,
                  const Coef* coef_in, int coef_batch, const float* noise_labels, int n_noise, float* out,
-                 void* act, int B, int H, int W, hipStream_t s) {
-  const int ch = P.desc.ch;
+                 void* act, int B, int H, int W, hipStream_t s, const float* film_ready) {
   const int dxm = P.desc.dx_mode;
   int rc;
-  EmbArgs e{noise_labels, n_noise, ch, pk + P.freqs, pk + P.w0, pk + P.b0, pk + P.w1, pk + P.b1,
-            pk + P.waff, pk + P.baff, P.film_rows, nullptr, at<float>(act, L.t[L.film].off)};
-  if ((rc = launch_embedding(e, s))) return rc;
+  const float* film_table = film_ready;
+  if (!film_table) {
+    float* film = at<float>(act, L.t[L.film].off);
+    if ((rc = launch_plan_embedding(P, pk, noise_labels, n_noise, film, s))) return rc;
+    film_table = film;
+  }
   std::vector<SumTiles> st(L.t.size());
   ConvArgs ci{};
   ci.xa = cond; ci.Ca = P.desc.cond_channels;
@@ -691,8 +699,8 @@
     if ((rc = launch_conv(cc, 9, s))) return rc;
   }
   size_t bi = 0;
-  for (const BlockP& b : P.enc) if ((rc = run_block(P, b, L.blocks[bi++], L, act, pk, B, n_noise, s, st))) return rc;
-  for (const BlockP& b : P.dec) if ((rc = run_block(P, b, L.blocks[bi++], L, act, pk, B, n_noise, s, st))) return rc;
+  for (const BlockP& b : P.enc) if ((rc = run_block(P, b, L.blocks[bi++], L, act, pk, B, n_noise, s, st, film_table))) return rc;
+  for (const BlockP& b : P.dec) if ((rc = run_block(P, b, L.blocks[bi++], L, act, pk, B, n_noise, s, st, film_table))) return rc;
   const TRef& last = L.t[L.last];
   GnArgs go{at<float>(act, last.off), nullptr, last.C, 0, H * W, B, P.out_norm.groups, pk + P.out_norm.gamma,
             pk + P.out_norm.beta, nullptr, 0, 0, 1e-5f, at<Coef>(act, L.t[L.coef_out].off),
@@ -718,23 +726,25 @@
 int denoise_impl(const mcedm_plan& P, const Layout& L, const Header& hd, const float* pk, const float* x, const float* dx,
                  const float* sigma_dev, float sigma_host, int use_host, int n_sigma, const float* cond,
                  float w, float* D_out, float* F_out, void* ws, int B, int H, int W, float sigma_data,
-                 hipStream_t s) {
+                 hipStream_t s, const EvalTables* pre) {
   int rc;
-  float* coefs4 = at<float>(ws, hd.coefs4);
-  float* c_noise = at<float>(ws, hd.c_noise);
-  Coef* coef_in = at<Coef>(ws, hd.coef_in);
+  const float* coefs4 = pre ? pre->coefs4 : at<float>(ws, hd.coefs4);
+  const float* c_noise = pre ? pre->c_noise : at<float>(ws, hd.c_noise);
+  const Coef* coef_in = pre ? pre->coef_in : at<Coef>(ws, hd.coef_in);
+  const float* film = pre ? pre->film : nullptr;
   float* Fbuf = at<float>(ws, hd.F);
   void* act = at<char>(ws, hd.total);
-  if ((rc = launch_precond_prepare(sigma_dev, sigma_host, use_host, n_sigma, sigma_data, P.desc.cond_channels,
-                                   P.desc.in_channels, P.desc.dx_mode == MCEDM_DX_CAT ? P.desc.dx_channels : 0, coefs4, c_noise,
-                                   coef_in, s))) return rc;
-  if ((rc = forward_impl(P, L, pk, x, dx, cond, coef_in, n_sigma > 1 ? 1 : 0, c_noise, n_sigma, Fbuf, act, B, H, W, s))) return rc;
+  if (!pre && (rc = launch_precond_prepare(sigma_dev, sigma_host, use_host, n_sigma, sigma_data, P.desc.cond_channels,
+                                           P.desc.in_channels, P.desc.dx_mode == MCEDM_DX_CAT ? P.desc.dx_channels : 0,
+                                           at<float>(ws, hd.coefs4), at<float>(ws, hd.c_noise), at<Coef>(ws, hd.coef_in), s))) return rc;
+  if ((rc = forward_impl(P, L, pk, x, dx, cond, coef_in, n_sigma > 1 ? 1 : 0, c_noise, n_sigma, Fbuf, act, B, H, W, s, film))) return rc;
   const float* Fu = nullptr;
   if (fabsf(w) >= 0.001f && (cond != nullptr || dx != nullptr)) {
     float* Fubuf = at<float>(ws, hd.Fu);
-    if ((rc = forward_impl(P, L, pk, x, nullptr, nullptr, coef_in, n_sigma > 1 ? 1 : 0, c_noise, n_sigma, Fubuf, act, B, H, W, s))) return rc;
+    if ((rc = forward_impl(P, L, pk, x, nullptr, nullptr, coef_in, n_sigma > 1 ? 1 : 0, c_noise, n_sigma, Fubuf, act, B, H, W, s, film))) return rc;
     Fu = Fubuf;
   }
+  if (pre && pre->leave_F && !Fu && !F_out) return MCEDM_OK;
   const size_t per = (size_t)P.desc.out_channels * H * W;
   return launch_precond_finish(x, Fbuf, Fu, w, coefs4, n_sigma, per, per * B, D_out, F_out, s);
 }
diff --git a/m-cedm_amd/csrc/plan.hpp b/m-cedm_amd/csrc/plan.hpp
--- a/m-cedm_amd/csrc/plan.hpp
+++ b/m-cedm_amd/csrc/plan.hpp
@@ -187,11 +187,13 @@
 
 int forward_impl(const mcedm_plan& P, const Layout& L, const float* pk, const float* x, const float* dx, const float* cond,
                  const Coef* coef_in, int coef_batch, const float* noise_labels, int n_noise, float* out,
-                 void* act, int B, int H, int W, hipStream_t s);
+                 void* act, int B, int H, int W, hipStream_t s, const float* film_ready = nullptr);
+int launch_plan_embedding(const mcedm_plan& P, const float* pk, const float* labels, int n, float* film, hipStream_t s);
+struct EvalTables { const float* coefs4; const float* c_noise; const Coef* coef_in; const float* film; int leave_F; };
 int denoise_impl(const mcedm_plan& P, const Layout& L, const Header& hd, const float* pk, const float* x, const float* dx,
                  const float* sigma_dev, float sigma_host, int use_host, int n_sigma, const float* cond,
                  float w, float* D_out, float* F_out, void* ws, int B, int H, int W, float sigma_data,
-                 hipStream_t s);
+                 hipStream_t s, const EvalTables* pre = nullptr);
 
 size_t backward_scratch_bytes(const mcedm_plan& P, const Layout& L, int B, int H, int W);
 }
diff --git a/m-cedm_amd/csrc/sampler.hip b/m-cedm_amd/csrc/sampler.hip
--- a/m-cedm_amd/csrc/sampler.hip
+++ b/m-cedm_amd/csrc/sampler.hip
@@ -1,5 +1,6 @@
 #include <algorithm>
 #include <cmath>
+#include <cstdlib>
 #include <vector>
 
 #include "heun.hpp"
@@ -18,15 +19,73 @@
   return MCEDM_OK;
 }
 
+static void edm_eval_sigma_list(const std::vector<double>& t, const std::vector<double>& gammas, std::vector<float>& sig) {
+  const int N = (int)gammas.size();
+  sig.clear();
+  for (int i = 0; i < N; ++i) {
+    sig.push_back((float)(t[i] + gammas[i] * t[i]));
+    if (i < N - 1) sig.push_back((float)t[i + 1]);
+  }
+}
+static int edm_schedule(const mcedm_sampler_desc* sp, std::vector<double>& t, std::vector<double>& gammas) {
+  const int N = sp->timesteps;
+  t.resize(N + 1);
+  const int rc = mcedm_edm_t_steps(sp, t.data());
+  if (rc) return rc;
+  gammas.resize(N);
+  for (int i = 0; i < N; ++i) {
+    const bool in_range = sp->S_min <= t[i] && t[i] <= sp->S_max;
+    gammas[i] = in_range ? std::min(sp->S_churn / N, std::sqrt(2.0) - 1.0) : 0.0;
+  }
+  return MCEDM_OK;
+}
+
+extern "C" int mcedm_edm_eval_sigmas(const mcedm_sampler_desc* sp, float* sigmas) {
+  MCEDM_REQUIRE(sp && sigmas, "edm_eval_sigmas: null argument");
+  MCEDM_REQUIRE(sp->timesteps >= 2 && sp->timesteps <= 4096, "edm_eval_sigmas: timesteps=%d out of range", sp->timesteps);
+  std::vector<double> t, gammas;
+  std::vector<float> sig;
+  const int rc = edm_schedule(sp, t, gammas);
+  if (rc) return rc;
+  edm_eval_sigma_list(t, gammas, sig);
+  std::copy(sig.begin(), sig.end(), sigmas);
+  return MCEDM_OK;
+}
+
 namespace mcedm {
-struct SamplerBufs : HeunBufs { size_t dx, g, dxin; };
+static int g_sampler_tables = -1;
+void set_sampler_tables(int enable) { g_sampler_tables = enable; }
+static bool sampler_tables_on() {
+  static int env = -1;
+  if (env < 0) { const char* e = getenv("MCEDM_SAMPLER_TABLES"); env = e ? atoi(e) : 1; }
+  return (g_sampler_tables >= 0 ? g_sampler_tables : env) != 0;
+}
+
+constexpr int SAMPLER_TABLE_ROWS = 128;
+struct SamplerBufs : HeunBufs { size_t dx, g, dxin, t_coefs4, t_cnoise, t_coefin, t_film; };
+static size_t sampler_table_bytes(const mcedm_plan& P) {
+  const int Ct = P.desc.in_channels + P.desc.cond_channels + P.desc.dx_channels;
+  const size_t R = SAMPLER_TABLE_ROWS;
+  return align_up(R * 4 * sizeof(float), 256) + align_up(R * sizeof(float), 256) + align_up(R * Ct * sizeof(Coef), 256) +
+         align_up(R * P.film_rows * sizeof(float), 256);
+}
 static SamplerBufs sampler_bufs(const mcedm_plan& P, int B, int H, int W) {
   const size_t n = (size_t)B * P.desc.in_channels * H * W;
-  SamplerBufs s{heun_bufs(n), 0, 0, 0};
+  SamplerBufs s{heun_bufs(n), 0, 0, 0, 0, 0, 0, 0};
   s.dx = heun_take(s, n * 4); s.g = heun_take(s, n * 4);
   s.dxin = heun_take(s, n * 4);
+  const int Ct = P.desc.in_channels + P.desc.cond_channels + P.desc.dx_channels;
+  const size_t R = SAMPLER_TABLE_ROWS;
+  s.t_coefs4 = heun_take(s, R * 4 * sizeof(float)); s.t_cnoise = heun_take(s, R * sizeof(float));
+  s.t_coefin = heun_take(s, R * Ct * sizeof(Coef)); s.t_film = heun_take(s, R * P.film_rows * sizeof(float));
   return s;
 }
+}
+
+extern "C" int mcedm_sampler_table_bytes(const mcedm_plan* plan, size_t* bytes) {
+  MCEDM_REQUIRE(plan && bytes, "sampler_table_bytes: null argument");
+  *bytes = sampler_table_bytes(*plan);
+  return MCEDM_OK;
 }
 
 extern "C" int mcedm_sampler_workspace_bytes(const mcedm_plan* plan, int B, int H, int W, size_t* bytes) {
@@ -50,14 +109,10 @@
                 "heun_sample: with a mask, cond must carry hu_known in its first %d channels", P.desc.in_channels);
   MCEDM_REQUIRE(sp->timesteps >= 2 && sp->timesteps <= 4096, "heun_sample: timesteps=%d out of range", sp->timesteps);
   const int N = sp->timesteps;
-  std::vector<double> t(N + 1);
-  if ((rc = mcedm_edm_t_steps(sp, t.data()))) return rc;
-  std::vector<double> gammas(N);
-  for (int i = 0; i < N; ++i) {
-    const bool in_range = sp->S_min <= t[i] && t[i] <= sp->S_max;
-    gammas[i] = in_range ? std::min(sp->S_churn / N, std::sqrt(2.0) - 1.0) : 0.0;
+  std::vector<double> t, gammas;
+  if ((rc = edm_schedule(sp, t, gammas))) return rc;
+  for (int i = 0; i < N; ++i)
     MCEDM_REQUIRE(gammas[i] == 0.0 || step_noise != nullptr || rng_seed != nullptr, "heun_sample: S_churn > 0 needs step_noise (or mcedm_heun_sample_rng)");
-  }
   Layout L;
   if ((rc = build_layout(P, B, H, W, 0, 1, &L))) return rc;
   const Header hd = header_for(P, B, H, W);
@@ -73,11 +128,34 @@
   float* dxin = dxc ? at<float>(workspace, sb.dxin) : nullptr;
   float* dxg = gd ? at<float>(workspace, sb.dx) : nullptr;
   const float wgt = gd ? (float)gd->weight : 0.f;
+  std::vector<float> sig;
+  edm_eval_sigma_list(t, gammas, sig);
+  const int n_ev = (int)sig.size();
+  const bool tables = sampler_tables_on() && n_ev <= SAMPLER_TABLE_ROWS;
+  const bool blend = fabsf(w) >= 0.001f && (cond != nullptr || dxc != nullptr);
+  const bool fuse = tables && !gd && !blend;
+  const int Ct = P.desc.cond_channels + P.desc.in_channels + (P.desc.dx_mode == MCEDM_DX_CAT ? P.desc.dx_channels : 0);
+  float* t_coefs4 = at<float>(workspace, sb.t_coefs4);
+  float* t_cnoise = at<float>(workspace, sb.t_cnoise);
+  Coef* t_coefin = at<Coef>(workspace, sb.t_coefin);
+  float* t_film = at<float>(workspace, sb.t_film);
+  if (tables) {
+    if ((rc = launch_precond_prepare_rows(sig.data(), n_ev, sd, P.desc.cond_channels, P.desc.in_channels,
+                                          P.desc.dx_mode == MCEDM_DX_CAT ? P.desc.dx_channels : 0, t_coefs4, t_cnoise, t_coefin, s))) return rc;
+    if ((rc = launch_plan_embedding(P, pk, t_cnoise, n_ev, t_film, s))) return rc;
+  }
+  int ev = 0;
   auto denoise = [&](double sigma, bool) -> int {
     int e = dxc ? guidance_dx(P.desc.cond_channels, *dxc, cond, h.x32, dxin, gscratch, B, H, W, s) : MCEDM_OK;
     if (e) return e;
-    e = denoise_impl(P, L, hd, pk, h.x32, dxin, nullptr, (float)sigma, 1, 1, cond, w, h.D, nullptr, uws, B, H, W, sd, s);
+    MCEDM_REQUIRE(ev < n_ev && sig[ev] == (float)sigma, "heun_sample: evaluation %d is not at the noise level of its table row", ev);
+    EvalTables row{t_coefs4 + 4 * (size_t)ev, t_cnoise + ev, t_coefin + (size_t)ev * Ct, t_film + (size_t)ev * P.film_rows, fuse ? 1 : 0};
+    e = denoise_impl(P, L, hd, pk, h.x32, dxin, nullptr, (float)sigma, 1, 1, cond, w, h.D, nullptr, uws, B, H, W, sd, s,
+                     tables ? &row : nullptr);
     if (e) return e;
+    h.F = fuse ? at<float>(uws, hd.F) : nullptr;
+    h.c4 = fuse ? row.coefs4 : nullptr;
+    ++ev;
     return gd ? guidance_dx(P.desc.cond_channels, *gd, cond, h.D, dxg, gscratch, B, H, W, s) : MCEDM_OK;
   };
 
diff --git a/m-cedm_amd/lib.py b/m-cedm_amd/lib.py
--- a/m-cedm_amd/lib.py
+++ b/m-cedm_amd/lib.py
@@ -14,7 +14,7 @@
     "mcedm_version", "mcedm_last_error", "mcedm_unet_plan_create", "mcedm_unet_plan_destroy",
     "mcedm_unet_param_count", "mcedm_unet_param_info", "mcedm_unet_packed_bytes", "mcedm_unet_pack_weights",
     "mcedm_unet_workspace_bytes", "mcedm_unet_forward", "mcedm_edm_denoise", "mcedm_sampler_workspace_bytes",
-    "mcedm_heun_sample", "mcedm_edm_t_steps", "mcedm_edm_loss", "mcedm_edm_noise_inputs",
+    "mcedm_heun_sample", "mcedm_edm_t_steps", "mcedm_edm_eval_sigmas", "mcedm_sampler_table_bytes", "mcedm_edm_loss", "mcedm_edm_noise_inputs",
     "mcedm_edm_denoise_backward", "mcedm_edm_denoise_backward_bucketed", "mcedm_unet_grad_buckets", "mcedm_sqnorm",
     "mcedm_adam_ema_step",
     "mcedm_swe_fv_step", "mcedm_swe_fv_residual", "mcedm_darcy_residual", "mcedm_swe_fv_guidance", "mcedm_darcy_guidance",
@@ -44,7 +44,7 @@
 }
 GN_SYNC_WORDS = 130
 VARIANTS = {"conv_wino": 0, "conv_wino1": 1, "conv_resident": 2, "conv8": 3, "attn_fused": 4, "wgrad_wino": 5, "conv1x1_reg": 6,
-            "conv_wino_fold": 7, "conv_wino_upz": 8}
+            "conv_wino_fold": 7, "conv_wino_upz": 8, "conv_thin_in": 9}
 
 
 class UNetDesc(C.Structure):
@@ -145,6 +145,8 @@
     lib.mcedm_unet_plan_set_variant.argtypes = [vp, i32, i32]
     lib.mcedm_ddpm_plan_set_variant.argtypes = [vp, i32, i32]
     lib.mcedm_edm_t_steps.argtypes = [C.POINTER(SamplerDesc), C.POINTER(C.c_double)]
+    lib.mcedm_edm_eval_sigmas.argtypes = [C.POINTER(SamplerDesc), C.POINTER(C.c_float)]
+    lib.mcedm_sampler_table_bytes.argtypes = [vp, C.POINTER(sz)]
     lib.mcedm_edm_loss.argtypes = [f32p, f32p, f32p, f32p, i32, i32, i32, i32, C.c_double, f32p, f32p, vp, sz, vp]
     lib.mcedm_edm_noise_inputs.argtypes = [f32p, f32p, f32p, f32p, i32, i32, i32, i32, C.c_double, C.c_double, f32p,
                                            f32p, vp]
@@ -278,6 +280,12 @@
     return list(arr)
 
 
+def edm_eval_sigmas(sd: SamplerDesc) -> List[float]:
+    arr = (C.c_float * (2 * sd.timesteps - 1))()
+    check(load().mcedm_edm_eval_sigmas(C.byref(sd), arr), "edm_eval_sigmas")
+    return list(arr)
+
+
 class Workspace:
 
     def __init__(self):
@@ -436,6 +444,9 @@
 
     def sampler_workspace_bytes(self, B: int, H: int, W: int) -> int:
         return self._bytes("mcedm_sampler_workspace_bytes", "sampler_workspace_bytes", B, H, W)
+
+    def sampler_table_bytes(self) -> int:
+        return self._bytes("mcedm_sampler_table_bytes", "sampler_table_bytes")
 
     def _check_dx(self, x, dx):
         if dx is None:
@@ -1192,7 +1203,7 @@
               "mcedm_op_conv_wino_packed_floats", "mcedm_op_pack_conv_wino", "mcedm_op_conv_wino", "mcedm_op_set_conv_wino", "mcedm_op_set_conv_wino1",
               "mcedm_op_set_wgrad_wino", "mcedm_op_set_conv1x1_reg", "mcedm_op_gn_bwd_sync", "mcedm_op_pack_conv_wino_dgrad",
               "mcedm_op_ddim_cond_step", "mcedm_op_ddim_cond_step_rng", "mcedm_op_set_conv_wino_fold", "mcedm_op_set_conv_wino_upz", "mcedm_op_conv_wino_sums", "mcedm_op_pack_conv_frag", "mcedm_op_conv_skip",
-              "mcedm_op_attn_block64"]
+              "mcedm_op_attn_block64", "mcedm_op_set_conv_thin_in", "mcedm_op_set_sampler_tables"]
 
 
 def prof_enable(on: bool) -> None:
@@ -1248,6 +1259,18 @@
     lib = _bind_ops()
     lib.mcedm_op_set_conv_wino_upz.argtypes = [C.c_int]
     check(lib.mcedm_op_set_conv_wino_upz(int(enable)), "set_conv_wino_upz")
+
+
+def set_conv_thin_in(enable: int = -1) -> None:
+    lib = _bind_ops()
+    lib.mcedm_op_set_conv_thin_in.argtypes = [C.c_int]
+    check(lib.mcedm_op_set_conv_thin_in(int(enable)), "set_conv_thin_in")
+
+
+def set_sampler_tables(enable: int = -1) -> None:
+    lib = _bind_ops()
+    lib.mcedm_op_set_sampler_tables.argtypes = [C.c_int]
+    check(lib.mcedm_op_set_sampler_tables(int(enable)), "set_sampler_tables")
 
 
 def set_wgrad_wino(enable: int = -1) -> None:
```

Result: no change. 82.49 states/s (median of 6 runs) (+0.7%).
